# rrwick/Autocycler

Measured on NVIDIA H100. Metric: input-assembly Mbp/sec through compress->unitig GFA, higher is better.
Workload: dtype u64

## Files before the change

### autocycler_b200/csrc/backend.h

```cpp
#pragma once
#include <cstddef>
#include <cstdint>
#include <cstdio>
#include <cstdlib>
#include <cstring>
#include <stdexcept>
#include <string>

extern unsigned long long g_ac_kernel_launches;

#ifdef AC_EMULATE
#define AC_HD inline
#define AC_D inline

template <class T> inline T ac_atomic_cas(T* p, T cmp, T val) { T old = *p; if (old == cmp) *p = val; return old; }
template <class T> inline T ac_atomic_add(T* p, T v) { T old = *p; *p = (T)(old + v); return old; }
template <class T> inline T ac_atomic_or(T* p, T v) { T old = *p; *p = (T)(old | v); return old; }
template <class T> inline T ac_atomic_and(T* p, T v) { T old = *p; *p = (T)(old & v); return old; }
template <class T> inline T ac_atomic_min(T* p, T v) { T old = *p; if (v < old) *p = v; return old; }
template <class T> inline T ac_atomic_max(T* p, T v) { T old = *p; if (v > old) *p = v; return old; }
template <class T> inline T ac_ld_volatile(const T* p) { return *p; }
template <class T> inline T ac_ld_cg(const T* p) { return *p; }
inline void ac_st_stream(uint32_t* p, uint32_t v) { *p = v; }
inline void ac_ld_group(const uint64_t* p, uint64_t out[4]) { out[0] = p[0]; out[1] = p[1]; out[2] = p[2]; out[3] = p[3]; }
inline uint64_t ac_umul64hi(uint64_t a, uint64_t b) { return (uint64_t)(((unsigned __int128)a * b) >> 64); }
inline uint32_t ac_popc(uint32_t v) { return (uint32_t)__builtin_popcount(v); }
inline int ac_ctz(uint32_t v) { return __builtin_ctz(v); }

struct AcStream { int dummy; };

inline void* ac_dev_alloc(size_t bytes) { void* p = malloc(bytes ? bytes : 1); if (!p) throw std::runtime_error("emu alloc failed"); return p; }
inline void ac_dev_free(void* p) { free(p); }
inline void ac_memset(void* p, int v, size_t bytes, AcStream*) { memset(p, v, bytes); }
inline void ac_h2d(void* d, const void* h, size_t bytes, AcStream*) { memcpy(d, h, bytes); }
inline void ac_d2h(void* h, const void* d, size_t bytes, AcStream*) { memcpy(h, d, bytes); }
inline void ac_copy_dd(void* dst, const void* src, size_t bytes, AcStream*) { memcpy(dst, src, bytes); }
inline void ac_sync(AcStream*) {}
inline void* ac_host_alloc(size_t bytes) { return malloc(bytes ? bytes : 1); }
inline void ac_host_free(void* p) { free(p); }
inline int ac_smem_optin() { return 227 * 1024; }
struct AcTimer { explicit AcTimer(AcStream*) {} void stop() {} float ms() const { return 0.f; } };
struct DeviceContext {
    int device; AcStream stream{};
    DeviceContext(int device, void*) : device(device) {}
    void make_current() const {}
};

template <class Body> inline void ac_launch(const char*, AcStream*, const Body& body, uint64_t n);
template <int CTAS, class Body> inline void ac_launch_occ(const char* name, AcStream* st, const Body& body, uint64_t n) { ac_launch(name, st, body, n); }
template <class Body> inline void ac_launch(const char*, AcStream*, const Body& body, uint64_t n) {
    for (uint64_t i = 0; i < n; ++i) body(i);
}
struct AcGridSync { void operator()() const {} };
template <class Body> inline void ac_launch_coop(const char*, AcStream*, const Body& body, uint64_t, uint64_t = 256) { AcGridSync sync; body(0, 1, sync); }
struct AcEvent {};
inline void ac_record(AcEvent*, AcStream*) {}
inline void ac_wait(AcStream*, AcEvent*) {}

#else
#include <cuda_runtime.h>

#ifdef __CUDACC__
#define AC_HD __host__ __device__ __forceinline__
#define AC_D __device__ __forceinline__
#else
#define AC_HD inline
#define AC_D inline
#endif

#define AC_CUDA_CHECK(expr) do { cudaError_t _e = (expr); if (_e != cudaSuccess) \
    throw std::runtime_error(std::string(#expr) + ": " + cudaGetErrorString(_e)); } while (0)

#ifdef __CUDACC__
AC_D uint64_t ac_atomic_cas(uint64_t* p, uint64_t cmp, uint64_t val) {
    return (uint64_t)atomicCAS((unsigned long long*)p, (unsigned long long)cmp, (unsigned long long)val);
}
AC_D uint32_t ac_atomic_cas(uint32_t* p, uint32_t cmp, uint32_t val) { return atomicCAS(p, cmp, val); }
AC_D uint32_t ac_atomic_add(uint32_t* p, uint32_t v) { return atomicAdd(p, v); }
AC_D uint64_t ac_atomic_add(uint64_t* p, uint64_t v) { return (uint64_t)atomicAdd((unsigned long long*)p, (unsigned long long)v); }
AC_D unsigned long long ac_atomic_add(unsigned long long* p, unsigned long long v) { return atomicAdd(p, v); }
AC_D uint32_t ac_atomic_or(uint32_t* p, uint32_t v) { return atomicOr(p, v); }
AC_D uint32_t ac_atomic_min(uint32_t* p, uint32_t v) { return atomicMin(p, v); }
AC_D uint32_t ac_atomic_max(uint32_t* p, uint32_t v) { return atomicMax(p, v); }
AC_D uint64_t ac_atomic_min(uint64_t* p, uint64_t v) { return (uint64_t)atomicMin((unsigned long long*)p, (unsigned long long)v); }
AC_D uint64_t ac_atomic_max(uint64_t* p, uint64_t v) { return (uint64_t)atomicMax((unsigned long long*)p, (unsigned long long)v); }
template <class T> AC_D T ac_ld_volatile(const T* p) { return *(const volatile T*)p; }
AC_D uint64_t ac_ld_cg(const uint64_t* p) { return (uint64_t)__ldcg(reinterpret_cast<const unsigned long long*>(p)); }
AC_D void ac_ld_group(const uint64_t* p, uint64_t out[4]) {
    asm volatile("ld.global.cg.v2.u64 {%0,%1}, [%2];" : "=l"(out[0]), "=l"(out[1]) : "l"(p) : "memory");
    asm volatile("ld.global.cg.v2.u64 {%0,%1}, [%2];" : "=l"(out[2]), "=l"(out[3]) : "l"(p + 2) : "memory");
}
AC_D void ac_st_stream(uint32_t* p, uint32_t v) { __stcs(p, v); }
AC_D uint64_t ac_umul64hi(uint64_t a, uint64_t b) { return __umul64hi(a, b); }
AC_D uint32_t ac_popc(uint32_t v) { return (uint32_t)__popc(v); }
AC_D int ac_ctz(uint32_t v) { return __ffs((int)v) - 1; }
AC_D uint64_t ac_atomic_or(uint64_t* p, uint64_t v) { return (uint64_t)atomicOr((unsigned long long*)p, (unsigned long long)v); }
AC_D uint64_t ac_atomic_and(uint64_t* p, uint64_t v) { return (uint64_t)atomicAnd((unsigned long long*)p, (unsigned long long)v); }
#endif

struct AcStream { cudaStream_t s; };

inline void* ac_dev_alloc(size_t bytes) { void* p = nullptr; AC_CUDA_CHECK(cudaMalloc(&p, bytes ? bytes : 1)); return p; }
inline void ac_dev_free(void* p) { if (p) cudaFree(p); }
inline void ac_memset(void* p, int v, size_t bytes, AcStream* st) { AC_CUDA_CHECK(cudaMemsetAsync(p, v, bytes, st->s)); }
inline void ac_h2d(void* d, const void* h, size_t bytes, AcStream* st) { AC_CUDA_CHECK(cudaMemcpyAsync(d, h, bytes, cudaMemcpyHostToDevice, st->s)); }
inline void ac_d2h(void* h, const void* d, size_t bytes, AcStream* st) { AC_CUDA_CHECK(cudaMemcpyAsync(h, d, bytes, cudaMemcpyDeviceToHost, st->s)); }
inline void ac_copy_dd(void* dst, const void* src, size_t bytes, AcStream* st) { AC_CUDA_CHECK(cudaMemcpyAsync(dst, src, bytes, cudaMemcpyDeviceToDevice, st->s)); }
inline void ac_sync(AcStream* st) { AC_CUDA_CHECK(cudaStreamSynchronize(st->s)); }
inline void ac_debug_sync(const char* name, AcStream* st) {
    static const bool on = getenv("AC_SYNC_LAUNCHES") != nullptr;
    if (!on) return;
    const cudaError_t e = cudaStreamSynchronize(st->s);
    if (e != cudaSuccess) throw std::runtime_error(std::string("kernel ") + name + " failed: " + cudaGetErrorString(e));
}
inline void* ac_host_alloc(size_t bytes) { void* p = nullptr; AC_CUDA_CHECK(cudaMallocHost(&p, bytes ? bytes : 1)); return p; }
inline void ac_host_free(void* p) { if (p) cudaFreeHost(p); }
inline uint64_t ac_sm_count() {
    static int sms = 0;
    if (!sms) { int dev = 0; cudaGetDevice(&dev); cudaDeviceGetAttribute(&sms, cudaDevAttrMultiProcessorCount, dev); if (sms <= 0) sms = 132; }
    return (uint64_t)sms;
}
inline int ac_smem_optin() {
    static int optin = -1;
    if (optin < 0) { int dev = 0; AC_CUDA_CHECK(cudaGetDevice(&dev)); AC_CUDA_CHECK(cudaDeviceGetAttribute(&optin, cudaDevAttrMaxSharedMemoryPerBlockOptin, dev)); }
    return optin;
}
struct AcEvent {
    cudaEvent_t e = nullptr;
    AcEvent() { AC_CUDA_CHECK(cudaEventCreateWithFlags(&e, cudaEventDisableTiming)); }
    AcEvent(const AcEvent&) = delete; AcEvent& operator=(const AcEvent&) = delete;
    ~AcEvent() { cudaEventDestroy(e); }
};
inline void ac_record(AcEvent* ev, AcStream* st) { AC_CUDA_CHECK(cudaEventRecord(ev->e, st->s)); }
inline void ac_wait(AcStream* st, AcEvent* ev) { AC_CUDA_CHECK(cudaStreamWaitEvent(st->s, ev->e, 0)); }
class AcTimer {
    cudaEvent_t e0 = nullptr, e1 = nullptr; AcStream* st;
public:
    explicit AcTimer(AcStream* st) : st(st) { AC_CUDA_CHECK(cudaEventCreate(&e0)); AC_CUDA_CHECK(cudaEventCreate(&e1)); AC_CUDA_CHECK(cudaEventRecord(e0, st->s)); }
    AcTimer(const AcTimer&) = delete; AcTimer& operator=(const AcTimer&) = delete;
    ~AcTimer() { cudaEventDestroy(e0); cudaEventDestroy(e1); }
    void stop() { AC_CUDA_CHECK(cudaEventRecord(e1, st->s)); }
    float ms() const { float t = 0.f; AC_CUDA_CHECK(cudaEventElapsedTime(&t, e0, e1)); return t; }
};
struct DeviceContext {
    int device; AcStream stream; bool own_stream = false;
    DeviceContext(int device, void* s) : device(device) {
        int n = 0;
        cudaError_t e = cudaGetDeviceCount(&n);
        if (e != cudaSuccess || n == 0)
            throw std::runtime_error(std::string("autocycler_gpu: no CUDA device available (") + cudaGetErrorString(e) + "); this library has no CPU path");
        AC_CUDA_CHECK(cudaSetDevice(device));
        if (s) stream.s = (cudaStream_t)s;
        else { AC_CUDA_CHECK(cudaStreamCreateWithFlags(&stream.s, cudaStreamNonBlocking)); own_stream = true; }
    }
    DeviceContext(const DeviceContext&) = delete; DeviceContext& operator=(const DeviceContext&) = delete;
    ~DeviceContext() { if (own_stream) { cudaSetDevice(device); cudaStreamDestroy(stream.s); } }
    void make_current() const { AC_CUDA_CHECK(cudaSetDevice(device)); }
};

#ifdef __CUDACC__
#include <cooperative_groups.h>
template <class... P, class... A> inline void ac_launch_kernel(const char* name, AcStream* st, void (*kernel)(P...), dim3 grid, dim3 block, size_t smem, A... args) {
    if (smem > 0) AC_CUDA_CHECK(cudaFuncSetAttribute(kernel, cudaFuncAttributeMaxDynamicSharedMemorySize, (int)smem));
    kernel<<<grid, block, smem, st->s>>>(args...);
    cudaError_t e = cudaGetLastError();
    if (e != cudaSuccess) throw std::runtime_error(std::string("launch ") + name + ": " + cudaGetErrorString(e));
    ++g_ac_kernel_launches;
    ac_debug_sync(name, st);
}

template <class Body> __global__ void __launch_bounds__(256) ac_body_kernel(const Body body, uint64_t n) {
    const uint64_t stride = (uint64_t)gridDim.x * blockDim.x;
    const uint32_t lane = threadIdx.x & 31u;
    for (uint64_t base = (uint64_t)blockIdx.x * blockDim.x + (threadIdx.x - lane); base < n; base += stride) {
        const uint64_t i = base + lane;
        if (i < n) body(i);
        __syncwarp();
    }
}

template <class Body, int CTAS> __global__ void __launch_bounds__(256, CTAS) ac_body_kernel_occ(const Body body, uint64_t n) {
    const uint64_t stride = (uint64_t)gridDim.x * blockDim.x;
    const uint32_t lane = threadIdx.x & 31u;
    for (uint64_t base = (uint64_t)blockIdx.x * blockDim.x + (threadIdx.x - lane); base < n; base += stride) {
        const uint64_t i = base + lane;
        if (i < n) body(i);
        __syncwarp();
    }
}
template <int CTAS, class Body> inline void ac_launch_occ(const char* name, AcStream* st, const Body& body, uint64_t n) {
    if (n == 0) return;
    const int threads = 256;
    const uint64_t want = (n + threads - 1) / threads, max_blocks = ac_sm_count() * (uint64_t)CTAS * 2;
    ac_launch_kernel(name, st, ac_body_kernel_occ<Body, CTAS>, (unsigned)(want < max_blocks ? want : max_blocks), threads, 0, body, n);
}

struct AcGridSync { __device__ __forceinline__ void operator()() const { cooperative_groups::this_grid().sync(); } };
template <class Body> __global__ void __launch_bounds__(256) ac_coop_kernel(const Body body) {
    AcGridSync sync;
    body((uint64_t)blockIdx.x * blockDim.x + threadIdx.x, (uint64_t)gridDim.x * blockDim.x, sync);
}
template <class Body> inline void ac_launch_coop(const char* name, AcStream* st, const Body& body, uint64_t work, uint64_t per_block = 256) {
    static int resident = 0;
    if (!resident) {
        int per_sm = 0;
        cudaOccupancyMaxActiveBlocksPerMultiprocessor(&per_sm, ac_coop_kernel<Body>, 256, 0);
        resident = per_sm * (int)ac_sm_count();
        if (resident <= 0) throw std::runtime_error(std::string("cooperative launch ") + name + ": kernel does not fit");
    }
    uint64_t want = (work + per_block - 1) / per_block;
    if (want < 1) want = 1;
    const int sms = (int)ac_sm_count();
    const uint64_t cap = resident < sms ? (uint64_t)resident : (uint64_t)sms;
    const unsigned blocks = (unsigned)(want < cap ? want : cap);
    void* args[] = {(void*)&body};
    cudaError_t e = cudaLaunchCooperativeKernel((void*)ac_coop_kernel<Body>, dim3(blocks), dim3(256), args, 0, st->s);
    if (e != cudaSuccess) throw std::runtime_error(std::string("cooperative launch ") + name + ": " + cudaGetErrorString(e));
    ++g_ac_kernel_launches;
    ac_debug_sync(name, st);
}

template <class Body> inline void ac_launch(const char* name, AcStream* st, const Body& body, uint64_t n) {
    if (n == 0) return;
    const int threads = 256;
    uint64_t want = (n + threads - 1) / threads;
    const uint64_t max_blocks = ac_sm_count() * 16;
    ac_launch_kernel(name, st, ac_body_kernel<Body>, (unsigned)(want < max_blocks ? want : max_blocks), threads, 0, body, n);
}
#endif
#endif

struct DevBuf {
    void* p = nullptr; size_t cap = 0;
    void ensure(size_t bytes) {
        if (bytes > cap) {
            ac_dev_free(p); p = nullptr; cap = 0; p = ac_dev_alloc(bytes); cap = bytes;
#ifdef AC_EMULATE
            static const bool poison = getenv("AC_EMU_POISON") != nullptr;
            if (poison) memset(p, 0xA5, cap);
#endif
        }
    }
    template <class T> T* as() { return (T*)p; }
    ~DevBuf() { ac_dev_free(p); }
};

struct PinBuf {
    void* p = nullptr; size_t cap = 0;
    void ensure(size_t bytes) { if (bytes > cap) { ac_host_free(p); p = nullptr; cap = 0; p = ac_host_alloc(bytes); cap = bytes; } }
    template <class T> T* as() { return (T*)p; }
    ~PinBuf() { ac_host_free(p); }
};

template <class T, uint64_t TILE, int LEVELS> struct SerialScan {
    DevBuf level[LEVELS];
    T run(AcStream* st, const T* in, T* out, uint64_t n, bool want_total, int l = 0);
};
#if defined(AC_EMULATE) || defined(__CUDACC__)
template <class T, uint64_t TILE> struct ScanSumBody {
    const T* in; uint64_t n; T* sums;
    AC_D void operator()(uint64_t t) const {
        const uint64_t lo = t * TILE, hi = lo + TILE < n ? lo + TILE : n;
        T s = 0;
        for (uint64_t x = lo; x < hi; ++x) s += in[x];
        sums[t] = s;
    }
};
template <class T, uint64_t TILE> struct ScanApplyBody {
    const T* in; T* out; uint64_t n; const T* tile_off;
    AC_D void operator()(uint64_t t) const {
        const uint64_t lo = t * TILE, hi = lo + TILE < n ? lo + TILE : n;
        T acc = tile_off ? tile_off[t] : 0;
        for (uint64_t x = lo; x < hi; ++x) { const T v = in[x]; out[x] = acc; acc += v; }
    }
};
template <class T, uint64_t TILE, int LEVELS> T SerialScan<T, TILE, LEVELS>::run(AcStream* st, const T* in, T* out, uint64_t n, bool want_total, int l) {
    if (n == 0) return 0;
    if (l >= LEVELS) throw std::runtime_error("scan too deep");
    const uint64_t nb = (n + TILE - 1) / TILE;
    if (nb == 1 && !want_total) { ac_launch("scan_apply", st, ScanApplyBody<T, TILE>{in, out, n, nullptr}, 1); return 0; }
    level[l].ensure(nb * sizeof(T));
    T* sums = level[l].template as<T>();
    T total = 0;
    ac_launch("scan_sum", st, ScanSumBody<T, TILE>{in, n, sums}, nb);
    if (nb == 1) { ac_d2h(&total, sums, sizeof(T), st); ac_sync(st); }
    else total = run(st, sums, sums, nb, want_total, l + 1);
    ac_launch("scan_apply", st, ScanApplyBody<T, TILE>{in, out, n, nb == 1 ? nullptr : sums}, nb);
    return total;
}
#endif

struct DeviceScan {
    uint32_t operator()(AcStream* st, const uint32_t* in, uint32_t* out, uint64_t n, bool want_total = true);
    void keep_total(AcStream* st, uint32_t* x, uint64_t n, uint32_t* total_dst) { (*this)(st, x, x, n, false); ac_copy_dd(total_dst, x + (n - 1), 4, st); }
#ifndef AC_EMULATE
    DevBuf state; unsigned long long epoch = 0, tickets = 0;
#else
    SerialScan<uint32_t, 256, 4> serial;
#endif
};
```

### autocycler_b200/csrc/pipeline.cu

```cuda
#include "pipeline.h"

#include <algorithm>
#include <cmath>
#include <vector>

unsigned long long g_ac_kernel_launches = 0;

#define AC_NONE32 0xFFFFFFFFu
#define AC_CHUNK 32
#define AC_MINCHUNK 128
#define AC_MAX_RANKS 16
#define AC_BOUND_STRIPES 64
#ifndef AC_INSERT_CTAS
#define AC_INSERT_CTAS 2
#endif

struct TableView {
    Slot* slots;
    uint64_t cap;
    const uint64_t* packed;
    const SeqInfo* seqs;
    uint32_t n_seqs;
    uint32_t* count_big;
    uint32_t gb;
    uint32_t alarm;
};
AC_D uint64_t table_home(const TableView& t, uint64_t h) { return ac_umul64hi(h, t.cap >> 2) << 2; }
AC_D uint32_t table_depth(const TableView& t, uint64_t slot) { return t.count_big ? t.count_big[slot] : slot_count(t.slots[slot]); }

template <int W> AC_D Key<W> window_key(const TableView& t, uint64_t g, bool dotted, const KParams& p) {
    Key<W> key = fetch_codes<W>(t.packed, g, p);
    if (dotted) {
        const SeqInfo s = t.seqs[find_seq(t.seqs, t.n_seqs, g)];
        key.d = window_dots(s, g - s.start, p.k);
    }
    return key;
}

template <int W> AC_D uint32_t table_find(const TableView& t, const Key<W>& a, const Key<W>& arc, const KParams& p) {
    const uint64_t h = key_hash(key_select(key_is_canonical(a, p), a, arc));
    const uint32_t tag = make_tag(a.d != 0, h, t.gb);
    uint64_t slot = table_home(t, h);
    for (;;) {
        const Slot e = t.slots[slot];
        if (e == AC_EMPTY_SLOT) return AC_NONE32;
        if (slot_tag(e, t.gb) == tag) {
            Key<W> rep = window_key<W>(t, slot_gpos(e, t.gb), a.d != 0, p);
            if (key_eq(rep, a) || key_eq(rep, arc)) return (uint32_t)slot;
        }
        if (++slot == t.cap) slot = 0;
    }
}

AC_D void slot_add_occurrence(const TableView& t, uint64_t slot, Slot seen, uint64_t g, uint32_t add, uint32_t flags, bool track_min, unsigned long long* counters) {
    if (!t.count_big && slot_count(seen) + add >= t.alarm) counters[3] = 1;
    if (!track_min) {
        if (t.count_big) ac_atomic_add(&t.count_big[slot], add);
        else ac_atomic_add(&t.slots[slot], (uint64_t)add << AC_SLOT_COUNT_SHIFT);
        if (flags & ~slot_flags(seen)) ac_atomic_or(&t.slots[slot], (uint64_t)flags);
        return;
    }
    if (t.count_big) ac_atomic_add(&t.count_big[slot], add);
    Slot old = seen;
    for (;;) {
        Slot nw = old | flags;
        if (!t.count_big) { nw += (uint64_t)add << AC_SLOT_COUNT_SHIFT; if (slot_count(old) + add >= t.alarm) counters[3] = 1; }
        if (g < slot_gpos(old, t.gb)) nw = slot_with_gpos(nw, g, t.gb);
        const Slot was = ac_atomic_cas(&t.slots[slot], old, nw);
        if (was == old) return;
        old = was;
    }
}

template <int W, class F> AC_D void for_each_successor(const Key<W>& a, const Key<W>& arc, bool any_dotted, const KParams& p, F&& f) {
    if (a.d == 0) {
        for (uint64_t x = 0; x < 4; ++x) {
            Key<W> s = a, src = arc;
            key_push_right(s, x, p); key_push_left(src, 3 - x, p);
            f(s, src);
        }
        if (any_dotted) { Key<W> s = a; key_push_right(s, 0, p); s.d = -1; f(s, key_rc(s, p)); }
    } else if (a.d > 0) {
        for (uint64_t x = 0; x < 4; ++x) { Key<W> s = a; key_push_right(s, x, p); s.d = a.d - 1; f(s, key_rc(s, p)); }
        if (a.d == 1) { Key<W> s = a; key_push_right(s, 0, p); s.d = -1; f(s, key_rc(s, p)); }
    } else {
        Key<W> s = a; key_push_right(s, 0, p); s.d = a.d - 1; f(s, key_rc(s, p));
    }
}

struct PackBody {
    const uint8_t* ascii; uint64_t total; uint64_t* packed; const SeqInfo* seqs; uint32_t n_seqs; uint8_t* interior;
    AC_D void operator()(uint64_t i) const {
        uint64_t word = 0;
        const uint64_t base = i * 32;
        for (uint32_t j = 0; j < 32; ++j) {
            const uint64_t g = base + j;
            const uint64_t code = g < total ? base_code(ascii[g]) : 0;
            word |= code << (62 - 2 * j);
        }
        packed[i] = word;
        if (interior) {
            const SeqInfo s = seqs[find_seq(seqs, n_seqs, base)];
            const uint64_t fs0 = base - s.start;
            interior[i] = fs0 >= (uint64_t)s.lead + 1 && fs0 + 33 + s.trail <= s.len ? 1 : 0;
        }
    }
};

template <int W> struct InsertBody {
    TableView t; KParams p;
    const uint8_t* interior;
    uint32_t g_first;
    uint32_t g_begin, g_end;
    bool track_min;
    uint32_t* pos_slot;
    unsigned long long* counters;
    bool sizing;
    uint32_t* claimed_bits;
    struct Unit { Key<W> fwd, rc; uint64_t h; uint32_t flags, g; bool valid; };
    AC_D void interior_unit(uint32_t l, const uint64_t (&x)[W + 2], Unit& u) const {
        uint64_t xs[W + 1];
#pragma unroll
        for (int j = 0; j <= W; ++j) xs[j] = x[j + 1];
        const uint32_t sh = 2 * l;
        uint64_t y[W];
        ac_stream_window<W>(xs, sh, y);
        const uint32_t al = 64 - p.top_bits;
#pragma unroll
        for (int j = W - 1; j >= 0; --j) { uint64_t v = y[j] >> al; if (al && j > 0) v |= y[j - 1] << (64 - al); u.fwd.w[j] = v; }
        u.fwd.d = 0;
        u.rc = key_rc(u.fwd, p);
        const bool canon_fwd = key_is_canonical(u.fwd, p);
        const uint32_t nb = (uint32_t)(y[W - 1] >> (62 - 2 * (p.k & 31u))) & 3u;
        const uint32_t pb = l ? (uint32_t)(xs[0] >> (64 - sh)) & 3u : (uint32_t)x[0] & 3u;
        const uint32_t out_b = canon_fwd ? nb : 3u - pb, in_b = canon_fwd ? pb : 3u - nb;
        u.flags = (1u << (AC_AUX_OBS_OUT_SHIFT + out_b)) | (1u << (AC_AUX_OBS_IN_SHIFT + in_b));
        u.h = key_hash(key_select(canon_fwd, u.fwd, u.rc));
        u.valid = true;
    }
    AC_D bool edge_unit(uint32_t g, Key<W>& fwd, Key<W>& rc, uint64_t& h, uint32_t& flags) const {
        const SeqInfo s = t.seqs[find_seq(t.seqs, t.n_seqs, g)];
        const uint64_t fs = g - s.start;
        if (!(g >= g_begin && g < g_end && fs < s.len)) return false;
        fwd = fetch_codes<W>(t.packed, g, p);
        fwd.d = window_dots(s, fs, p.k);
        rc = key_rc(fwd, p);
        const bool canon_fwd = key_is_canonical(fwd, p);
        flags = 0;
        if (fs == 0) flags |= canon_fwd ? AC_AUX_FIRST_CANON : AC_AUX_FIRST_RC;
        if (fs + 1 == s.len) flags |= canon_fwd ? AC_AUX_FIRST_RC : AC_AUX_FIRST_CANON;
        if (fwd.d == 0) {
            if (fs + 1 < s.len && window_dots(s, fs + 1, p.k) == 0) {
                const uint32_t b = packed_base(t.packed, (uint64_t)g + p.k);
                flags |= canon_fwd ? (1u << (AC_AUX_OBS_OUT_SHIFT + b)) : (1u << (AC_AUX_OBS_IN_SHIFT + 3 - b));
            }
            if (fs > 0 && window_dots(s, fs - 1, p.k) == 0) {
                const uint32_t b = packed_base(t.packed, (uint64_t)g - 1);
                flags |= canon_fwd ? (1u << (AC_AUX_OBS_IN_SHIFT + b)) : (1u << (AC_AUX_OBS_OUT_SHIFT + 3 - b));
            }
        }
        h = key_hash(key_select(canon_fwd, fwd, rc));
        return true;
    }
    template <int N> AC_D void upsert(const Unit (&u)[N], const Slot* home_group = nullptr) const {
        const uint32_t tag_mask = (1u << AC_SLOT_TAG_BITS(t.gb)) - 1u;
        const uint32_t empty_hi = 0xFFFFFFFFu << (32u - t.gb);
        bool dotted[N], done[N], failed[N];
        uint32_t tag[N], probes[N], fresh[N];
        uint64_t slot[N];
#pragma unroll
        for (int w = 0; w < N; ++w) {
            dotted[w] = u[w].valid && u[w].fwd.d != 0;
            tag[w] = make_tag(dotted[w], u[w].h, t.gb);
            slot[w] = table_home(t, u[w].h);
            done[w] = !u[w].valid; failed[w] = false; probes[w] = 0; fresh[w] = 0;
        }
        bool fetched = home_group != nullptr;
        for (;;) {
            bool claimed[N], scanning[N]; Slot q[N];
#pragma unroll
            for (int w = 0; w < N; ++w) { claimed[w] = false; q[w] = 0; scanning[w] = !done[w]; }
            for (;;) {
                Slot grp[N][4];
#pragma unroll
                for (int w = 0; w < N; ++w) {
                    if (!scanning[w]) continue;
                    if (w == 0 && fetched) { grp[0][0] = home_group[0]; grp[0][1] = home_group[1]; grp[0][2] = home_group[2]; grp[0][3] = home_group[3]; }
                    else ac_ld_group(t.slots + (slot[w] & ~3ull), grp[w]);
                }
                fetched = false;
                bool more = false;
#pragma unroll
                for (int w = 0; w < N; ++w) {
                    if (!scanning[w]) continue;
                    const uint64_t base = slot[w] & ~3ull;
                    uint32_t cand = 0;
#pragma unroll
                    for (uint32_t j = 0; j < 4; ++j) {
                        const bool is_empty = (uint32_t)(grp[w][j] >> 32) >= empty_hi;
                        const bool has_tag = ((slot_tag_word(grp[w][j]) ^ tag[w]) & tag_mask) == 0;
                        cand |= (is_empty || has_tag) ? 1u << j : 0u;
                    }
                    cand &= 0xFu << (slot[w] & 3u);
                    if (cand == 0) {
                        slot[w] = base + 4; if (slot[w] >= t.cap) slot[w] = 0;
                        if (++probes[w] > 2048) { counters[2] = 1; failed[w] = true; done[w] = true; scanning[w] = false; }
                        else more = true;
                        continue;
                    }
                    const uint32_t j = (uint32_t)ac_ctz(cand);
                    slot[w] = base + j;
                    q[w] = j == 0 ? grp[w][0] : j == 1 ? grp[w][1] : j == 2 ? grp[w][2] : grp[w][3];
                    if ((uint32_t)(q[w] >> 32) >= empty_hi) {
                        q[w] = ac_atomic_cas(&t.slots[slot[w]], (Slot)AC_EMPTY_SLOT, make_slot(u[w].g, tag[w], t.count_big ? 0u : 1u, u[w].flags, t.gb));
                        if (q[w] == AC_EMPTY_SLOT) { claimed[w] = true; scanning[w] = false; continue; }
                        if (slot_tag(q[w], t.gb) != tag[w]) { ++slot[w]; if (slot[w] >= t.cap) slot[w] = 0; more = true; continue; }
                    }
                    scanning[w] = false;
                }
                if (!more) break;
            }
#ifdef __CUDA_ARCH__
            __syncwarp();
#pragma unroll
            for (int w = 0; w < N; ++w) fresh[w] |= __ballot_sync(0xFFFFFFFFu, !done[w] && claimed[w]);
#else
            for (int w = 0; w < N; ++w) if (!done[w] && claimed[w]) fresh[w] = 1;
#endif
            Key<W> rep[N] = {};
#pragma unroll
            for (int w = 0; w < N; ++w) if (!done[w] && !claimed[w]) rep[w] = window_key<W>(t, slot_gpos(q[w], t.gb), dotted[w], p);
#pragma unroll
            for (int w = 0; w < N; ++w) {
                if (done[w]) continue;
                if (claimed[w]) {
                    if (t.count_big) ac_atomic_add(&t.count_big[slot[w]], 1u);
                    if (sizing) ac_atomic_add(&counters[0], 1ull);
                    if (dotted[w]) ac_atomic_add(&counters[1], 1ull);
                    done[w] = true;
                } else if (key_eq(rep[w], u[w].fwd) || key_eq(rep[w], u[w].rc)) {
                    if (!sizing) slot_add_occurrence(t, slot[w], q[w], u[w].g, 1u, u[w].flags, track_min, counters);
                    done[w] = true;
                } else if (++slot[w] == t.cap) slot[w] = 0;
            }
            bool all_done = true;
#pragma unroll
            for (int w = 0; w < N; ++w) all_done = all_done && done[w];
#ifdef __CUDA_ARCH__
            if (__all_sync(0xFFFFFFFFu, all_done)) break;
#else
            if (all_done) break;
#endif
        }
#pragma unroll
        for (int w = 0; w < N; ++w) {
            if (u[w].valid && !failed[w] && pos_slot) ac_st_stream(&pos_slot[u[w].g], (uint32_t)slot[w]);
            if (!claimed_bits) continue;
#ifdef __CUDA_ARCH__
            if ((threadIdx.x & 31u) == 0) claimed_bits[u[w].g >> 5] = fresh[w];
#else
            if (fresh[w]) claimed_bits[u[w].g >> 5] |= 1u << (u[w].g & 31u);
#endif
        }
    }
    AC_D void prepare(uint64_t i, Unit (&u)[2]) const {
        const uint32_t g0 = g_first + (uint32_t)(i >> 5) * 64u, l = (uint32_t)i & 31u, i0 = g0 >> 5;
        bool inner[2];
#pragma unroll
        for (int s = 0; s < 2; ++s) {
            const uint64_t b = (uint64_t)g0 + 32u * s;
            inner[s] = b >= g_begin && b + 32 <= g_end && interior[i0 + s];
        }
        uint64_t x[W + 3] = {};
        if (inner[0] || inner[1]) {
            if (inner[0]) x[0] = t.packed[i0 - 1];
#pragma unroll
            for (int j = 0; j <= W + 1; ++j) x[j + 1] = t.packed[i0 + j];
        }
#pragma unroll
        for (int s = 0; s < 2; ++s) {
            u[s].g = g0 + 32u * s + l; u[s].fwd = Key<W>(); u[s].rc = Key<W>(); u[s].h = 0; u[s].flags = 0;
            if (inner[s]) {
                uint64_t xs[W + 2];
#pragma unroll
                for (int j = 0; j <= W + 1; ++j) xs[j] = x[s + j];
                interior_unit(l, xs, u[s]);
            } else u[s].valid = edge_unit(u[s].g, u[s].fwd, u[s].rc, u[s].h, u[s].flags);
        }
    }
    AC_D void operator()(uint64_t i) const {
        Unit u[2]; prepare(i, u);
#ifdef AC_EMULATE
        Slot grp[4] = {0, 0, 0, 0};
        if (u[0].valid && !sizing) { ac_ld_group(t.slots + table_home(t, u[0].h), grp); upsert<2>(u, grp); return; }
#endif
        upsert<2>(u);
    }
};

template <int W> struct SampleBody {
    InsertBody<W> ins; uint32_t total;
    AC_D static bool sampled(uint32_t centre7) {
        uint32_t c = centre7;
        if ((c >> 6) & 2u) {
            uint32_t r = 0;
            for (int b = 0; b < 7; ++b) r |= ((c >> (2 * b)) & 3u) << (2 * (6 - b));
            c = ~r & 0x3FFFu;
        }
        return ((c * 0x9E3779B1u) >> 26) == 0;
    }
    AC_D void operator()(uint64_t i) const {
        const uint32_t g0 = (uint32_t)i * 32u;
        const uint32_t k = ins.p.k, h = ins.p.h;
        const bool interior = g0 + 32 <= total && ins.interior[g0 >> 5];
        uint32_t hits = 0;
        if (interior) {
            const uint32_t first = g0 + h - 3;
            uint64_t acc = 0;
            for (uint32_t b = 0; b < 6; ++b) acc = (acc << 2) | packed_base(ins.t.packed, (uint64_t)first + b);
            for (uint32_t l = 0; l < 32; ++l) {
                acc = (acc << 2) | packed_base(ins.t.packed, (uint64_t)first + 6 + l);
                if (sampled((uint32_t)acc & 0x3FFFu)) hits |= 1u << l;
            }
        } else if (g0 < total) {
            uint32_t sj = find_seq(ins.t.seqs, ins.t.n_seqs, g0);
            for (uint32_t l = 0; l < 32; ++l) {
                const uint32_t g = g0 + l;
                if (g >= total) break;
                while (sj + 1 < ins.t.n_seqs && ins.t.seqs[sj + 1].start <= g) ++sj;
                const SeqInfo q = ins.t.seqs[sj];
                const uint64_t fs = g - q.start;
                if (fs >= q.len || window_dots(q, fs, k) != 0) continue;
                uint32_t c = 0;
                for (uint32_t b = 0; b < 7; ++b) c = (c << 2) | packed_base(ins.t.packed, (uint64_t)g + h - 3 + b);
                if (sampled(c)) hits |= 1u << l;
            }
        }
#ifdef __CUDA_ARCH__
        for (;;) {
            const bool have = hits != 0;
            if (!__any_sync(0xFFFFFFFFu, have)) break;
            typename InsertBody<W>::Unit u[1];
            u[0].fwd = Key<W>(); u[0].rc = Key<W>(); u[0].h = 0; u[0].flags = 0; u[0].g = g0; u[0].valid = have;
            if (have) {
                const uint32_t l = (uint32_t)ac_ctz(hits); hits &= hits - 1; u[0].g = g0 + l;
                u[0].fwd = fetch_codes<W>(ins.t.packed, u[0].g, ins.p); u[0].rc = key_rc(u[0].fwd, ins.p);
                u[0].h = key_hash(key_select(key_is_canonical(u[0].fwd, ins.p), u[0].fwd, u[0].rc));
            }
            ins.template upsert<1>(u);
        }
#else
        for (; hits; hits &= hits - 1) {
            typename InsertBody<W>::Unit u[1];
            u[0].g = g0 + (uint32_t)ac_ctz(hits); u[0].flags = 0; u[0].valid = true;
            u[0].fwd = fetch_codes<W>(ins.t.packed, u[0].g, ins.p); u[0].rc = key_rc(u[0].fwd, ins.p);
            u[0].h = key_hash(key_select(key_is_canonical(u[0].fwd, ins.p), u[0].fwd, u[0].rc));
            ins.template upsert<1>(u);
        }
#endif
    }
};

struct ExtNode { uint64_t h; bool flip, palindrome; };
template <int W> AC_D ExtNode ext_node(const Key<W>& m, const Key<W>& m_rc) {
    const int c = key_cmp_codes(m, m_rc);
    ExtNode n; n.flip = c > 0; n.palindrome = c == 0; n.h = key_hash(key_select(n.flip, m_rc, m));
    return n;
}
AC_D uint64_t ext_word(uint64_t h, uint64_t n_words) { return ac_umul64hi(h * 0x9E3779B97F4A7C15ull, n_words); }
AC_D uint32_t ext_other_strand(uint32_t e) { const uint32_t s = e < 5 ? e : e - 5; return (e < 5 ? 5u : 0u) + (s == 4 ? 4u : 3u - s); }
AC_D uint64_t ext_bits(uint64_t h, uint32_t e) {
    const uint64_t x = (h ^ (e + 1) * 0xD6E8FEB86659FD93ull) * 0x9E3779B97F4A7C15ull;
    return (1ull << (x >> 58)) | (1ull << ((x >> 52) & 63)) | (1ull << ((x >> 46) & 63));
}
template <int W> AC_D void ext_add(uint64_t* filter, uint64_t n_words, const Key<W>& m, const Key<W>& m_rc, uint32_t e) {
    const ExtNode n = ext_node(m, m_rc);
    uint64_t mask = ext_bits(n.h, n.flip ? ext_other_strand(e) : e);
    if (n.palindrome) mask |= ext_bits(n.h, ext_other_strand(e));
    uint64_t* w = &filter[ext_word(n.h, n_words)];
    if ((ac_ld_volatile(w) & mask) != mask) ac_atomic_or(w, mask);
}
template <int W> AC_D void ext_add_kmer(uint64_t* filter, uint64_t n_words, const Key<W>& f, const Key<W>& r, const KParams& p) {
    if (f.d == 0 || f.d == -1) ext_add<W>(filter, n_words, key_prefix(f), key_suffix(r, p), f.d ? 4u : (uint32_t)f.w[W - 1] & 3u);
    if (f.d == 0 || f.d == 1) ext_add<W>(filter, n_words, key_suffix(f, p), key_prefix(r), 5u + (f.d ? 4u : key_base(f, 0, p)));
}
AC_D uint32_t ext_test(uint64_t word, const ExtNode& n, uint32_t side, uint32_t want) {
    uint32_t got = 0;
#pragma unroll
    for (uint32_t s = 0; s < 5; ++s) {
        const uint32_t e = 5 * side + s;
        const uint64_t m = ext_bits(n.h, n.flip ? ext_other_strand(e) : e);
        if (((want >> s) & 1u) && (word & m) == m) got |= 1u << s;
    }
    return got;
}

template <int W> struct AdjacencyBody {
    TableView t; KParams p; bool any_dotted; const uint32_t* occupied; uint8_t* flags8;
    const uint64_t* filter; uint64_t n_fwords;
    AC_D void operator()(uint64_t x) const {
        const uint64_t i = occupied[x];
        const Slot e = t.slots[i];
        const uint32_t aux = slot_flags(e);
        const Key<W> f = window_key<W>(t, slot_gpos(e, t.gb), slot_dotted(e, t.gb), p);
        const Key<W> r = key_rc(f, p);
        const bool canon_fwd = key_is_canonical(f, p);
        const Key<W> c = key_select(canon_fwd, f, r), crc = key_select(canon_fwd, r, f);
        uint32_t out_c = 0, in_c = 0, cand;
        if (c.d == 0) {
            const uint32_t obs_out = (aux >> AC_AUX_OBS_OUT_SHIFT) & 15u, obs_in = (aux >> AC_AUX_OBS_IN_SHIFT) & 15u;
            out_c = ac_popc(obs_out); in_c = ac_popc(obs_in);
            const uint32_t syms = any_dotted ? 31u : 15u;
            const ExtNode last = ext_node<W>(key_suffix(c, p), key_prefix(crc)), first = ext_node<W>(key_prefix(c), key_suffix(crc, p));
            const uint64_t w_last = filter[ext_word(last.h, n_fwords)], w_first = filter[ext_word(first.h, n_fwords)];
            cand = ext_test(w_last, last, 0, syms & ~obs_out) | ext_test(w_first, first, 1, syms & ~obs_in) << 5;
        } else {
            const int32_t d = c.d;
            cand = (d > 0 ? 15u : 0u) | (d == 1 || d < 0 ? 16u : 0u) | (d < 0 ? 15u << 5 : 0u) | (d == -1 || d > 0 ? 16u << 5 : 0u);
        }
        for (; cand; cand &= cand - 1) {
            const uint32_t j = (uint32_t)ac_ctz(cand), s = j < 5 ? j : j - 5;
            Key<W> a = c;
            if (j < 5) { key_push_right(a, s & 3u, p); a.d = s == 4 ? (c.d > 0 ? -1 : c.d - 1) : (c.d > 0 ? c.d - 1 : c.d); }
            else { key_push_left(a, s & 3u, p); a.d = s == 4 ? (c.d < 0 ? 1 : c.d + 1) : (c.d < 0 ? c.d + 1 : c.d); }
            if (table_find<W>(t, a, key_rc(a, p), p) != AC_NONE32) { if (j < 5) ++out_c; else ++in_c; }
        }
        uint32_t bits = 0;
        if (out_c == 1 && !(aux & AC_AUX_FIRST_RC)) bits |= AC_FLAG8_OUT_OK;
        if (in_c == 1 && !(aux & AC_AUX_FIRST_CANON)) bits |= AC_FLAG8_IN_OK;
        flags8[i] = (uint8_t)bits;
    }
};
template <int W> struct AdjacencyOwnBody {
    AdjacencyBody<W> all; const uint32_t* range; uint64_t w0, w1;
    AC_D void operator()(uint64_t x) const { x += range[w0]; if (x < range[w1]) all(x); }
};

struct BoundaryBody {
    const uint64_t* packed; const SeqInfo* seqs; uint32_t n_seqs; uint32_t h; uint64_t g_begin, g_end;
    const uint32_t* pos_slot; const uint8_t* flags8; const uint8_t* interior;
    uint32_t* bmask; uint32_t* bcount;
    struct State { uint32_t slot; bool valid, first, in_ok, out_ok; };
    AC_D State state(uint64_t g, bool known_interior) const {
        State st; st.slot = 0; st.valid = false; st.first = false; st.in_ok = false; st.out_ok = false;
        if (!known_interior) {
            if (g < g_begin || g >= g_end) return st;
            const SeqInfo s = seqs[find_seq(seqs, n_seqs, g)];
            const uint64_t fs = g - s.start;
            if (fs >= s.len) return st;
            st.first = fs == 0;
        }
        st.valid = true;
        st.slot = pos_slot[g];
        const uint8_t fl = flags8[st.slot];
        const bool o = packed_base(packed, g + h) < 2;
        st.in_ok = o ? (fl & 2) : (fl & 1); st.out_ok = o ? (fl & 1) : (fl & 2);
        return st;
    }
    AC_D static bool starts(const State& me, const State& prev) {
        if (!me.valid) return false;
        const bool merged = !me.first && prev.out_ok && me.in_ok && me.slot != prev.slot;
        return !merged;
    }
    AC_D void operator()(uint64_t g) const {
        const uint64_t g0 = g & ~31ull;
        const bool inside = interior[g0 >> 5] && g0 >= g_begin && g0 + 32 <= g_end;
#ifdef __CUDA_ARCH__
        const uint32_t lane = (uint32_t)g & 31u;
        State me, prev; prev.valid = true; prev.first = false; prev.in_ok = false;
        if (inside) {
            const bool extra = lane == 0;
            const uint32_t slot = pos_slot[g], slot_b = extra ? pos_slot[g - 1] : 0u;
            const uint32_t fl = flags8[slot], fl_b = extra ? flags8[slot_b] : 0u;
            const bool o = packed_base(packed, g + h) < 2, o_b = extra && packed_base(packed, g - 1 + h) < 2;
            me.valid = true; me.first = false; me.slot = slot; me.in_ok = o ? (fl & 2u) : (fl & 1u); me.out_ok = o ? (fl & 1u) : (fl & 2u);
            prev.slot = __shfl_up_sync(0xFFFFFFFFu, slot, 1); prev.out_ok = __shfl_up_sync(0xFFFFFFFFu, (int)me.out_ok, 1) != 0;
            if (extra) { prev.slot = slot_b; prev.out_ok = o_b ? (fl_b & 1u) : (fl_b & 2u); }
        } else {
            me = state(g, false);
            prev.slot = __shfl_up_sync(0xFFFFFFFFu, me.slot, 1); prev.out_ok = __shfl_up_sync(0xFFFFFFFFu, (int)me.out_ok, 1) != 0;
            if (lane == 0 && me.valid && !me.first) prev = state(g - 1, false);
        }
        const uint32_t word = __ballot_sync(0xFFFFFFFFu, starts(me, prev));
        if (lane == 0) { bmask[g0 >> 5] = word; bcount[g0 >> 5] = (uint32_t)__popc(word); }
#else
        if (g != g0) return;
        uint32_t word = 0;
        State prev = state(g0, inside);
        if (prev.valid && !prev.first) { const State before = state(g0 - 1, false); if (starts(prev, before)) word |= 1u; } else if (prev.valid) word |= 1u;
        for (uint32_t j = 1; j < 32; ++j) { const State me = state(g0 + j, inside); if (starts(me, prev)) word |= 1u << j; prev = me; }
        bmask[g0 >> 5] = word; bcount[g0 >> 5] = (uint32_t)__builtin_popcount(word);
#endif
    }
};

struct RunScatterBody {
    const uint32_t* bmask; const uint32_t* boff; uint64_t* run_start;
    AC_D void operator()(uint64_t i) const {
        uint32_t bits = bmask[i];
        uint32_t off = boff[i];
        while (bits) {
            const int b = ac_ctz(bits);
            run_start[off++] = i * 32 + (uint64_t)b;
            bits &= bits - 1;
        }
    }
};

struct RunEndsLocalBody {
    const SeqInfo* seqs; uint32_t n_seqs; const uint64_t* run_start; uint64_t n_runs; const uint32_t* pos_slot;
    uint32_t* run_len; uint32_t* run_hs; uint32_t* run_ts;
    AC_D void operator()(uint64_t r) const {
        const uint64_t g0 = run_start[r];
        const SeqInfo s = seqs[find_seq(seqs, n_seqs, g0)];
        const uint64_t seq_last = s.start + s.len - 1;
        uint64_t g1 = seq_last;
        if (r + 1 < n_runs && run_start[r + 1] <= seq_last) g1 = run_start[r + 1] - 1;
        run_len[r] = (uint32_t)(g1 - g0 + 1); run_hs[r] = pos_slot[g0]; run_ts[r] = pos_slot[g1];
    }
};
struct RunExportBody {
    const uint64_t* run_start; const uint32_t* run_len; const uint32_t* run_hs; const uint32_t* run_ts; const Slot* slots; uint32_t gb; RunRec* out;
    AC_D void operator()(uint64_t r) const {
        RunRec x; x.start = (uint32_t)run_start[r]; x.len = run_len[r];
        x.head_rep = (uint32_t)slot_gpos(slots[run_hs[r]], gb); x.tail_rep = (uint32_t)slot_gpos(slots[run_ts[r]], gb);
        out[r] = x;
    }
};
struct RunImportBody {
    const RunRec* in; const uint32_t* pos_slot; uint64_t* run_start; uint32_t* run_len; uint32_t* run_hs; uint32_t* run_ts;
    uint32_t n_ranks; uint64_t first[AC_MAX_RANKS + 1]; const RunRec* src[AC_MAX_RANKS];
    AC_D void operator()(uint64_t r) const {
        const RunRec* from = in + r;
        if (n_ranks) { uint32_t q = 0; while (q + 1 < n_ranks && first[q + 1] <= r) ++q; from = src[q] + (r - first[q]); }
        const RunRec x = *from;
        run_start[r] = x.start; run_len[r] = x.len; run_hs[r] = pos_slot[x.head_rep]; run_ts[r] = pos_slot[x.tail_rep];
    }
};
struct RunKeyBody {
    const uint64_t* packed; uint32_t h; const uint64_t* run_start; const uint32_t* run_hs; const uint32_t* run_ts;
    uint32_t* run_uk; uint8_t* run_dir; uint32_t* uid_rep;
    AC_D void operator()(uint64_t r) const {
        const uint32_t hs = run_hs[r], ts = run_ts[r];
        const uint32_t uk = hs < ts ? hs : ts;
        uint8_t dir;
        if (hs != ts) dir = hs < ts ? 0 : 1;
        else dir = packed_base(packed, run_start[r] + h) < 2 ? 0 : 1;
        run_uk[r] = uk; run_dir[r] = dir;
        ac_atomic_min(&uid_rep[uk], (uint32_t)r);
    }
};

struct RepFlagBody {
    const uint32_t* run_uk; const uint32_t* uid_rep; uint32_t* is_rep;
    AC_D void operator()(uint64_t r) const { is_rep[r] = uid_rep[run_uk[r]] == (uint32_t)r ? 1u : 0u; }
};

struct RunAssignBody {
    const uint64_t* run_start; const uint32_t* run_len; const uint32_t* run_uk; const uint8_t* run_dir;
    const uint32_t* uid_rep; const uint32_t* rep_idx; const uint32_t* run_hs; const uint32_t* run_ts; TableView t;
    uint32_t* run_unitig; DeviceUnitig* unitigs; uint32_t* slot_unitig;
    AC_D void operator()(uint64_t r) const {
        const uint32_t rep = uid_rep[run_uk[r]];
        const uint32_t j = rep_idx[rep];
        run_unitig[r] = (j << 1) | (run_dir[r] == run_dir[rep] ? 1u : 0u);
        if (rep == (uint32_t)r) {
            const uint32_t hs = run_hs[r], ts = run_ts[r];
            DeviceUnitig u;
            u.start = run_start[r]; u.len = run_len[r]; u.depth = table_depth(t, hs); u.flip = 0; u.min_d = 0;
            u.head_slot = hs; u.tail_slot = ts;
            for (int w = 0; w < AC_MAX_W; ++w) u.min_w[w] = 0;
            unitigs[j] = u;
            slot_unitig[hs] = j; slot_unitig[ts] = j;
        }
    }
};

struct ClaimedCountBody { const uint32_t* bits; uint64_t n_words; uint32_t* cnt; AC_D void operator()(uint64_t w) const { cnt[w] = w < n_words ? ac_popc(bits[w]) : 0u; } };
template <int W> struct ClaimedListBody {
    const uint32_t* bits; const uint32_t* off; const uint32_t* pos_slot; uint32_t* list;
    TableView t; KParams p; const uint8_t* interior; uint64_t* filter; uint64_t n_fwords;
    AC_D void operator()(uint64_t g) const {
        const uint32_t m = bits[g >> 5], b = (uint32_t)g & 31u;
        if (!((m >> b) & 1u)) return;
        list[off[g >> 5] + ac_popc(m & ((1u << b) - 1u))] = pos_slot[g];
        if (filter) {
            const Key<W> f = window_key<W>(t, g, !interior[g >> 5], p);
            ext_add_kmer<W>(filter, n_fwords, f, key_rc(f, p), p);
        }
    }
};
struct ExportScatterBody {
    TableView t; const uint32_t* occupied; SlotRec* out;
    AC_D void operator()(uint64_t x) const { const uint64_t i = occupied[x]; SlotRec r; r.slot = t.slots[i]; r.count = table_depth(t, i); r.pad = 0; out[x] = r; }
};
template <int W> struct MergeBody {
    TableView t; KParams p; const SlotRec* in; uint32_t* pos_slot; unsigned long long* counters; uint32_t* claimed_bits;
    AC_D void operator()(uint64_t i) const {
        const SlotRec r = in[i];
        const uint64_t g = slot_gpos(r.slot, t.gb);
        const bool dotted = slot_dotted(r.slot, t.gb);
        const uint32_t flags = slot_flags(r.slot);
        const Key<W> fwd = window_key<W>(t, g, dotted, p);
        const Key<W> rc = key_rc(fwd, p);
        const uint64_t h = key_hash(key_is_canonical(fwd, p) ? fwd : rc);
        const uint32_t tag = make_tag(dotted, h, t.gb);
        const Slot mine = make_slot(g, tag, t.count_big ? 0u : r.count, flags, t.gb);
        if (!t.count_big && r.count >= t.alarm) counters[3] = 1;
        uint64_t slot = table_home(t, h);
        for (uint32_t probes = 0;; ++probes) {
            if (probes > 8192) { counters[2] = 1; return; }
            Slot e = ac_ld_cg(&t.slots[slot]);
            if (e == AC_EMPTY_SLOT) {
                e = ac_atomic_cas(&t.slots[slot], (Slot)AC_EMPTY_SLOT, mine);
                if (e == AC_EMPTY_SLOT) { if (t.count_big) ac_atomic_add(&t.count_big[slot], r.count); if (dotted) ac_atomic_add(&counters[1], 1ull); ac_atomic_or(&claimed_bits[g >> 5], 1u << (g & 31u)); break; }
            }
            if (slot_tag(e, t.gb) == tag) {
                const Key<W> rep = window_key<W>(t, slot_gpos(e, t.gb), dotted, p);
                if (key_eq(rep, fwd) || key_eq(rep, rc)) { slot_add_occurrence(t, slot, e, g, r.count, flags, true, counters); break; }
            }
            if (++slot == t.cap) slot = 0;
        }
        pos_slot[g] = (uint32_t)slot;
    }
};

struct ChunkCountBody {
    const DeviceUnitig* unitigs; uint32_t* nchunks;
    AC_D void operator()(uint64_t j) const { nchunks[j] = (unitigs[j].len + AC_MINCHUNK - 1) / AC_MINCHUNK; }
};

template <int W> struct MinPartial { Key<W> key; uint32_t from_rc; };

template <int W> struct ChunkMinBody {
    const uint64_t* packed; const SeqInfo* seqs; uint32_t n_seqs; KParams p;
    const DeviceUnitig* unitigs; uint32_t n_unitigs; const uint32_t* chunk_off; MinPartial<W>* partial;
    AC_D void operator()(uint64_t c) const {
        uint32_t lo = 0, hi = n_unitigs;
        while (hi - lo > 1) { uint32_t mid = (lo + hi) >> 1; if (chunk_off[mid] <= c) lo = mid; else hi = mid; }
        const DeviceUnitig u = unitigs[lo];
        const uint64_t first = (c - chunk_off[lo]) * AC_MINCHUNK;
        const uint64_t n = (u.len - first < AC_MINCHUNK) ? u.len - first : AC_MINCHUNK;
        uint64_t g = u.start + first;
        const SeqInfo s = seqs[find_seq(seqs, n_seqs, g)];
        uint64_t fs = g - s.start;
        Key<W> fwd, rc, best = Key<W>(); bool rolling = false, have = false; uint32_t best_rc = 0;
        for (uint64_t t = 0; t < n; ++t, ++g, ++fs) {
            const int32_t d = window_dots(s, fs, p.k);
            if (d != 0) { fwd = fetch_codes<W>(packed, g, p); fwd.d = d; rc = key_rc(fwd, p); rolling = false; }
            else if (!rolling) { fwd = fetch_codes<W>(packed, g, p); rc = key_rc(fwd, p); rolling = true; }
            else { const uint64_t code = packed_base(packed, g + p.k - 1); key_push_right(fwd, code, p); key_push_left(rc, 3 - code, p); }
            if (!have || key_less5(fwd, best)) { best = fwd; best_rc = 0; have = true; }
            if (key_less5(rc, best)) { best = rc; best_rc = 1; }
        }
        MinPartial<W> out; out.key = best; out.from_rc = best_rc;
        partial[c] = out;
    }
};

template <int W> struct UnitigMinBody {
    const uint32_t* chunk_off; const MinPartial<W>* partial; DeviceUnitig* unitigs;
    AC_D void operator()(uint64_t j) const {
        const uint32_t c0 = chunk_off[j], c1 = chunk_off[j + 1];
        MinPartial<W> best = partial[c0];
        for (uint32_t c = c0 + 1; c < c1; ++c) { const MinPartial<W> q = partial[c]; if (key_less5(q.key, best.key)) best = q; }
        DeviceUnitig u = unitigs[j];
        u.flip = best.from_rc; u.min_d = best.key.d;
        for (int w = 0; w < W; ++w) u.min_w[w] = best.key.w[w];
        unitigs[j] = u;
    }
};

template <int W> struct LinkBody {
    TableView t; KParams p; bool any_dotted;
    const DeviceUnitig* unitigs; const uint32_t* pos_slot; const uint32_t* slot_unitig;
    uint32_t* link_count; uint32_t* links;
    AC_D void operator()(uint64_t i) const {
        const uint32_t j = (uint32_t)(i >> 1), e = (uint32_t)(i & 1);
        const DeviceUnitig u = unitigs[j];
        Key<W> tail, tail_rc;
        if (e == 0) {
            const uint64_t g = u.start + u.len - 1;
            tail = fetch_codes<W>(t.packed, g, p);
            const SeqInfo s = t.seqs[find_seq(t.seqs, t.n_seqs, g)];
            tail.d = window_dots(s, g - s.start, p.k);
            tail_rc = key_rc(tail, p);
        } else {
            const uint64_t g = u.start;
            tail_rc = fetch_codes<W>(t.packed, g, p);
            const SeqInfo s = t.seqs[find_seq(t.seqs, t.n_seqs, g)];
            tail_rc.d = window_dots(s, g - s.start, p.k);
            tail = key_rc(tail_rc, p);
        }
        uint32_t n = 0;
        for_each_successor<W>(tail, tail_rc, any_dotted, p, [&](const Key<W>& a, const Key<W>& arc) {
            const uint32_t s2 = table_find<W>(t, a, arc, p);
            if (s2 == AC_NONE32) return;
            const uint32_t j2 = slot_unitig[s2];
            const DeviceUnitig v = unitigs[j2];
            const bool a_canon = key_is_canonical(a, p);
            const bool head_fwd = v.head_slot == s2 && ((packed_base(t.packed, v.start + p.h) < 2) == a_canon);
            if (n < AC_MAX_LINKS) links[i * AC_MAX_LINKS + n] = (j2 << 1) | (head_fwd ? 0u : 1u);
            ++n;
        });
        link_count[i] = n;
    }
};

struct alignas(16) SortRec { uint64_t a, b; uint32_t c, d, id, pad; };
struct SeedLess {
    const DeviceUnitig* unitigs; int W;
    typedef SortRec Key;
    AC_D Key load(uint32_t id) const {
        const DeviceUnitig& x = unitigs[id];
        Key k; k.id = id; k.pad = 0; k.a = x.min_w[0]; k.b = W > 1 ? x.min_w[1] : 0; k.c = x.min_d > 0 ? (uint32_t)x.min_d : 0u; k.d = x.min_d < 0 ? (uint32_t)-x.min_d : 0u;
        return k;
    }
    AC_D bool less_keys(const Key& x, const Key& y, uint32_t ia, uint32_t ib) const {
        if (x.c != y.c) return x.c > y.c;
        if (x.a != y.a) return x.a < y.a;
        if (x.b != y.b) return x.b < y.b;
        if (W > 2) return (*this)(ia, ib);
        return x.d > y.d;
    }
    AC_D bool operator()(uint32_t a, uint32_t b) const {
        const DeviceUnitig& x = unitigs[a]; const DeviceUnitig& y = unitigs[b];
        const int lx = x.min_d > 0 ? x.min_d : 0, ly = y.min_d > 0 ? y.min_d : 0;
        if (lx != ly) return lx > ly;
        for (int w = 0; w < W; ++w) if (x.min_w[w] != y.min_w[w]) return x.min_w[w] < y.min_w[w];
        const int tx = x.min_d < 0 ? -x.min_d : 0, ty = y.min_d < 0 ? -y.min_d : 0;
        return tx > ty;
    }
};
#define AC_SORT_LEAF 8
#define AC_SORT_WAYS 8
template <class Less> struct MergeWaysBody {
    Less less; uint32_t n, width, steps; const SortRec* in; SortRec* out; uint32_t* idx_out;
    AC_D void operator()(uint64_t i) const {
        const SortRec me = in[i];
        const uint64_t run = i / width, group = run / AC_SORT_WAYS, group_start = group * AC_SORT_WAYS * (uint64_t)width;
        uint32_t lo[AC_SORT_WAYS], hi[AC_SORT_WAYS];
#pragma unroll
        for (int s = 0; s < AC_SORT_WAYS; ++s) {
            const uint64_t first = group_start + (uint64_t)s * width, last = first + width;
            lo[s] = (uint32_t)(first < n ? first : n); hi[s] = (uint32_t)(last < n ? last : n);
            if (group * AC_SORT_WAYS + s == run) hi[s] = lo[s];
        }
        for (uint32_t step = 0; step < steps; ++step) {
#pragma unroll
            for (int s = 0; s < AC_SORT_WAYS; ++s) {
                if (lo[s] < hi[s]) {
                    const uint32_t mid = (lo[s] + hi[s]) >> 1;
                    const SortRec x = in[mid];
                    const bool earlier = group * AC_SORT_WAYS + s < run;
                    const bool before = earlier ? !less.less_keys(me, x, me.id, x.id) : less.less_keys(x, me, x.id, me.id);
                    if (before) lo[s] = mid + 1; else hi[s] = mid;
                }
            }
        }
        uint64_t pos = group_start + (i - run * width);
#pragma unroll
        for (int s = 0; s < AC_SORT_WAYS; ++s) {
            const uint64_t first = group_start + (uint64_t)s * width;
            if (group * AC_SORT_WAYS + s != run && first < n) pos += lo[s] - (uint32_t)first;
        }
        out[pos] = me; idx_out[pos] = me.id;
    }
};

#ifndef AC_EMULATE
#define AC_SORT_TILE 2048
#else
#define AC_SORT_TILE 16
#endif
#ifndef AC_EMULATE
template <class Less> __global__ void __launch_bounds__(1024) ac_tile_sort_kernel(const Less less, uint32_t n, uint32_t* __restrict__ idx, SortRec* __restrict__ recs) {
    extern __shared__ __align__(16) unsigned char tile_smem[];
    SortRec* keys = reinterpret_cast<SortRec*>(tile_smem);
    uint16_t* buf0 = reinterpret_cast<uint16_t*>(tile_smem + AC_SORT_TILE * sizeof(SortRec));
    uint16_t* buf1 = buf0 + AC_SORT_TILE;
    const uint32_t base = blockIdx.x * AC_SORT_TILE, count = n - base < AC_SORT_TILE ? n - base : AC_SORT_TILE;
    for (uint32_t i = threadIdx.x; i < count; i += blockDim.x) { SortRec r = less.load(base + i); r.id = base + i; r.pad = 0; keys[i] = r; }
    __syncthreads();
    auto before = [&](uint32_t x, uint32_t y) { return less.less_keys(keys[x], keys[y], base + x, base + y); };
    if (threadIdx.x < AC_SORT_TILE / AC_SORT_LEAF) {
        const uint32_t a = threadIdx.x * AC_SORT_LEAF, b = a + AC_SORT_LEAF < count ? a + AC_SORT_LEAF : count;
        uint16_t v[AC_SORT_LEAF];
        for (uint32_t x = a; x < b; ++x) {
            uint32_t y = x - a;
            while (y > 0 && before(x, v[y - 1])) { v[y] = v[y - 1]; --y; }
            v[y] = (uint16_t)x;
        }
        for (uint32_t x = a; x < b; ++x) buf0[x] = v[x - a];
    }
    __syncthreads();
    uint16_t* in = buf0; uint16_t* out = buf1;
    for (uint32_t width = AC_SORT_LEAF; width < count; width *= 2) {
        for (uint32_t i = threadIdx.x; i < count; i += blockDim.x) {
            const uint32_t me = in[i];
            const uint32_t run = i / width, pair_start = (run & ~1u) * width, run_start = run * width;
            const bool left = !(run & 1u);
            uint32_t lo, hi;
            if (left) { lo = run_start + width; hi = lo + width; } else { lo = pair_start; hi = run_start; }
            if (lo > count) lo = count;
            if (hi > count) hi = count;
            const uint32_t first = lo;
            while (lo < hi) { const uint32_t mid = (lo + hi) >> 1; const bool bf = left ? before(in[mid], me) : !before(me, in[mid]); if (bf) lo = mid + 1; else hi = mid; }
            out[pair_start + (i - run_start) + (lo - first)] = (uint16_t)me;
        }
        __syncthreads();
        uint16_t* t = in; in = out; out = t;
    }
    for (uint32_t i = threadIdx.x; i < count; i += blockDim.x) { const SortRec r = keys[in[i]]; recs[base + i] = r; idx[base + i] = r.id; }
}
#endif
template <class Less> struct TileSortBody {
    Less less; uint32_t n; uint32_t* idx; SortRec* recs;
    AC_D void operator()(uint64_t c) const {
        const uint32_t a = (uint32_t)c * AC_SORT_TILE, b = a + AC_SORT_TILE < n ? a + AC_SORT_TILE : n;
        for (uint32_t x = a; x < b; ++x) {
            uint32_t y = x;
            while (y > a && less(x, idx[y - 1])) { idx[y] = idx[y - 1]; --y; }
            idx[y] = x;
        }
        for (uint32_t x = a; x < b; ++x) { SortRec r = less.load(idx[x]); r.id = idx[x]; r.pad = 0; recs[x] = r; }
    }
};
template <class Less> static uint32_t* sort_indices(AcStream* stream, const Less& less, uint32_t n, uint32_t* a, uint32_t* b, SortRec* ra, SortRec* rb) {
    if (n == 0) return a;
    const uint64_t tiles = ((uint64_t)n + AC_SORT_TILE - 1) / AC_SORT_TILE;
#ifndef AC_EMULATE
    const size_t smem = AC_SORT_TILE * (sizeof(SortRec) + 2 * sizeof(uint16_t));
    ac_launch_kernel("tile_sort", stream, ac_tile_sort_kernel<Less>, (unsigned)tiles, 1024, smem, less, n, a, ra);
#else
    ac_launch("tile_sort", stream, TileSortBody<Less>{less, n, a, ra}, tiles);
#endif
    for (uint64_t width = AC_SORT_TILE; width < n; width *= AC_SORT_WAYS) {
        uint32_t steps = 1; while ((1ull << steps) <= width) ++steps;
        ac_launch("merge_pass", stream, MergeWaysBody<Less>{less, n, (uint32_t)width, steps, ra, rb, b}, n);
        std::swap(a, b); std::swap(ra, rb);
    }
    return a;
}

struct NumberKeyBody {
    const UnitigRec* rec; const char* arena; uint64_t* prefix;
    AC_D void operator()(uint64_t s) const {
        const unsigned char* q = (const unsigned char*)(arena + rec[s].seq_off);
        const uint32_t m = rec[s].len < 8 ? rec[s].len : 8;
        uint64_t v = 0;
        for (uint32_t i = 0; i < m; ++i) v |= (uint64_t)q[i] << (56 - 8 * i);
        prefix[s] = v;
    }
};
struct InversePermBody { const uint32_t* order; uint32_t* pos; AC_D void operator()(uint64_t n) const { pos[order[n]] = (uint32_t)n; } };
struct NumberLess {
    const UnitigRec* rec; const uint32_t* depth; const char* arena; const uint64_t* prefix;
    const uint32_t* pos;
    typedef SortRec Key;
    AC_D Key load(uint32_t id) const { Key k; k.id = id; k.pad = 0; k.a = prefix[id]; k.b = pos ? pos[id] : id; k.c = rec[id].len; k.d = depth[id]; return k; }
    AC_D bool less_keys(const Key& x, const Key& y, uint32_t ia, uint32_t ib) const {
        if (x.c != y.c) return x.c > y.c;
        if (x.a != y.a) return x.a < y.a;
        if (x.c > 8) return (*this)(ia, ib);
        if (x.d != y.d) return x.d > y.d;
        return x.b < y.b;
    }
    AC_D bool operator()(uint32_t a, uint32_t b) const {
        const uint32_t la = rec[a].len, lb = rec[b].len;
        if (la != lb) return la > lb;
        if (prefix[a] != prefix[b]) return prefix[a] < prefix[b];
        const char* x = arena + rec[a].seq_off; const char* y = arena + rec[b].seq_off;
        for (uint32_t i = 8; i < la; ++i) if (x[i] != y[i]) return (unsigned char)x[i] < (unsigned char)y[i];
        if (depth[a] != depth[b]) return depth[a] > depth[b];
        return pos ? pos[a] < pos[b] : a < b;
    }
};


struct SeedGatherBody {
    const uint32_t* perm; const DeviceUnitig* unitigs; uint32_t n;
    uint32_t* rank; uint32_t* len; uint32_t* depth; uint32_t* need; uint32_t* min_fpos; uint32_t* min_rpos;
    AC_D void operator()(uint64_t s) const {
        if (s == n) { need[s] = 0; return; }
        const uint32_t j = perm[s];
        const DeviceUnitig& u = unitigs[j];
        rank[j] = (uint32_t)s; len[s] = u.len; depth[s] = u.depth; need[s] = u.len + 2 * AC_SEQ_SLACK;
        min_fpos[s] = 0xFFFFFFFFu; min_rpos[s] = 0xFFFFFFFFu;
    }
};
struct SeqOffBody { const uint32_t* need_off; uint64_t* seq_off; AC_D void operator()(uint64_t s) const { seq_off[s] = (uint64_t)need_off[s] + AC_SEQ_SLACK; } };

struct EmitSeqBody {
    const uint64_t* packed; uint32_t h; const DeviceUnitig* unitigs; uint32_t n_unitigs; const uint32_t* chunk_off;
    const uint32_t* rank; const uint64_t* seq_off; char* arena;
    AC_D void operator()(uint64_t c) const {
        uint32_t lo = 0, hi = n_unitigs;
        while (hi - lo > 1) { uint32_t mid = (lo + hi) >> 1; if (chunk_off[mid] <= c) lo = mid; else hi = mid; }
        const DeviceUnitig u = unitigs[lo];
        const uint64_t first = (c - chunk_off[lo]) * AC_MINCHUNK;
        const uint64_t n = (u.len - first < AC_MINCHUNK) ? u.len - first : AC_MINCHUNK;
        char* dst = arena + seq_off[rank[lo]];
        const uint64_t g0 = u.start + h + first;
        if (!u.flip) for (uint64_t t = 0; t < n; ++t) dst[first + t] = "ACGT"[packed_base(packed, g0 + t)];
        else for (uint64_t t = 0; t < n; ++t) dst[u.len - 1 - (first + t)] = "TGCA"[packed_base(packed, g0 + t)];
    }
};

AC_D UStrand seed_strand(uint32_t dev_strand, const uint32_t* rank, const DeviceUnitig* unitigs) {
    const uint32_t j = dev_strand >> 1;
    return (rank[j] << 1) | ((dev_strand & 1u) ^ (unitigs[j].flip & 1u));
}

struct LinkCountBody {
    const uint32_t* link_count; const uint32_t* rank; const DeviceUnitig* unitigs; uint32_t n_strands; uint32_t* cnt;
    AC_D void operator()(uint64_t i) const {
        if (i == n_strands) { cnt[i] = 0; return; }
        cnt[seed_strand((uint32_t)i, rank, unitigs)] = link_count[i];
    }
};

struct LinkOrderBody {
    const uint32_t* link_count; const uint32_t* links; const uint32_t* rank; const DeviceUnitig* unitigs;
    const uint32_t* next_off; UStrand* next; uint32_t* prev_cnt; uint32_t* hairpins;
    AC_D static uint64_t order_key(UStrand from, UStrand t) {
        const uint32_t a = from >> 1, b = t >> 1; const bool trev = t & 1;
        uint32_t phase;
        if (!(from & 1)) phase = trev ? 1 : 0;
        else phase = trev ? (b < a ? 0 : (b == a ? 1 : 3)) : 2;
        return ((uint64_t)phase << 32) | b;
    }
    AC_D void operator()(uint64_t i) const {
        const UStrand from = seed_strand((uint32_t)i, rank, unitigs);
        const uint32_t n = link_count[i];
        UStrand t[AC_MAX_LINKS];
        for (uint32_t x = 0; x < n && x < AC_MAX_LINKS; ++x) t[x] = seed_strand(links[i * AC_MAX_LINKS + x], rank, unitigs);
        for (uint32_t x = 1; x < n; ++x) {
            const UStrand v = t[x]; const uint64_t kv = order_key(from, v); uint32_t y = x;
            while (y > 0 && order_key(from, t[y - 1]) > kv) { t[y] = t[y - 1]; --y; }
            t[y] = v;
        }
        UStrand* out = next + next_off[from];
        for (uint32_t x = 0; x < n; ++x) { out[x] = t[x]; ac_atomic_add(&prev_cnt[t[x]], 1u); if (t[x] == (from ^ 1u)) ac_atomic_add(hairpins, 1u); }
    }
};
struct PrevFillBody {
    const uint32_t* next_off; const UStrand* next; const uint32_t* prev_off; uint32_t* cursor; UStrand* prev;
    AC_D void operator()(uint64_t from) const {
        for (uint32_t x = next_off[from]; x < next_off[from + 1]; ++x) { const UStrand t = next[x]; prev[prev_off[t] + ac_atomic_add(&cursor[t], 1u)] = (UStrand)from; }
    }
};
struct PrevSortBody {
    const uint32_t* prev_off; UStrand* prev;
    AC_D void operator()(uint64_t s) const {
        UStrand* p = prev + prev_off[s]; const uint32_t n = prev_off[s + 1] - prev_off[s];
        for (uint32_t x = 1; x < n; ++x) { const UStrand v = p[x]; uint32_t y = x; while (y > 0 && p[y - 1] > v) { p[y] = p[y - 1]; --y; } p[y] = v; }
    }
};

struct PathBody {
    const SeqInfo* seqs; uint32_t n_seqs; const uint64_t* run_start; const uint32_t* run_len; const uint32_t* run_unitig;
    const uint32_t* rank; const DeviceUnitig* unitigs; UStrand* path; uint32_t* min_fpos; uint32_t* min_rpos;
    AC_D void operator()(uint64_t x) const {
        const uint32_t dev = run_unitig[x] >> 1, same = run_unitig[x] & 1;
        const uint32_t s = rank[dev];
        const bool plus = (same ^ (unitigs[dev].flip & 1u)) != 0;
        path[x] = (s << 1) | (plus ? 0u : 1u);
        const uint64_t g = run_start[x];
        const SeqInfo q = seqs[find_seq(seqs, n_seqs, g)];
        const uint32_t fs = (uint32_t)(g - q.start), mirrored = q.len - fs - run_len[x];
        ac_atomic_min(&min_fpos[s], plus ? fs : mirrored);
        ac_atomic_min(&min_rpos[s], plus ? mirrored : fs);
    }
};
struct PackRecBody {
    const uint64_t* seq_off; const uint32_t* len; const uint32_t* min_fpos; const uint32_t* min_rpos; UnitigRec* rec;
    AC_D void operator()(uint64_t s) const {
        UnitigRec r; r.seq_off = seq_off[s]; r.len = len[s]; r.min_fpos = min_fpos[s]; r.min_rpos = min_rpos[s];
        r.room_before = AC_SEQ_SLACK; r.room_after = AC_SEQ_SLACK; r.flags = 0;
        rec[s] = r;
    }
};
struct FixedSeedBody {
    const uint64_t* path_off; const UStrand* path; uint8_t* fixed_start; uint8_t* fixed_end;
    AC_D void operator()(uint64_t i) const {
        if (path_off[i + 1] == path_off[i]) return;
        const UStrand first = path[path_off[i]], last = path[path_off[i + 1] - 1];
        if (!(first & 1u)) fixed_start[first >> 1] = 1; else fixed_end[first >> 1] = 1;
        if (!(last & 1u)) fixed_end[last >> 1] = 1; else fixed_start[last >> 1] = 1;
    }
};
struct FixedSpreadBody {
    const uint8_t* seed_start; const uint8_t* seed_end; const uint32_t* next_off; const UStrand* next; const uint32_t* prev_off; const UStrand* prev;
    uint8_t* fixed_start; uint8_t* fixed_end;
    AC_D void operator()(uint64_t u) const {
        const uint32_t s = (uint32_t)u << 1;
        if (seed_start[u]) for (uint32_t x = prev_off[s]; x < prev_off[s + 1]; ++x) { const UStrand up = prev[x]; if (!(up & 1u)) fixed_end[up >> 1] = 1; else fixed_start[up >> 1] = 1; }
        if (seed_end[u]) for (uint32_t x = next_off[s]; x < next_off[s + 1]; ++x) { const UStrand down = next[x]; if (!(down & 1u)) fixed_start[down >> 1] = 1; else fixed_end[down >> 1] = 1; }
    }
};
struct CandidateView {
    const uint32_t* order; const uint32_t* next_off; const UStrand* next; const uint32_t* prev_off; const UStrand* prev;
    const uint8_t* fixed_start; const uint8_t* fixed_end;
    AC_D bool eligible(uint32_t idx, uint32_t side) const {
        const UStrand self = idx << 1;
        const uint32_t* off = side == 0 ? prev_off : next_off; const UStrand* lst = side == 0 ? prev : next;
        const uint32_t* back_off = side == 0 ? next_off : prev_off; const UStrand* back = side == 0 ? next : prev;
        const uint32_t gn = off[self + 1] - off[self];
        if (gn < 2 || (side == 0 ? fixed_start[idx] : fixed_end[idx])) return false;
        for (uint32_t a = 0; a < gn; ++a) {
            const UStrand p = lst[off[self] + a];
            if (back_off[p + 1] - back_off[p] != 1 || back[back_off[p]] != self || (p >> 1) == idx) return false;
            const bool rev = p & 1u;
            if (side == 0 ? ((!rev && fixed_end[p >> 1]) || (rev && fixed_start[p >> 1])) : ((!rev && fixed_start[p >> 1]) || (rev && fixed_end[p >> 1]))) return false;
        }
        return true;
    }
};
struct CandidateFlagBody {
    CandidateView v; uint32_t n; uint32_t* flag;
    AC_D void operator()(uint64_t x) const {
        if (x == 2ull * n) { flag[x] = 0; return; }
        flag[x] = v.eligible(v.order[x >> 1], (uint32_t)(x & 1)) ? 1u : 0u;
    }
};
struct CandidateFillBody {
    CandidateView v; const uint32_t* flag_in; const uint32_t* index; ExpandCandidate* cands; int32_t* cand_at;
    AC_D void operator()(uint64_t x) const {
        const uint32_t idx = v.order[x >> 1], side = (uint32_t)(x & 1);
        const bool is_cand = index[x + 1] != index[x];
        cand_at[2 * (size_t)idx + side] = is_cand ? (int32_t)index[x] : -1;
        if (!is_cand) return;
        const UStrand self = idx << 1;
        const uint32_t* off = side == 0 ? v.prev_off : v.next_off; const UStrand* lst = side == 0 ? v.prev : v.next;
        ExpandCandidate c; c.idx = idx; c.side = (uint16_t)side; c.gn = (uint16_t)(off[self + 1] - off[self]);
        for (uint32_t a = 0; a < 6; ++a) c.src[a] = a < c.gn ? lst[off[self] + a] : 0u;
        cands[index[x]] = c;
        (void)flag_in;
    }
};
struct DependentsBody {
    const uint32_t* next_off; const UStrand* next; const uint32_t* prev_off; const UStrand* prev; const int32_t* cand_at; ExpandDeps* deps;
    AC_D void operator()(uint64_t u) const {
        ExpandDeps d;
        d.c[0] = cand_at[2 * u]; d.c[1] = cand_at[2 * u + 1];
        for (uint32_t rev = 0; rev < 2; ++rev) {
            const UStrand s = ((uint32_t)u << 1) | rev;
            const bool one_next = next_off[s + 1] - next_off[s] == 1, one_prev = prev_off[s + 1] - prev_off[s] == 1;
            d.c[2 + 2 * rev] = (one_next && !(next[next_off[s]] & 1u)) ? cand_at[2 * (size_t)(next[next_off[s]] >> 1)] : -1;
            d.c[3 + 2 * rev] = (one_prev && !(prev[prev_off[s]] & 1u)) ? cand_at[2 * (size_t)(prev[prev_off[s]] >> 1) + 1] : -1;
        }
        deps[u] = d;
    }
};
AC_D char ac_complement(char c) { return c == 'A' ? 'T' : c == 'T' ? 'A' : c == 'C' ? 'G' : c == 'G' ? 'C' : c; }
struct CommonLengthBody {
    const ExpandCandidate* cands; const UnitigRec* rec; const char* arena; uint32_t* spec_len;
    AC_D char at(UStrand s, uint32_t side, uint32_t i) const {
        const UnitigRec& r = rec[s >> 1]; const char* p = arena + r.seq_off;
        const bool at_back = (side == 0) != (bool)(s & 1u);
        const char b = at_back ? p[r.len - 1 - i] : p[i];
        return (s & 1u) ? ac_complement(b) : b;
    }
    AC_D void operator()(uint64_t ci) const {
        const ExpandCandidate& cd = cands[ci];
        uint32_t c = rec[cd.src[0] >> 1].len;
        for (uint32_t a = 1; a < cd.gn; ++a) {
            const uint32_t la = rec[cd.src[a] >> 1].len;
            if (la < c) c = la;
            uint32_t m = 0;
            while (m < c && at(cd.src[a], cd.side, m) == at(cd.src[0], cd.side, m)) ++m;
            c = m;
        }
        spec_len[ci] = c;
    }
};

struct LevelPredBody {
    const ExpandCandidate* cands; const ExpandDeps* deps; int32_t* pred;
    AC_D int32_t before(uint32_t u, int32_t ci) const { int32_t best = -1; for (int x = 0; x < 6; ++x) { const int32_t d = deps[u].c[x]; if (d < ci && d > best) best = d; } return best; }
    AC_D void operator()(uint64_t ci) const {
        const ExpandCandidate& cd = cands[ci];
        pred[ci * 7] = before(cd.idx, (int32_t)ci);
        for (uint32_t a = 0; a < 6; ++a) pred[ci * 7 + 1 + a] = a < cd.gn ? before(cd.src[a] >> 1, (int32_t)ci) : -1;
    }
};
struct LevelRelaxBody {
    const int32_t* pred; uint32_t* level; uint32_t* changed_and_max;
    AC_D void operator()(uint64_t ci) const {
        uint32_t lv = 0;
        for (int x = 0; x < 7; ++x) { const int32_t q = pred[ci * 7 + x]; if (q >= 0) { const uint32_t l = ac_ld_volatile(&level[q]); if (l > lv) lv = l; } }
        if (lv + 1 != level[ci]) { level[ci] = lv + 1; changed_and_max[0] = 1; }
        ac_atomic_max(&changed_and_max[1], lv + 1);
    }
};
struct RelocBoundBody {
    const ExpandCandidate* cands; const UnitigRec* rec; const int32_t* cand_at; unsigned long long* bound;
    AC_D uint32_t shortest(const ExpandCandidate& cd) const { uint32_t m = 0xFFFFFFFFu; for (uint32_t a = 0; a < cd.gn; ++a) { const uint32_t l = rec[cd.src[a] >> 1].len; if (l < m) m = l; } return m; }
    AC_D unsigned long long bound_of(uint64_t ci) const {
        const ExpandCandidate& cd = cands[ci];
        const int32_t other = cand_at[2 * (size_t)cd.idx + (cd.side ^ 1u)];
        const unsigned long long mine = shortest(cd), partner = other >= 0 ? shortest(cands[other]) : 0;
        return (unsigned long long)rec[cd.idx].len + mine + 2 * partner + 10ull * AC_SEQ_SLACK + 64;
    }
    AC_D void operator()(uint64_t ci) const {
        ac_atomic_add(bound + (ci & (AC_BOUND_STRIPES - 1)), bound_of(ci));
    }
};
struct LevelsCoopBody {
    const int32_t* pred; uint32_t* level; uint32_t* flags; uint64_t n;
    template <class Sync> AC_D void operator()(uint64_t tid, uint64_t nt, Sync& sync) const {
        for (uint32_t round = 0;; ++round) {
            uint32_t* changed = flags + round % 3;
            if (tid == 0) flags[(round + 1) % 3] = 0;
            for (uint64_t ci = tid; ci < n; ci += nt) {
                uint32_t lv = 0;
                for (int x = 0; x < 7; ++x) { const int32_t q = pred[ci * 7 + x]; if (q >= 0) { const uint32_t l = ac_ld_volatile(&level[q]); if (l > lv) lv = l; } }
                if (lv + 1 != level[ci]) { level[ci] = lv + 1; *changed = 1; }
                ac_atomic_max(&flags[3], lv + 1);
            }
            sync();
            if (!ac_ld_volatile(changed)) return;
            if (round > 100000) { if (tid == 0) flags[4] = 1; return; }
        }
    }
};
struct StrandCursor { const char* base; int32_t step; uint32_t comp; };
AC_D char cursor_at(const StrandCursor& c, uint32_t i) { const char b = c.base[(int64_t)i * c.step]; return c.comp ? ac_complement(b) : b; }
AC_D uint32_t warp_first_mismatch(bool have, const StrandCursor& x, const StrandCursor& y, uint32_t limit) {
#ifdef __CUDA_ARCH__
    uint32_t mine = limit;
    const uint32_t lane = threadIdx.x & 31u;
    for (unsigned jobs = __ballot_sync(0xFFFFFFFFu, have); jobs; jobs &= jobs - 1) {
        const int o = __ffs((int)jobs) - 1;
        StrandCursor a, b;
        a.base = (const char*)__shfl_sync(0xFFFFFFFFu, (unsigned long long)x.base, o); a.step = __shfl_sync(0xFFFFFFFFu, x.step, o); a.comp = __shfl_sync(0xFFFFFFFFu, x.comp, o);
        b.base = (const char*)__shfl_sync(0xFFFFFFFFu, (unsigned long long)y.base, o); b.step = __shfl_sync(0xFFFFFFFFu, y.step, o); b.comp = __shfl_sync(0xFFFFFFFFu, y.comp, o);
        const uint32_t n = __shfl_sync(0xFFFFFFFFu, limit, o);
        uint32_t found = n;
        for (uint32_t i0 = 0; i0 < n; i0 += 32) {
            const uint32_t i = i0 + lane;
            const bool differs = i < n && cursor_at(a, i) != cursor_at(b, i);
            const unsigned m = __ballot_sync(0xFFFFFFFFu, differs);
            if (m) { found = i0 + (uint32_t)(__ffs((int)m) - 1); break; }
        }
        if ((int)lane == o) mine = found;
    }
    return mine;
#else
    if (!have) return limit;
    uint32_t m = 0;
    while (m < limit && cursor_at(x, m) == cursor_at(y, m)) ++m;
    return m;
#endif
}
AC_D void warp_copy(bool have, char* dst, const StrandCursor& src, uint32_t n) {
#ifdef __CUDA_ARCH__
    const uint32_t lane = threadIdx.x & 31u;
    for (unsigned jobs = __ballot_sync(0xFFFFFFFFu, have); jobs; jobs &= jobs - 1) {
        const int o = __ffs((int)jobs) - 1;
        StrandCursor a;
        a.base = (const char*)__shfl_sync(0xFFFFFFFFu, (unsigned long long)src.base, o); a.step = __shfl_sync(0xFFFFFFFFu, src.step, o); a.comp = __shfl_sync(0xFFFFFFFFu, src.comp, o);
        char* d = (char*)__shfl_sync(0xFFFFFFFFu, (unsigned long long)dst, o);
        const uint32_t m = __shfl_sync(0xFFFFFFFFu, n, o);
        for (uint32_t i = lane; i < m; i += 32) d[i] = cursor_at(a, i);
    }
    __syncwarp();
#else
    if (have) for (uint32_t i = 0; i < n; ++i) dst[i] = cursor_at(src, i);
#endif
}

struct ApplyLevelBody {
    const ExpandCandidate* cands; const ExpandDeps* deps; const uint32_t* level; uint32_t this_level; const uint32_t* spec_len;
    UnitigRec* rec; char* arena; unsigned long long* arena_used; unsigned long long* total_shifted; uint64_t* dirty; uint8_t* exhausted;
    bool all_due;
    unsigned long long* total_removed;
    uint32_t* due_cur = nullptr; uint32_t* due_next = nullptr;
    AC_D void count_mark(uint32_t cnd) const {
        const uint32_t lv = level[cnd];
        uint32_t* counts = !all_due && lv > this_level ? due_cur : due_next;
        ac_atomic_add(counts + lv, 1u);
    }
    AC_D StrandCursor cursor(UStrand s, uint32_t side) const {
        const UnitigRec& r = rec[s >> 1]; const char* p = arena + r.seq_off;
        const bool at_back = (side == 0) != (bool)(s & 1u);
        StrandCursor c; c.base = at_back ? p + r.len - 1 : p; c.step = at_back ? -1 : 1; c.comp = s & 1u;
        return c;
    }
    AC_D void mark(int32_t cnd, bool hard, int32_t below) const {
        if (cnd < 0 || cnd >= below || (!hard && exhausted[cnd])) return;
        ac_atomic_or(&dirty[(size_t)cnd >> 6], (uint64_t)1 << (cnd & 63));
        count_mark((uint32_t)cnd);
    }
    AC_D void operator()(uint64_t ci, uint64_t n) const {
        bool active = ci < n && level[ci] == this_level;
        if (active && !all_due) {
            const uint64_t bit = (uint64_t)1 << (ci & 63);
            if (!(ac_ld_volatile(&dirty[ci >> 6]) & bit)) active = false;
            else ac_atomic_and(&dirty[ci >> 6], ~bit);
        }
#ifdef __CUDA_ARCH__
        if (!__any_sync(0xFFFFFFFFu, active)) return;
#else
        if (!active) return;
#endif
        ExpandCandidate cd; cd.idx = 0; cd.side = 0; cd.gn = 0;
        if (active) cd = cands[ci];
        const uint32_t idx = cd.idx, gn = cd.gn, side = cd.side;
        bool dup = false, pristine = all_due; uint32_t min_len = 0xFFFFFFFFu;
        for (uint32_t a = 0; a < gn; ++a) {
            const uint32_t s = cd.src[a] >> 1;
            if (rec[s].len < min_len) min_len = rec[s].len;
            if (rec[s].flags) pristine = false;
            for (uint32_t b = 0; b < a; ++b) if (s == (cd.src[b] >> 1)) dup = true;
        }
        uint32_t common_len = 0;
        const bool compare = active && !pristine;
        if (active) common_len = pristine ? spec_len[ci] : rec[cd.src[0] >> 1].len;
        const StrandCursor first = active ? cursor(cd.src[0], side) : StrandCursor{nullptr, 0, 0};
        for (uint32_t a = 1; a < 6; ++a) {
            const bool have = compare && a < gn;
            StrandCursor other = first;
            if (have) { const uint32_t la = rec[cd.src[a] >> 1].len; if (la < common_len) common_len = la; other = cursor(cd.src[a], side); }
            const uint32_t m = warp_first_mismatch(have, other, first, common_len);
            if (have) common_len = m;
        }
        uint32_t c = common_len;
        if (c > 0) { const uint32_t cap = (min_len - 1) / (dup ? 2u : 1u); if (cap < c) c = cap; }
        const uint32_t min_pos = active ? (side == 0 ? rec[idx].min_fpos : rec[idx].min_rpos) : 0;
        if (c > 0) { if (min_pos == 0) c = 0; else if (min_pos - 1 < c) c = min_pos - 1; }
        if (active) exhausted[ci] = c == common_len;
        const bool moving = active && c > 0;
        UnitigRec d = rec[moving ? idx : 0];
        const bool relocate = moving && (side == 0 ? d.room_before < c : d.room_after < c);
        StrandCursor old_seq{arena + d.seq_off, 1, 0};
        if (relocate) {
            const uint32_t before = side == 0 ? c + 4 * AC_SEQ_SLACK : (d.room_before > AC_SEQ_SLACK ? d.room_before : AC_SEQ_SLACK);
            const uint32_t after = side == 0 ? (d.room_after > AC_SEQ_SLACK ? d.room_after : AC_SEQ_SLACK) : c + 4 * AC_SEQ_SLACK;
            const unsigned long long at_off = ac_atomic_add(arena_used, (unsigned long long)before + d.len + after);
            d.seq_off = at_off + before; d.room_before = before; d.room_after = after;
        }
        warp_copy(relocate, arena + d.seq_off, old_seq, d.len);
        StrandCursor piece = first;
        if (moving && side == 0) { piece.base = first.base + (int64_t)(c - 1) * first.step; piece.step = -first.step; }
        warp_copy(moving, side == 0 ? arena + d.seq_off - c : arena + d.seq_off + d.len, piece, c);
        if (!moving) return;
        for (uint32_t a = 0; a < gn; ++a) {
            UnitigRec& r = rec[cd.src[a] >> 1];
            const bool rev = cd.src[a] & 1u;
            if (side == 0) { if (!rev) { r.min_rpos += c; r.len -= c; r.room_after += c; } else { r.min_fpos += c; r.len -= c; r.seq_off += c; r.room_before += c; } }
            else           { if (!rev) { r.min_fpos += c; r.len -= c; r.seq_off += c; r.room_before += c; } else { r.min_rpos += c; r.len -= c; r.room_after += c; } }
            r.flags = 1;
        }
        if (side == 0) { d.seq_off -= c; d.room_before -= c; d.len += c; d.min_fpos -= c; }
        else { d.room_after -= c; d.len += c; d.min_rpos -= c; }
        d.flags = 1;
        rec[idx] = d;
        const int32_t below = all_due ? (int32_t)ci : 0x7FFFFFFF;
        { const ExpandDeps& dd = deps[idx]; const bool grew_start = side == 0;
          mark(dd.c[3], grew_start, below); mark(dd.c[4], grew_start, below); mark(dd.c[2], !grew_start, below); mark(dd.c[5], !grew_start, below); }
        for (uint32_t a = 0; a < gn; ++a) {
            const ExpandDeps& ds = deps[cd.src[a] >> 1];
            const bool trimmed_end = (side == 0) != (bool)(cd.src[a] & 1u);
            if (trimmed_end) { mark(ds.c[3], false, below); mark(ds.c[4], false, below); mark(ds.c[1], false, below); }
            else { mark(ds.c[2], false, below); mark(ds.c[5], false, below); mark(ds.c[0], false, below); }
        }
        if (c != common_len) { ac_atomic_or(&dirty[(size_t)ci >> 6], (uint64_t)1 << (ci & 63)); count_mark((uint32_t)ci); }
        ac_atomic_add(total_shifted, (unsigned long long)c);
        ac_atomic_add(total_removed, (unsigned long long)c * (gn - 1));
    }
};

#define AC_PASS_SET_WORDS (AC_BOUND_STRIPES + 3)
#define AC_PASS_SET(q) (1 + (q) * AC_PASS_SET_WORDS)
#define AC_PASS_REMOVED (1 + 2 * AC_PASS_SET_WORDS)
#define AC_PASS_WORDS (2 + 2 * AC_PASS_SET_WORDS)
struct SimplifyCoopBody {
    ApplyLevelBody apply; RelocBoundBody next_bound; uint64_t n; const uint32_t* n_levels;
    unsigned long long* c64; unsigned long long* res; uint64_t arena_cap; uint32_t first_set; bool first_is_pass_one;
    uint32_t* due; uint32_t due_stride, first_due;
    template <class Sync> AC_D void operator()(uint64_t tid, uint64_t nt, Sync& sync) const {
        const uint32_t levels = *n_levels;
        ApplyLevelBody a = apply;
        RelocBoundBody nb = next_bound;
        for (uint32_t pass = 0;; ++pass) {
            const uint32_t q = (first_set + pass) & 1u;
            unsigned long long* mine = c64 + AC_PASS_SET(q); unsigned long long* other = c64 + AC_PASS_SET(q ^ 1u);
            a.all_due = first_is_pass_one && pass == 0; a.total_shifted = mine;
            const uint32_t dq = (first_due + pass) % 3u;
            a.due_cur = due + (size_t)dq * due_stride; a.due_next = due + (size_t)((dq + 1u) % 3u) * due_stride;
            uint32_t* due_old = due + (size_t)((dq + 2u) % 3u) * due_stride;
            bool fenced = false;
            for (uint32_t l = 1; l <= levels; ++l) {
                if (!a.all_due && l < levels && ac_ld_volatile(&a.due_cur[l]) == 0) continue;
                a.this_level = l;
#ifdef AC_EMULATE
                if (getenv("AC_HOST_PROFILE")) {
                    uint64_t due = 0;
                    for (uint64_t ci = 0; ci < n; ++ci) if (a.level[ci] == l && (a.all_due || ((a.dirty[ci >> 6] >> (ci & 63)) & 1))) ++due;
                    fprintf(stderr, "[device] pass %u level %u: %llu due at its start\n", pass, l, (unsigned long long)due);
                }
#endif
                for (uint64_t base = 0; base < n; base += nt) a(base + tid, n);
                sync();
                if (!fenced && tid == 0) {
                    for (uint32_t x = 0; x < AC_PASS_SET_WORDS; ++x) other[x] = 0;
                    for (uint32_t x = 0; x <= levels; ++x) due_old[x] = 0;
                }
                fenced = true;
                if (l == levels && tid == 0) mine[2 + AC_BOUND_STRIPES] = ac_ld_volatile(c64);
            }
            nb.bound = mine + 1;
            for (uint64_t ci = tid; ci < n; ci += nt)
                if (ac_ld_volatile(&a.dirty[ci >> 6]) >> (ci & 63) & 1) {
                    ac_atomic_add(nb.bound + (ci & (AC_BOUND_STRIPES - 1)), nb.bound_of(ci));
                    ac_atomic_add(mine + 1 + AC_BOUND_STRIPES, 1ull);
                }
            sync();
            const unsigned long long moved = ac_ld_volatile(mine), used = ac_ld_volatile(mine + 2 + AC_BOUND_STRIPES);
            unsigned long long bound = 0;
            for (uint32_t x = 0; x < AC_BOUND_STRIPES; ++x) bound += ac_ld_volatile(mine + 1 + x);
            const bool go_on = moved != 0 && used + bound + 64 <= arena_cap && pass < 1000000u;
            if (tid == 0) { res[0] = moved; res[1] += moved; res[2] = pass + 1; res[3] = bound; res[4] = ac_ld_volatile(mine + 1 + AC_BOUND_STRIPES); res[5] = q ^ 1u; res[6] = used; res[7] = (dq + 1u) % 3u; }
            if (!go_on) return;
        }
    }
};

AC_D uint32_t ac_put_dec(char* p, uint32_t v) {
    char tmp[10]; uint32_t n = 0;
    do { tmp[n++] = (char)('0' + v % 10); v /= 10; } while (v);
    for (uint32_t i = 0; i < n; ++i) p[i] = tmp[n - 1 - i];
    return n;
}
AC_D uint32_t ac_dec_len(uint32_t v) { uint32_t n = 1; while (v >= 10) { v /= 10; ++n; } return n; }
struct GfaView {
    const uint32_t* order; const uint32_t* number_of;
    const UnitigRec* rec; const char* arena; const uint32_t* depth; const uint32_t* next_off; const UStrand* next;
};
struct GfaSizeBody {
    GfaView v; uint32_t n_unitigs; uint32_t* s_size; uint32_t* l_size;
    AC_D void operator()(uint64_t n) const {
        if (n == n_unitigs) { s_size[n] = 0; l_size[n] = 0; return; }
        const uint32_t idx = v.order[n], nl = ac_dec_len((uint32_t)n + 1);
        s_size[n] = 2 + nl + 1 + v.rec[idx].len + 6 + ac_dec_len(v.depth[idx]) + 4;
        uint32_t l = 0;
        for (uint32_t from = idx << 1; from <= (idx << 1 | 1u); ++from)
            for (uint32_t x = v.next_off[from]; x < v.next_off[from + 1]; ++x) l += nl + ac_dec_len(v.number_of[v.next[x] >> 1] + 1) + 11;
        l_size[n] = l;
    }
};
struct GfaSegmentBody {
    GfaView v; const uint32_t* s_off; char* text;
    AC_D void operator()(uint64_t n) const {
        const uint32_t idx = v.order[n];
        char* p = text + s_off[n];
        *p++ = 'S'; *p++ = '\t'; p += ac_put_dec(p, (uint32_t)n + 1); *p++ = '\t';
        p += v.rec[idx].len;
        *p++ = '\t'; *p++ = 'D'; *p++ = 'P'; *p++ = ':'; *p++ = 'f'; *p++ = ':'; p += ac_put_dec(p, v.depth[idx]);
        *p++ = '.'; *p++ = '0'; *p++ = '0'; *p++ = '\n';
    }
};
struct GfaChunkCountBody {
    GfaView v; uint32_t n_unitigs; uint32_t* pieces;
    AC_D void operator()(uint64_t n) const { pieces[n] = n == n_unitigs ? 0u : (v.rec[v.order[n]].len + 63) / 64; }
};
struct GfaSequenceBody {
    GfaView v; uint32_t n_unitigs; const uint32_t* piece_off; const uint32_t* s_off; char* text;
    AC_D void operator()(uint64_t t) const {
        const uint64_t c = t >> 5; const uint32_t lane = (uint32_t)t & 31u;
        uint32_t lo = 0, hi = n_unitigs;
#ifdef __CUDA_ARCH__
        while (hi - lo > 1) {
            const uint32_t step = (hi - lo + 31) / 32, probe = lo + lane * step;
            const unsigned le = __ballot_sync(0xFFFFFFFFu, probe < hi && piece_off[probe] <= c);
            lo += (uint32_t)(31 - __clz((int)le)) * step;
            hi = lo + step < hi ? lo + step : hi;
        }
#else
        while (hi - lo > 1) { const uint32_t mid = (lo + hi) >> 1; if (piece_off[mid] <= c) lo = mid; else hi = mid; }
#endif
        const uint32_t idx = v.order[lo], first = ((uint32_t)c - piece_off[lo]) * 64, len = v.rec[idx].len;
        const uint32_t m = len - first < 64 ? len - first : 64;
        const char* src = v.arena + v.rec[idx].seq_off + first;
        char* dst = text + s_off[lo] + 2 + ac_dec_len(lo + 1) + 1 + first;
        for (uint32_t i = lane; i < m; i += 32) dst[i] = src[i];
    }
};
struct GfaLinkBody {
    GfaView v; const uint32_t* l_off; char* text;
    AC_D void operator()(uint64_t n) const {
        const uint32_t idx = v.order[n];
        char* p = text + l_off[n];
        for (uint32_t rev = 0; rev < 2; ++rev) {
            const uint32_t from = idx << 1 | rev;
            for (uint32_t x = v.next_off[from]; x < v.next_off[from + 1]; ++x) {
                const UStrand to = v.next[x];
                *p++ = 'L'; *p++ = '\t'; p += ac_put_dec(p, (uint32_t)n + 1); *p++ = '\t'; *p++ = rev ? '-' : '+'; *p++ = '\t';
                p += ac_put_dec(p, v.number_of[to >> 1] + 1); *p++ = '\t'; *p++ = (to & 1u) ? '-' : '+'; *p++ = '\t'; *p++ = '0'; *p++ = 'M'; *p++ = '\n';
            }
        }
    }
};
struct PathLastBody { const uint64_t* path_off; uint8_t* last; AC_D void operator()(uint64_t i) const { if (path_off[i + 1] > path_off[i]) last[path_off[i + 1] - 1] = 1; } };
AC_D uint32_t path_number(const UStrand* path, const uint32_t* number_of, uint64_t x) { return (number_of ? number_of[path[x] >> 1] : path[x] >> 1) + 1; }
struct PathSizeBody {
    const UStrand* path; const uint32_t* number_of; const uint8_t* last; uint64_t steps; uint32_t* p_size;
    AC_D void operator()(uint64_t x) const { p_size[x] = x == steps ? 0u : ac_dec_len(path_number(path, number_of, x)) + 1 + (last[x] ? 0u : 1u); }
};
struct PathTokenBody {
    const UStrand* path; const uint32_t* number_of; uint32_t* dst; uint64_t stride; uint32_t n_ranks; uint64_t first[AC_MAX_RANKS + 1];
    AC_D void operator()(uint64_t x) const {
        uint32_t q = 0; while (q + 1 < n_ranks && first[q + 1] <= x) ++q;
        dst[(uint64_t)q * stride + (x - first[q])] = (number_of[path[x] >> 1] << 1) | (path[x] & 1u);
    }
};
struct PathTextBody {
    const UStrand* path; const uint32_t* number_of; const uint8_t* last; const uint32_t* p_off; char* text;
    AC_D void operator()(uint64_t x) const {
        char* p = text + p_off[x];
        p += ac_put_dec(p, path_number(path, number_of, x)); *p++ = (path[x] & 1u) ? '-' : '+';
        if (!last[x]) *p++ = ',';
    }
};
struct PathLineView { const uint64_t* path_off; uint32_t n_seqs; const uint32_t* p_off; const uint64_t* wrap_off; const uint32_t* pre_len; const uint32_t* suf_len; const char* blob; const uint64_t* blob_off;
                      uint64_t wrap_base; };
struct PathTextFullBody {
    const UStrand* path; const uint32_t* number_of; const uint8_t* last; PathLineView v; char* text;
    AC_D void operator()(uint64_t x) const {
        uint32_t lo = 0, hi = v.n_seqs;
        while (hi - lo > 1) { const uint32_t mid = (lo + hi) >> 1; if (v.path_off[mid] <= x) lo = mid; else hi = mid; }
        char* p = text + (v.wrap_off[lo] - v.wrap_base) + v.pre_len[lo] + v.p_off[x];
        p += ac_put_dec(p, path_number(path, number_of, x)); *p++ = (path[x] & 1u) ? '-' : '+';
        if (!last[x]) *p++ = ',';
    }
};
struct PathWrapBody {
    PathLineView v; char* text;
    AC_D void operator()(uint64_t x) const {
        const uint64_t t = x >> 5; const uint32_t lane = (uint32_t)x & 31u;
        const uint32_t i = (uint32_t)(t >> 1); const bool suffix = t & 1;
        const char* src = v.blob + v.blob_off[i] + (suffix ? v.pre_len[i] : 0u);
        char* dst = text + (v.wrap_off[i] - v.wrap_base) + (suffix ? v.pre_len[i] + v.p_off[v.path_off[i + 1]] : v.p_off[v.path_off[i]]);
        const uint32_t n = suffix ? v.suf_len[i] : v.pre_len[i];
        for (uint32_t b = lane; b < n; b += 32) dst[b] = src[b];
    }
};

struct PathOffBody {
    const SeqInfo* seqs; uint32_t n_seqs; const uint64_t* run_start; uint64_t n_runs; uint64_t* path_off;
    AC_D void operator()(uint64_t i) const {
        if (i == n_seqs) { path_off[i] = n_runs; return; }
        uint64_t lo = 0, hi = n_runs;
        while (lo < hi) { const uint64_t mid = (lo + hi) >> 1; if (run_start[mid] < seqs[i].start) lo = mid + 1; else hi = mid; }
        path_off[i] = lo;
    }
};

struct NeedleSlot { uint64_t w[2]; uint32_t id; uint32_t used; };
template <int WH> struct LiteralScanBody {
    const uint64_t* packed; const SeqInfo* seqs; uint32_t n_seqs; KParams p; uint64_t total;
    const NeedleSlot* table; uint64_t table_mask;
    LiteralHit* hits; uint64_t hit_cap; unsigned long long* n_hits;
    AC_D void operator()(uint64_t i) const {
        uint64_t g = i * 64;
        const uint64_t g1 = (g + 64 < total) ? g + 64 : total;
        uint32_t si = find_seq(seqs, n_seqs, g);
        while (g < g1) {
            const SeqInfo s = seqs[si];
            const uint64_t lo = s.start + s.lead, hi = s.start + s.lead + s.len - p.k;
            if (g > hi || s.len < p.k) { if (si + 1 >= n_seqs) return; ++si; if (seqs[si].start > g) g = seqs[si].start; continue; }
            if (g < lo) g = lo;
            if (g >= g1) return;
            const uint64_t stop = (hi + 1 < g1) ? hi + 1 : g1;
            Key<WH> key = fetch_codes<WH>(packed, g, p);
            for (;;) {
                uint64_t slot = key_hash(key) & table_mask;
                for (;;) {
                    const NeedleSlot n = table[slot];
                    if (!n.used) break;
                    bool eq = n.w[0] == key.w[0];
                    if (WH > 1) eq = eq && n.w[1] == key.w[WH - 1];
                    if (eq) { const unsigned long long at = ac_atomic_add(n_hits, 1ull); if (at < hit_cap) { LiteralHit hh; hh.needle = n.id; hh.pad = 0; hh.gpos = g; hits[at] = hh; } break; }
                    slot = (slot + 1) & table_mask;
                }
                if (++g >= stop) break;
                key_push_right(key, packed_base(packed, g + p.k - 1), p);
            }
        }
    }
};

#ifndef AC_EMULATE
#define AC_SCAN_TILE 4096
#define AC_SCAN_STATE(epoch, status, value) (((unsigned long long)(epoch) << 34) | ((unsigned long long)(status) << 32) | (unsigned long long)(value))
__global__ void __launch_bounds__(256) ac_scan_chained_kernel(const uint32_t* in, uint64_t n, uint32_t* out, unsigned long long* state, unsigned long long epoch,
                                                               unsigned long long* ticket, unsigned long long ticket_base, uint32_t n_tiles, uint32_t* total_out) {
    __shared__ uint32_t warp_tot[8];
    __shared__ uint32_t s_tile, s_prefix;
    const uint32_t lane = threadIdx.x & 31, warp = threadIdx.x >> 5;
    if (threadIdx.x == 0) s_tile = (uint32_t)(atomicAdd(ticket, 1ull) - ticket_base);
    __syncthreads();
    const uint32_t tile = s_tile;
    const uint64_t tile0 = (uint64_t)tile * AC_SCAN_TILE;
    uint32_t v[AC_SCAN_TILE / 1024][4], t[AC_SCAN_TILE / 1024], mine = 0;
#pragma unroll
    for (int r = 0; r < AC_SCAN_TILE / 1024; ++r) {
        const uint64_t i = tile0 + (uint64_t)r * 1024 + threadIdx.x * 4;
        if (i + 3 < n) { const uint4 q = *reinterpret_cast<const uint4*>(in + i); v[r][0] = q.x; v[r][1] = q.y; v[r][2] = q.z; v[r][3] = q.w; }
        else { for (int j = 0; j < 4; ++j) v[r][j] = (i + j < n) ? in[i + j] : 0; }
        t[r] = v[r][0] + v[r][1] + v[r][2] + v[r][3]; mine += t[r];
    }
    uint32_t sum = mine;
    for (int o = 16; o; o >>= 1) sum += __shfl_down_sync(0xFFFFFFFFu, sum, o);
    if (lane == 0) warp_tot[warp] = sum;
    __syncthreads();
    if (warp == 0) {
        uint32_t total = 0;
        for (int w2 = 0; w2 < 8; ++w2) total += warp_tot[w2];
        uint32_t prefix = 0;
        if (tile > 0) {
            if (lane == 0) *(volatile unsigned long long*)&state[tile] = AC_SCAN_STATE(epoch, 1, total);
            for (int64_t first = (int64_t)tile - 1; first >= 0; first -= 32) {
                const int64_t j = first - lane;
                unsigned long long w = AC_SCAN_STATE(epoch, 2, 0);
                if (j >= 0) do { w = *(volatile unsigned long long*)&state[j]; } while ((w >> 34) != epoch || ((w >> 32) & 3ull) == 0);
                const unsigned closed = __ballot_sync(0xFFFFFFFFu, ((w >> 32) & 3ull) == 2);
                const int stop = closed ? __ffs((int)closed) - 1 : 31;
                uint32_t part = (int)lane <= stop ? (uint32_t)w : 0u;
                for (int o = 16; o; o >>= 1) part += __shfl_down_sync(0xFFFFFFFFu, part, o);
                prefix += __shfl_sync(0xFFFFFFFFu, part, 0);
                if (closed) break;
            }
        }
        if (lane == 0) {
            *(volatile unsigned long long*)&state[tile] = AC_SCAN_STATE(epoch, 2, prefix + total);
            s_prefix = prefix;
            if (tile + 1 == n_tiles && total_out) *total_out = prefix + total;
        }
    }
    __syncthreads();
    uint32_t carry = s_prefix;
#pragma unroll
    for (int r = 0; r < AC_SCAN_TILE / 1024; ++r) {
        const uint64_t i = tile0 + (uint64_t)r * 1024 + threadIdx.x * 4;
        uint32_t inc = t[r];
        for (int o = 1; o < 32; o <<= 1) { const uint32_t u = __shfl_up_sync(0xFFFFFFFFu, inc, o); if (lane >= (uint32_t)o) inc += u; }
        __syncthreads();
        if (lane == 31) warp_tot[warp] = inc;
        __syncthreads();
        uint32_t wbase = 0, total = 0;
        for (uint32_t w2 = 0; w2 < 8; ++w2) { const uint32_t x = warp_tot[w2]; if (w2 < warp) wbase += x; total += x; }
        uint32_t e = carry + wbase + inc - t[r];
        if (i + 3 < n) { uint4 q; q.x = e; q.y = e + v[r][0]; q.z = q.y + v[r][1]; q.w = q.z + v[r][2]; *reinterpret_cast<uint4*>(out + i) = q; }
        else { for (int j = 0; j < 4; ++j) { if (i + j < n) out[i + j] = e; e += v[r][j]; } }
        carry += total;
    }
}
uint32_t DeviceScan::operator()(AcStream* st, const uint32_t* in, uint32_t* out, uint64_t n, bool want_total) {
    if (n == 0) return 0;
    const uint64_t nb = (n + AC_SCAN_TILE - 1) / AC_SCAN_TILE;
    if (nb > 0x7FFFFFFFull) throw std::runtime_error("scan too large");
    if ((nb + 4) * 8 > state.cap) {
        state.ensure((nb + 4) * 8 * 2);
        ac_memset(state.p, 0, state.cap, st);
        tickets = 0;
    }
    unsigned long long* s = state.as<unsigned long long>();
    epoch = (epoch + 1) & 0x3FFFFFFFull; if (epoch == 0) epoch = 1;
    ac_launch_kernel("scan", st, ac_scan_chained_kernel, (unsigned)nb, 256, 0, in, n, out, s + 2, epoch, s, tickets, (uint32_t)nb, (uint32_t*)(s + 1));
    tickets += nb;
    uint32_t total_sum = 0;
    if (want_total) { ac_d2h(&total_sum, s + 1, sizeof(uint32_t), st); ac_sync(st); }
    return total_sum;
}
#else
uint32_t DeviceScan::operator()(AcStream* st, const uint32_t* in, uint32_t* out, uint64_t n, bool want_total) { return serial.run(st, in, out, n, want_total); }
#endif

#ifdef AC_EMULATE
struct ScratchSet { std::vector<DevBuf*> bufs; };
struct ScratchBuf : DevBuf { explicit ScratchBuf(ScratchSet& set) { set.bufs.push_back(this); } };
#else
struct ScratchSet {};
struct ScratchBuf : DevBuf { explicit ScratchBuf(ScratchSet&) {} };
#endif

enum Mark {
    UPLOAD_BEGIN, UPLOAD_END,
    PACK_BEGIN, PACK_END, SAMPLE_END, INSERT_BEGIN, INSERT_END, TABLE_END,
    RUNS_BEGIN, ADJACENCY_END, BOUNDARIES_END,
    FINISH_BEGIN, UNITIGS_END, SEEDS_END, LINKS_END, SEED_SORT_END, WORK_LIST_END, SIMPLIFY_END, GFA_END,
    ALL_BUT_ARENA, RESULTS_END, N_MARKS
};
enum class Stage { UPLOADED, TABLE, RUNS };

struct DevicePipeline::Impl : DeviceContext {
    uint64_t total = 0; uint32_t n_seqs = 0, k = 0, U = 0, n_chunks = 0; int W = 0;
    DevBuf ascii, seqs, d_wrap_off, d_pre_len, d_suf_len, d_blob, d_blob_off, needles;
    ScratchSet scratch;
    ScratchBuf packed{scratch}, interior8{scratch}, slots{scratch}, pos_slot{scratch}, counters{scratch}, count_big{scratch}, claimed{scratch}, claimed_cnt{scratch}, occ_list{scratch},
        ext_filter{scratch}, hits{scratch};
    ScratchBuf flags8{scratch}, bmask{scratch}, bcount{scratch}, boff{scratch}, run_start{scratch}, run_len{scratch}, run_hs{scratch}, run_ts{scratch};
    ScratchBuf run_uk{scratch}, run_dir{scratch}, is_rep{scratch}, rep_idx{scratch}, run_unitig{scratch}, uid_rep{scratch}, slot_unitig{scratch}, unitigs{scratch}, nchunks{scratch},
        chunk_off{scratch}, partial{scratch}, link_count{scratch}, links{scratch}, sort_a{scratch}, sort_b{scratch}, sort_ra{scratch}, sort_rb{scratch}, rank{scratch}, d_len{scratch},
        d_depth{scratch}, need{scratch}, d_seq_off{scratch}, d_min_fpos{scratch}, d_min_rpos{scratch}, d_arena{scratch}, strand_cnt{scratch}, d_next_off{scratch}, d_next{scratch},
        prev_cnt{scratch}, d_prev_off{scratch}, d_prev{scratch}, d_small{scratch}, d_path{scratch}, d_path_off{scratch}, d_rec{scratch}, num_prefix{scratch}, d_fixed{scratch}, cand_flag{scratch},
        cand_index{scratch}, d_cands{scratch}, d_cand_at{scratch}, d_deps{scratch}, d_spec{scratch};
    ScratchBuf d_pred{scratch}, d_level{scratch}, d_flagmax{scratch}, d_counters64{scratch}, d_dirty{scratch}, d_exhausted{scratch}, d_due{scratch}, d_arena2{scratch}, d_arena3{scratch},
        d_pos{scratch}, sort_c{scratch}, sort_d{scratch};
    ScratchBuf d_pos2{scratch}, gfa_s_size{scratch}, gfa_l_size{scratch}, gfa_p_size{scratch}, gfa_pieces{scratch}, d_last{scratch}, d_totals{scratch}, d_text{scratch}, d_own_off{scratch},
        d_own_last{scratch}, d_own_size{scratch}, d_ptext{scratch};
    ScratchBuf own_entries{scratch}, own_runs{scratch};
    DeviceScan scan;
    PinBuf h_rec, h_depth, h_order, h_order2, h_arena, h_next_off, h_next, h_prev_off, h_prev, h_path, h_path_off, h_run_start, h_run_len;
    PinBuf h_cands, h_deps, h_spec, h_fixed, h_text, h_ptext;
#ifndef AC_EMULATE
    cudaEvent_t ev[N_MARKS];
    AcStream copy_stream;
    Impl(int device, void* stream) : DeviceContext(device, stream) {
        for (auto& e : ev) AC_CUDA_CHECK(cudaEventCreate(&e));
        AC_CUDA_CHECK(cudaStreamCreateWithFlags(&copy_stream.s, cudaStreamNonBlocking));
    }
    ~Impl() { cudaSetDevice(device); for (auto& e : ev) cudaEventDestroy(e); cudaStreamDestroy(copy_stream.s); }
    void mark(Mark m) { AC_CUDA_CHECK(cudaEventRecord(ev[m], stream.s)); }
    void wait_mark(Mark m) { AC_CUDA_CHECK(cudaEventSynchronize(ev[m])); }
    float between(Mark a, Mark b) { float ms = 0; AC_CUDA_CHECK(cudaEventElapsedTime(&ms, ev[a], ev[b])); return ms; }
#else
    AcStream copy_stream{};
    Impl(int device, void* stream) : DeviceContext(device, stream) {}
    void mark(Mark) {}
    void wait_mark(Mark) {}
    float between(Mark, Mark) { return 0.f; }
#endif
    AcEvent text_rendered, text_copied;
    void copy_text_after_rendering(uint64_t to) {
        ac_record(&text_rendered, &stream); ac_wait(&copy_stream, &text_rendered);
        if (to > R.gfa_copied) ac_d2h(h_text.as<char>() + R.gfa_copied, d_text.as<char>() + R.gfa_copied, to - R.gfa_copied, &copy_stream);
        R.gfa_copied = to;
    }
    bool arena_pending = false;
    const std::function<void()>* before_results = nullptr;

    std::vector<SeqInfo> host_seqs;
    uint64_t cap = 0, n_windows = 0, n_runs = 0, g_begin = 0, g_end = 0, n_slots_used = 0, n_dotted = 0, n_fwords = 0;
    bool any_dotted = false, is_multi = false, big_counts = false;
    Stage stage = Stage::UPLOADED;
    void require(Stage s, const char* message) const { if (stage < s) throw std::runtime_error(message); }
    TableView table_view() { return TableView{slots.as<Slot>(), cap, packed.as<uint64_t>(), seqs.as<SeqInfo>(), n_seqs, big_counts ? count_big.as<uint32_t>() : nullptr, slot_gpos_bits(total), count_alarm()}; }
    static uint32_t count_alarm() { static const uint32_t a = getenv("AC_COUNT_ALARM") ? (uint32_t)atoi(getenv("AC_COUNT_ALARM")) : AC_SLOT_COUNT_ALARM; return a; }
    template <int W> void local_w(uint32_t seq_lo, uint32_t seq_hi, bool multi);
    template <int W> void insert_w();
    uint64_t safe_cap = 0;
    int table_attempt = 0;
    std::vector<std::pair<const void*, uint64_t>> merged;
    template <int W> void merge_w(const void* dev_ptr, uint64_t n);
    template <int W> void runs_local_w();
    template <int W> void unitigs_w(PipelineResult& out);
    void host_arrays(), paths(), work_list(), simplify(), renumber(), gfa(bool split_paths);
    void results(PipelineResult& out, bool keep_positions, bool fused);
    struct Pending {
        uint64_t n_links = 0, n_cands = 0;
        uint32_t* order_built = nullptr; uint32_t* final_order = nullptr; uint8_t* fix_start = nullptr;
        DevBuf* arena_src = nullptr; uint64_t arena_final = 0;
        bool any_moved = false, gfa_on_device = false, paths_split = false;
        uint64_t bases_removed = 0, gfa_bytes = 0, gfa_copied = 0;
    } R;
    void pull_graph(PipelineResult& out, bool keep_positions);
    std::vector<char> path_blob; std::vector<uint32_t> path_pre, path_suf; uint64_t path_wrap_total = 0;
    uint64_t uploaded_bytes = 0;
    uint64_t exp_n = 0, n_own_runs = 0; uint32_t own_seq_lo = 0, own_seq_hi = 0; bool exp_valid = false;
    template <int W> uint64_t list_claimed(bool with_filter);
    template <int W> uint64_t count_entries_w();
#ifdef AC_EMULATE
    static void fill(DevBuf* b) { static const bool on = getenv("AC_EMU_POISON") != nullptr; if (on && b->p) memset(b->p, 0xA5, b->cap); }
    void poison() { for (DevBuf* b : scratch.bufs) fill(b); for (DevBuf& b : scan.serial.level) fill(&b); }
    void poison_table() { for (DevBuf* b : {&slots, &pos_slot, &claimed, &claimed_cnt, &occ_list, &count_big, &counters}) fill(b); }
#else
    void poison() {}
    void poison_table() {}
#endif
};

DevicePipeline::DevicePipeline(int device, void* stream) : impl(new Impl(device, stream)) { impl->before_results = &before_results; }
DevicePipeline::~DevicePipeline() { delete impl; }

unsigned long long DevicePipeline::kernel_launches() const { return g_ac_kernel_launches; }
DeviceContext& DevicePipeline::context() { return *impl; }

void DevicePipeline::upload(const uint8_t* ascii, uint64_t total, const SeqInfo* seqs, uint32_t n_seqs, uint32_t k, uint32_t seq_lo, uint32_t seq_hi) {
    Impl& m = *impl; m.make_current();
    if (k < 3 || (k & 1) == 0) throw std::runtime_error("k must be odd and >= 3");
    const int W = (int)((2 * k + 63) / 64);
    if (W > AC_MAX_W) throw std::runtime_error("k-mer sizes above " + std::to_string(AC_MAX_K) + " are not supported by the GPU path (no CPU fallback exists)");
    if (total >= 0xFFFFFFF0ull) throw std::runtime_error("more than 2^32 padded input bytes are not supported");
    if (n_seqs == 0 || total == 0) throw std::runtime_error("no sequences");
    m.total = total; m.n_seqs = n_seqs; m.k = k; m.W = W; m.stage = Stage::UPLOADED;
    m.host_seqs.assign(seqs, seqs + n_seqs);
    m.mark(UPLOAD_BEGIN);
    m.ascii.ensure(total);
    if (seq_lo == 0 && seq_hi >= n_seqs) { ac_h2d(m.ascii.p, ascii, total, &m.stream); m.uploaded_bytes = total; }
    else {
        if (seq_lo > seq_hi || seq_hi > n_seqs) throw std::runtime_error("bad sequence shard");
        const uint64_t b0 = seq_lo < n_seqs ? seqs[seq_lo].start : total, b1 = seq_hi < n_seqs ? seqs[seq_hi].start : total;
        if (b1 > b0) ac_h2d(m.ascii.as<uint8_t>() + b0, ascii + b0, b1 - b0, &m.stream);
        m.uploaded_bytes = b1 - b0;
    }
    m.seqs.ensure(n_seqs * sizeof(SeqInfo));
    ac_h2d(m.seqs.p, seqs, n_seqs * sizeof(SeqInfo), &m.stream);
    if (m.path_pre.size() == n_seqs) {
        std::vector<uint64_t> wrap((size_t)n_seqs + 1, 0), boff((size_t)n_seqs + 1, 0);
        for (uint32_t i = 0; i < n_seqs; ++i) { wrap[i + 1] = wrap[i] + m.path_pre[i] + m.path_suf[i]; boff[i + 1] = wrap[i + 1]; }
        m.path_wrap_total = wrap[n_seqs];
        m.d_wrap_off.ensure(wrap.size() * 8); m.d_blob_off.ensure(boff.size() * 8); m.d_pre_len.ensure((size_t)n_seqs * 4); m.d_suf_len.ensure((size_t)n_seqs * 4); m.d_blob.ensure(m.path_blob.size() + 8);
        ac_h2d(m.d_wrap_off.p, wrap.data(), wrap.size() * 8, &m.stream); ac_h2d(m.d_blob_off.p, boff.data(), boff.size() * 8, &m.stream);
        ac_h2d(m.d_pre_len.p, m.path_pre.data(), (size_t)n_seqs * 4, &m.stream); ac_h2d(m.d_suf_len.p, m.path_suf.data(), (size_t)n_seqs * 4, &m.stream);
        if (!m.path_blob.empty()) ac_h2d(m.d_blob.p, m.path_blob.data(), m.path_blob.size(), &m.stream);
        ac_sync(&m.stream);
    } else m.path_wrap_total = 0;
    m.mark(UPLOAD_END);
}

void DevicePipeline::set_path_line_texts(const char* blob, const uint32_t* prefix_len, const uint32_t* suffix_len, uint32_t n) {
    Impl& m = *impl;
    m.path_pre.assign(prefix_len, prefix_len + n); m.path_suf.assign(suffix_len, suffix_len + n);
    uint64_t bytes = 0; for (uint32_t i = 0; i < n; ++i) bytes += (uint64_t)prefix_len[i] + suffix_len[i];
    m.path_blob.assign(blob, blob + bytes);
}

void DevicePipeline::find_literals(const uint8_t* ascii_host, uint64_t total_bytes, const SeqInfo* host_seq, uint32_t n, uint32_t h,
                                   const uint64_t* needle_words, uint32_t n_needles, std::vector<LiteralHit>& out) {
    Impl& m = *impl; m.make_current();
    const int WH = (int)((2 * h + 63) / 64);
    if (WH > 2) throw std::runtime_error("end repair literals longer than 64 bases are not supported by the GPU path");
    const KParams p = make_kparams(h, WH);
    m.ascii.ensure(total_bytes); ac_h2d(m.ascii.p, ascii_host, total_bytes, &m.stream);
    m.seqs.ensure(n * sizeof(SeqInfo)); ac_h2d(m.seqs.p, host_seq, n * sizeof(SeqInfo), &m.stream);
    const uint64_t n_words = (total_bytes + 31) / 32;
    m.packed.ensure((n_words + 6) * sizeof(uint64_t));
    ac_memset(m.packed.as<uint64_t>() + n_words, 0, 6 * sizeof(uint64_t), &m.stream);
    ac_launch("pack", &m.stream, PackBody{m.ascii.as<uint8_t>(), total_bytes, m.packed.as<uint64_t>(), nullptr, 0, nullptr}, n_words);
    uint64_t cap = 64; while (cap < 4ull * n_needles) cap <<= 1;
    std::vector<NeedleSlot> table(cap);
    for (uint32_t i = 0; i < n_needles; ++i) {
        Key<2> k2; k2.w[0] = needle_words[2 * i]; k2.w[1] = needle_words[2 * i + 1]; k2.d = 0;
        uint64_t hsh;
        if (WH == 1) { Key<1> k1; k1.w[0] = k2.w[1]; k1.d = 0; hsh = key_hash(k1); } else hsh = key_hash(k2);
        uint64_t slot = hsh & (cap - 1);
        while (table[slot].used) slot = (slot + 1) & (cap - 1);
        table[slot].w[0] = WH == 1 ? k2.w[1] : k2.w[0]; table[slot].w[1] = k2.w[1]; table[slot].id = i; table[slot].used = 1;
    }
    m.needles.ensure(cap * sizeof(NeedleSlot)); ac_h2d(m.needles.p, table.data(), cap * sizeof(NeedleSlot), &m.stream);
    m.counters.ensure(8 * sizeof(unsigned long long));
    uint64_t hit_cap = 1u << 20;
    for (;;) {
        m.hits.ensure(hit_cap * sizeof(LiteralHit));
        ac_memset(m.counters.p, 0, sizeof(unsigned long long), &m.stream);
        if (WH == 1) ac_launch("literal_scan", &m.stream, LiteralScanBody<1>{m.packed.as<uint64_t>(), m.seqs.as<SeqInfo>(), n, p, total_bytes, m.needles.as<NeedleSlot>(), cap - 1,
                                                                           m.hits.as<LiteralHit>(), hit_cap, m.counters.as<unsigned long long>()}, (total_bytes + 63) / 64);
        else ac_launch("literal_scan", &m.stream, LiteralScanBody<2>{m.packed.as<uint64_t>(), m.seqs.as<SeqInfo>(), n, p, total_bytes, m.needles.as<NeedleSlot>(), cap - 1,
                                                                     m.hits.as<LiteralHit>(), hit_cap, m.counters.as<unsigned long long>()}, (total_bytes + 63) / 64);
        unsigned long long found = 0;
        ac_d2h(&found, m.counters.p, sizeof found, &m.stream); ac_sync(&m.stream);
        if (found <= hit_cap) { out.resize(found); if (found) { ac_d2h(out.data(), m.hits.p, found * sizeof(LiteralHit), &m.stream); ac_sync(&m.stream); } break; }
        hit_cap = found + 1024;
    }
    m.stage = Stage::UPLOADED;
}

#define AC_W_CASE(fn, n, ...) case n: fn<n>(__VA_ARGS__); break;
#define AC_DISPATCH_W(fn, ...) switch (W) { AC_W_CASE(fn, 1, __VA_ARGS__) AC_W_CASE(fn, 2, __VA_ARGS__) AC_W_CASE(fn, 3, __VA_ARGS__) AC_W_CASE(fn, 4, __VA_ARGS__) \
    AC_W_CASE(fn, 5, __VA_ARGS__) AC_W_CASE(fn, 6, __VA_ARGS__) AC_W_CASE(fn, 7, __VA_ARGS__) AC_W_CASE(fn, 8, __VA_ARGS__) AC_W_CASE(fn, 9, __VA_ARGS__) AC_W_CASE(fn, 10, __VA_ARGS__) \
    AC_W_CASE(fn, 11, __VA_ARGS__) AC_W_CASE(fn, 12, __VA_ARGS__) AC_W_CASE(fn, 13, __VA_ARGS__) AC_W_CASE(fn, 14, __VA_ARGS__) AC_W_CASE(fn, 15, __VA_ARGS__) AC_W_CASE(fn, 16, __VA_ARGS__) \
    default: throw std::runtime_error("upload() must precede build()"); }

#define AC_N_COUNTERS 4
template <int W> void DevicePipeline::Impl::local_w(uint32_t seq_lo, uint32_t seq_hi, bool multi) {
    const KParams p = make_kparams(k, W);
    if (seq_lo > seq_hi || seq_hi > n_seqs) throw std::runtime_error("bad sequence shard");
    const SeqInfo* hs = host_seqs.data();
    if (seq_lo == seq_hi) { g_begin = g_end = 0; }
    else { g_begin = hs[seq_lo].start; g_end = hs[seq_hi - 1].start + hs[seq_hi - 1].len; }
    is_multi = multi; own_seq_lo = seq_lo; own_seq_hi = seq_hi; exp_valid = false;
    poison();
    n_windows = total - (uint64_t)n_seqs * (k - 1);
    cap = (n_windows + n_windows / 2 + 64 + 3) & ~3ull;
    if (cap >= 0xFFFFFFF0ull) throw std::runtime_error("input too large for 32-bit slot indices");

    mark(PACK_BEGIN);
    const uint64_t n_words = (total + 31) / 32;
    packed.ensure((n_words + W + 2) * sizeof(uint64_t));
    ac_memset(packed.as<uint64_t>() + n_words, 0, (W + 2) * sizeof(uint64_t), &stream);
    interior8.ensure(n_words + 8);
    ac_launch("pack", &stream, PackBody{ascii.as<uint8_t>(), total, packed.as<uint64_t>(), seqs.as<SeqInfo>(), n_seqs, interior8.as<uint8_t>()}, n_words);
    mark(PACK_END);

    const uint64_t safe_cap = cap;
    counters.ensure(AC_N_COUNTERS * sizeof(unsigned long long));
    unsigned long long hc[AC_N_COUNTERS] = {0, 0, 0, 0};
    big_counts = getenv("AC_BIG_COUNTS") != nullptr;
    const double load = getenv("AC_TABLE_LOAD") ? atof(getenv("AC_TABLE_LOAD")) : 0.5;
    if (load > 0 && n_windows > (1u << 16) && k >= 7) {
        const uint64_t sample_cap = (n_windows / 64 * 4 + 4096) & ~3ull;
        slots.ensure(sample_cap * sizeof(Slot));
        ac_memset(slots.p, 0xFF, sample_cap * sizeof(Slot), &stream);
        ac_memset(counters.p, 0, sizeof hc, &stream);
        const TableView sv{slots.as<Slot>(), sample_cap, packed.as<uint64_t>(), seqs.as<SeqInfo>(), n_seqs, nullptr, slot_gpos_bits(total), AC_SLOT_COUNT_ALARM};
        const InsertBody<W> sample_ins{sv, p, interior8.as<uint8_t>(), 0, 0, (uint32_t)total, false, nullptr, counters.as<unsigned long long>(), true, nullptr};
        ac_launch("sample", &stream, SampleBody<W>{sample_ins, (uint32_t)total}, ((total + 31) / 32 + 31) / 32 * 32);
        ac_d2h(hc, counters.p, sizeof hc, &stream); ac_sync(&stream);
        if (!hc[2]) {
            const uint64_t est = (hc[0] + 3 * (uint64_t)std::sqrt((double)hc[0]) + 16) * 64 + (uint64_t)n_seqs * 2 * k;
            cap = std::min<uint64_t>(safe_cap, ((uint64_t)((double)est / load) + 4096 + 3) & ~3ull);
        }
    }
    mark(SAMPLE_END);
    this->safe_cap = safe_cap;
    table_attempt = 0;
    merged.clear();
    insert_w<W>();
    mark(TABLE_END);
    stage = Stage::TABLE;
}

template <int W> void DevicePipeline::Impl::insert_w() {
    const KParams p = make_kparams(k, W);
    const uint64_t n_words = (total + 31) / 32;
    unsigned long long hc[AC_N_COUNTERS] = {0, 0, 0, 0};
    pos_slot.ensure(total * sizeof(uint32_t));
    for (;; ++table_attempt) {
        if (table_attempt > 3) throw std::runtime_error("k-mer table build did not settle");
        if (getenv("AC_HOST_PROFILE")) fprintf(stderr, "[device] k-mer table attempt %d: capacity %llu, side counts %d\n", table_attempt, (unsigned long long)cap, (int)big_counts);
        poison_table();
        slots.ensure(cap * sizeof(Slot));
        ac_memset(slots.p, 0xFF, cap * sizeof(Slot), &stream);
        if (big_counts) { count_big.ensure(cap * 4); ac_memset(count_big.p, 0, cap * 4, &stream); }
        ac_memset(counters.p, 0, sizeof hc, &stream);
        const TableView tv = table_view();
        const uint64_t g_first = g_begin & ~63ull;
        claimed.ensure((n_words + 8) * 4); ac_memset(claimed.p, 0, (n_words + 8) * 4, &stream);
        const InsertBody<W> ins{tv, p, interior8.as<uint8_t>(), (uint32_t)g_first, (uint32_t)g_begin, (uint32_t)g_end, is_multi, pos_slot.as<uint32_t>(), counters.as<unsigned long long>(), false, claimed.as<uint32_t>()};
        mark(INSERT_BEGIN);
        ac_launch_occ<AC_INSERT_CTAS>("insert", &stream, ins, (g_end - g_first + 63) / 64 * 32);
        mark(INSERT_END);
        ac_d2h(hc, counters.p, sizeof hc, &stream); ac_sync(&stream);
        if (hc[2] && cap != safe_cap) { cap = safe_cap; continue; }
        if (hc[2]) throw std::runtime_error("k-mer table overflow");
        if (hc[3] && !big_counts) { big_counts = true; continue; }
        break;
    }
    ++table_attempt;
    n_dotted = hc[1];
}

template <int W> uint64_t DevicePipeline::Impl::list_claimed(bool with_filter) {
    const uint64_t n_words = (total + 31) / 32;
    claimed_cnt.ensure((n_words + 1) * 4);
    ac_launch("claimed_count", &stream, ClaimedCountBody{claimed.as<uint32_t>(), n_words, claimed_cnt.as<uint32_t>()}, n_words + 1);
    const uint64_t n = scan(&stream, claimed_cnt.as<uint32_t>(), claimed_cnt.as<uint32_t>(), n_words + 1);
    occ_list.ensure((n + 1) * 4);
    if (with_filter) {
        static const uint64_t words_env = getenv("AC_EXT_FILTER_WORDS") ? strtoull(getenv("AC_EXT_FILTER_WORDS"), nullptr, 10) : 0;
        n_fwords = words_env ? words_env : n / 2 + 64;
        ext_filter.ensure(n_fwords * 8);
        ac_memset(ext_filter.p, 0, n_fwords * 8, &stream);
    }
    ac_launch("claimed_list", &stream, ClaimedListBody<W>{claimed.as<uint32_t>(), claimed_cnt.as<uint32_t>(), pos_slot.as<uint32_t>(), occ_list.as<uint32_t>(),
                                                          table_view(), make_kparams(k, W), interior8.as<uint8_t>(), with_filter ? ext_filter.as<uint64_t>() : nullptr, n_fwords}, n_words * 32);
    return n;
}
template <int W> uint64_t DevicePipeline::Impl::count_entries_w() {
    require(Stage::TABLE, "build_local must precede the entry export");
    exp_n = list_claimed<W>(false);
    exp_valid = true;
    return exp_n;
}
void DevicePipeline::export_entries(void* dst, uint64_t cap_records) {
    Impl& m = *impl; m.make_current();
    if (cap_records < m.exp_n) throw std::runtime_error("entry buffer too small");
    ac_launch("export_scatter", &m.stream, ExportScatterBody{m.table_view(), m.occ_list.as<uint32_t>(), (SlotRec*)dst}, m.exp_n);
    ac_sync(&m.stream);
}

template <int W> void DevicePipeline::Impl::merge_w(const void* dev_ptr, uint64_t n) {
    require(Stage::TABLE, "build_local must precede merge_entries");
    const KParams p = make_kparams(k, W);
    ac_launch("merge", &stream, MergeBody<W>{table_view(), p, (const SlotRec*)dev_ptr, pos_slot.as<uint32_t>(), counters.as<unsigned long long>(), claimed.as<uint32_t>()}, n);
    merged.emplace_back(dev_ptr, n);
}

template <int W> void DevicePipeline::Impl::runs_local_w() {
    require(Stage::TABLE, "build_local must precede runs_local");
    const KParams p = make_kparams(k, W);
    mark(RUNS_BEGIN);
    if (is_multi) {
        unsigned long long hc[AC_N_COUNTERS];
        ac_d2h(hc, counters.p, sizeof hc, &stream); ac_sync(&stream);
        if (hc[2] && cap != safe_cap) {
            cap = safe_cap;
            insert_w<W>();
            const TableView tv = table_view();
            for (const auto& e : merged)
                ac_launch("merge", &stream, MergeBody<W>{tv, p, (const SlotRec*)e.first, pos_slot.as<uint32_t>(), counters.as<unsigned long long>(), claimed.as<uint32_t>()}, e.second);
            ac_d2h(hc, counters.p, sizeof hc, &stream); ac_sync(&stream);
        }
        if (hc[2]) throw std::runtime_error("k-mer table overflow while merging");
        if (hc[3] && !big_counts) throw std::runtime_error("a k-mer occurs more than 524287 times across the ranks: not supported by the multi-GPU exchange");
        n_dotted = hc[1];
    }
    any_dotted = n_dotted != 0;
    const TableView tv = table_view();

    flags8.ensure(cap);
    n_slots_used = list_claimed<W>(true);
    const AdjacencyBody<W> adj{tv, p, any_dotted, occ_list.as<uint32_t>(), flags8.as<uint8_t>(), ext_filter.as<uint64_t>(), n_fwords};
    if (is_multi && exp_valid && exp_n + 64 < n_slots_used) {
        const uint64_t n_cw = (total + 31) / 32, n_adj = exp_n + 64;
        if (getenv("AC_HOST_PROFILE")) fprintf(stderr, "[device] adjacency flags for this rank's own k-mers: at most %llu of %llu\n", (unsigned long long)n_adj, (unsigned long long)n_slots_used);
        ac_launch("adjacency", &stream, AdjacencyOwnBody<W>{adj, claimed_cnt.as<uint32_t>(), g_begin >> 5, std::min<uint64_t>((g_end + 31) >> 5, n_cw)}, n_adj);
    } else ac_launch("adjacency", &stream, adj, n_slots_used);
    mark(ADJACENCY_END);

    const uint64_t n_bwords = (total + 31) / 32;
    bmask.ensure(n_bwords * sizeof(uint32_t)); bcount.ensure(n_bwords * sizeof(uint32_t)); boff.ensure(n_bwords * sizeof(uint32_t));
    ac_launch("boundaries", &stream, BoundaryBody{packed.as<uint64_t>(), seqs.as<SeqInfo>(), n_seqs, p.h, g_begin, g_end, pos_slot.as<uint32_t>(),
                                                  flags8.as<uint8_t>(), interior8.as<uint8_t>(), bmask.as<uint32_t>(), bcount.as<uint32_t>()}, n_bwords * 32);
    n_runs = scan(&stream, bcount.as<uint32_t>(), boff.as<uint32_t>(), n_bwords);
    mark(BOUNDARIES_END);
    run_start.ensure(n_runs * sizeof(uint64_t)); run_len.ensure(n_runs * 4); run_hs.ensure(n_runs * 4); run_ts.ensure(n_runs * 4);
    ac_launch("run_scatter", &stream, RunScatterBody{bmask.as<uint32_t>(), boff.as<uint32_t>(), run_start.as<uint64_t>()}, n_bwords);
    ac_launch("run_ends", &stream, RunEndsLocalBody{seqs.as<SeqInfo>(), n_seqs, run_start.as<uint64_t>(), n_runs, pos_slot.as<uint32_t>(),
                                                    run_len.as<uint32_t>(), run_hs.as<uint32_t>(), run_ts.as<uint32_t>()}, n_runs);
    n_own_runs = n_runs;
    stage = Stage::RUNS;
}

void DevicePipeline::export_runs(void* dst, uint64_t cap_records) {
    Impl& m = *impl; m.make_current();
    m.require(Stage::RUNS, "runs_local must precede export_runs");
    if (cap_records < m.n_runs) throw std::runtime_error("run buffer too small");
    ac_launch("run_export", &m.stream, RunExportBody{m.run_start.as<uint64_t>(), m.run_len.as<uint32_t>(), m.run_hs.as<uint32_t>(), m.run_ts.as<uint32_t>(),
                                                     m.slots.as<Slot>(), slot_gpos_bits(m.total), (RunRec*)dst}, m.n_runs);
    ac_sync(&m.stream);
}

void DevicePipeline::import_runs(const void* dev_ptr, uint64_t n) {
    Impl& m = *impl; m.make_current();
    m.require(Stage::RUNS, "runs_local must precede import_runs");
    m.n_runs = n;
    m.run_start.ensure(n * sizeof(uint64_t)); m.run_len.ensure(n * 4); m.run_hs.ensure(n * 4); m.run_ts.ensure(n * 4);
    RunImportBody body{(const RunRec*)dev_ptr, m.pos_slot.as<uint32_t>(), m.run_start.as<uint64_t>(), m.run_len.as<uint32_t>(), m.run_hs.as<uint32_t>(), m.run_ts.as<uint32_t>(), 0, {0}, {nullptr}};
    ac_launch("run_import", &m.stream, body, n);
}

void DevicePipeline::import_runs_from(const void* const* ptrs, const uint64_t* counts, uint32_t n_ranks) {
    Impl& m = *impl; m.make_current();
    m.require(Stage::RUNS, "runs_local must precede import_runs");
    if (n_ranks == 0 || n_ranks > AC_MAX_RANKS) throw std::runtime_error("import_runs: bad rank count");
    RunImportBody body{nullptr, m.pos_slot.as<uint32_t>(), nullptr, nullptr, nullptr, nullptr, n_ranks, {0}, {nullptr}};
    for (uint32_t q = 0; q < n_ranks; ++q) { body.first[q + 1] = body.first[q] + counts[q]; body.src[q] = (const RunRec*)ptrs[q]; }
    const uint64_t n = m.n_runs = body.first[n_ranks];
    m.run_start.ensure(n * sizeof(uint64_t)); m.run_len.ensure(n * 4); m.run_hs.ensure(n * 4); m.run_ts.ensure(n * 4);
    body.run_start = m.run_start.as<uint64_t>(); body.run_len = m.run_len.as<uint32_t>(); body.run_hs = m.run_hs.as<uint32_t>(); body.run_ts = m.run_ts.as<uint32_t>();
    ac_launch("run_import", &m.stream, body, n);
}

void DevicePipeline::finish(PipelineResult& out, bool keep_positions, bool fused, bool split_paths) {
    Impl& m = *impl; m.make_current(); const int W = m.W;
    if (split_paths && !fused) throw std::runtime_error("split path lines need the fused finish");
    AC_DISPATCH_W(m.unitigs_w, out)
    m.host_arrays();
    m.paths();
    m.work_list();
    if (fused && m.R.n_cands > 0) m.simplify();
    m.mark(SIMPLIFY_END);
    if (fused) {
        m.renumber();
        if (m.U < 100000000u) m.gfa(split_paths);
    }
    m.mark(GFA_END);
    m.results(out, keep_positions, fused);
}

template <int W> void DevicePipeline::Impl::unitigs_w(PipelineResult& out) {
    require(Stage::RUNS, "runs_local must precede finish");
    const KParams p = make_kparams(k, W);
    const TableView tv = table_view();
    out = PipelineResult();
    out.W = W; out.capacity = cap; out.n_slots_used = n_slots_used; out.n_dotted = n_dotted;
    R = Pending();
    mark(FINISH_BEGIN);
    run_uk.ensure(n_runs * 4); run_dir.ensure(n_runs);
    is_rep.ensure(n_runs * 4); rep_idx.ensure(n_runs * 4); run_unitig.ensure(n_runs * 4);
    uid_rep.ensure(cap * 4); slot_unitig.ensure(cap * 4);
    ac_memset(uid_rep.p, 0xFF, cap * 4, &stream);
    ac_launch("run_key", &stream, RunKeyBody{packed.as<uint64_t>(), p.h, run_start.as<uint64_t>(), run_hs.as<uint32_t>(), run_ts.as<uint32_t>(),
                                             run_uk.as<uint32_t>(), run_dir.as<uint8_t>(), uid_rep.as<uint32_t>()}, n_runs);
    ac_launch("rep_flag", &stream, RepFlagBody{run_uk.as<uint32_t>(), uid_rep.as<uint32_t>(), is_rep.as<uint32_t>()}, n_runs);
    U = scan(&stream, is_rep.as<uint32_t>(), rep_idx.as<uint32_t>(), n_runs);
    unitigs.ensure((size_t)U * sizeof(DeviceUnitig));
    ac_launch("run_assign", &stream, RunAssignBody{run_start.as<uint64_t>(), run_len.as<uint32_t>(), run_uk.as<uint32_t>(), run_dir.as<uint8_t>(),
                                                   uid_rep.as<uint32_t>(), rep_idx.as<uint32_t>(), run_hs.as<uint32_t>(), run_ts.as<uint32_t>(), tv,
                                                   run_unitig.as<uint32_t>(), unitigs.as<DeviceUnitig>(), slot_unitig.as<uint32_t>()}, n_runs);
    mark(UNITIGS_END);

    nchunks.ensure(((size_t)U + 1) * 4); chunk_off.ensure(((size_t)U + 1) * 4);
    ac_launch("chunk_count", &stream, ChunkCountBody{unitigs.as<DeviceUnitig>(), nchunks.as<uint32_t>()}, U);
    ac_memset(nchunks.as<uint32_t>() + U, 0, 4, &stream);
    n_chunks = scan(&stream, nchunks.as<uint32_t>(), chunk_off.as<uint32_t>(), (uint64_t)U + 1);
    partial.ensure((size_t)n_chunks * sizeof(MinPartial<W>));
    ac_launch("chunk_min", &stream, ChunkMinBody<W>{packed.as<uint64_t>(), seqs.as<SeqInfo>(), n_seqs, p, unitigs.as<DeviceUnitig>(), U,
                                                    chunk_off.as<uint32_t>(), partial.as<MinPartial<W>>()}, n_chunks);
    ac_launch("unitig_min", &stream, UnitigMinBody<W>{chunk_off.as<uint32_t>(), partial.as<MinPartial<W>>(), unitigs.as<DeviceUnitig>()}, U);
    mark(SEEDS_END);

    link_count.ensure((size_t)U * 2 * 4); links.ensure((size_t)U * 2 * AC_MAX_LINKS * 4);
    ac_launch("links", &stream, LinkBody<W>{tv, p, any_dotted, unitigs.as<DeviceUnitig>(), pos_slot.as<uint32_t>(), slot_unitig.as<uint32_t>(),
                                            link_count.as<uint32_t>(), links.as<uint32_t>()}, (uint64_t)U * 2);
    mark(LINKS_END);
}

void DevicePipeline::Impl::host_arrays() {
    sort_a.ensure((size_t)U * 4); sort_b.ensure((size_t)U * 4); sort_ra.ensure((size_t)U * sizeof(SortRec)); sort_rb.ensure((size_t)U * sizeof(SortRec));
    const SeedLess seed_less{unitigs.as<DeviceUnitig>(), W};
    const uint32_t* perm = sort_indices(&stream, seed_less, U, sort_a.as<uint32_t>(), sort_b.as<uint32_t>(), sort_ra.as<SortRec>(), sort_rb.as<SortRec>());
    mark(SEED_SORT_END);
    rank.ensure((size_t)U * 4); d_len.ensure((size_t)U * 4); d_depth.ensure((size_t)U * 4); need.ensure(((size_t)U + 1) * 4);
    d_seq_off.ensure((size_t)U * 8); d_min_fpos.ensure((size_t)U * 4); d_min_rpos.ensure((size_t)U * 4);
    ac_launch("seed_gather", &stream, SeedGatherBody{perm, unitigs.as<DeviceUnitig>(), U, rank.as<uint32_t>(), d_len.as<uint32_t>(), d_depth.as<uint32_t>(),
                                                     need.as<uint32_t>(), d_min_fpos.as<uint32_t>(), d_min_rpos.as<uint32_t>()}, (uint64_t)U + 1);
    if (n_windows + (uint64_t)U * 2 * AC_SEQ_SLACK >= 0xFFFFFFF0ull) throw std::runtime_error("unitig sequence arena would exceed 4 GB");
    const uint64_t arena_bytes = scan(&stream, need.as<uint32_t>(), need.as<uint32_t>(), (uint64_t)U + 1);
    ac_launch("seq_off", &stream, SeqOffBody{need.as<uint32_t>(), d_seq_off.as<uint64_t>()}, U);
    d_arena.ensure(arena_bytes);
    ac_launch("emit_seq", &stream, EmitSeqBody{packed.as<uint64_t>(), make_kparams(k, W).h, unitigs.as<DeviceUnitig>(), U, chunk_off.as<uint32_t>(), rank.as<uint32_t>(),
                                               d_seq_off.as<uint64_t>(), d_arena.as<char>()}, n_chunks);
    R.arena_final = arena_bytes; R.arena_src = &d_arena;
    const uint32_t n_strands = 2 * U;
    strand_cnt.ensure(((size_t)n_strands + 1) * 4); d_next_off.ensure(((size_t)n_strands + 1) * 4);
    prev_cnt.ensure(((size_t)n_strands + 1) * 4); d_prev_off.ensure(((size_t)n_strands + 1) * 4);
    ac_launch("link_count", &stream, LinkCountBody{link_count.as<uint32_t>(), rank.as<uint32_t>(), unitigs.as<DeviceUnitig>(), n_strands, strand_cnt.as<uint32_t>()},
              (uint64_t)n_strands + 1);
    const uint64_t n_links = R.n_links = scan(&stream, strand_cnt.as<uint32_t>(), d_next_off.as<uint32_t>(), (uint64_t)n_strands + 1);
    d_next.ensure(n_links * 4); d_prev.ensure(n_links * 4);
    ac_memset(prev_cnt.p, 0, ((size_t)n_strands + 1) * 4, &stream);
    d_small.ensure(64); ac_memset(d_small.p, 0, 64, &stream);
    ac_launch("link_order", &stream, LinkOrderBody{link_count.as<uint32_t>(), links.as<uint32_t>(), rank.as<uint32_t>(), unitigs.as<DeviceUnitig>(),
                                                   d_next_off.as<uint32_t>(), d_next.as<UStrand>(), prev_cnt.as<uint32_t>(), d_small.as<uint32_t>()}, n_strands);
    scan(&stream, prev_cnt.as<uint32_t>(), d_prev_off.as<uint32_t>(), (uint64_t)n_strands + 1, false);
    ac_memset(prev_cnt.p, 0, ((size_t)n_strands + 1) * 4, &stream);
    ac_launch("prev_fill", &stream, PrevFillBody{d_next_off.as<uint32_t>(), d_next.as<UStrand>(), d_prev_off.as<uint32_t>(), prev_cnt.as<uint32_t>(), d_prev.as<UStrand>()}, n_strands);
    ac_launch("prev_sort", &stream, PrevSortBody{d_prev_off.as<uint32_t>(), d_prev.as<UStrand>()}, n_strands);
}

void DevicePipeline::Impl::paths() {
    d_path.ensure(n_runs * 4); d_path_off.ensure(((size_t)n_seqs + 1) * 8);
    ac_launch("path", &stream, PathBody{seqs.as<SeqInfo>(), n_seqs, run_start.as<uint64_t>(), run_len.as<uint32_t>(), run_unitig.as<uint32_t>(), rank.as<uint32_t>(),
                                        unitigs.as<DeviceUnitig>(), d_path.as<UStrand>(), d_min_fpos.as<uint32_t>(), d_min_rpos.as<uint32_t>()}, n_runs);
    d_rec.ensure((size_t)U * sizeof(UnitigRec));
    ac_launch("pack_rec", &stream, PackRecBody{d_seq_off.as<uint64_t>(), d_len.as<uint32_t>(), d_min_fpos.as<uint32_t>(), d_min_rpos.as<uint32_t>(), d_rec.as<UnitigRec>()}, U);
    ac_launch("path_off", &stream, PathOffBody{seqs.as<SeqInfo>(), n_seqs, run_start.as<uint64_t>(), n_runs, d_path_off.as<uint64_t>()}, (uint64_t)n_seqs + 1);
    num_prefix.ensure((size_t)U * 8);
    ac_launch("number_key", &stream, NumberKeyBody{d_rec.as<UnitigRec>(), d_arena.as<char>(), num_prefix.as<uint64_t>()}, U);
    const NumberLess number_less{d_rec.as<UnitigRec>(), d_depth.as<uint32_t>(), d_arena.as<char>(), num_prefix.as<uint64_t>(), nullptr};
    R.order_built = sort_indices(&stream, number_less, U, sort_a.as<uint32_t>(), sort_b.as<uint32_t>(), sort_ra.as<SortRec>(), sort_rb.as<SortRec>());
}

void DevicePipeline::Impl::work_list() {
    d_fixed.ensure((size_t)U * 4); ac_memset(d_fixed.p, 0, (size_t)U * 4, &stream);
    uint8_t* seed_start = d_fixed.as<uint8_t>(); uint8_t* seed_end = seed_start + U; uint8_t* fix_start = R.fix_start = seed_end + U; uint8_t* fix_end = fix_start + U;
    ac_launch("fixed_seed", &stream, FixedSeedBody{d_path_off.as<uint64_t>(), d_path.as<UStrand>(), seed_start, seed_end}, n_seqs);
    ac_copy_dd(fix_start, seed_start, (size_t)U * 2, &stream);
    ac_launch("fixed_spread", &stream, FixedSpreadBody{seed_start, seed_end, d_next_off.as<uint32_t>(), d_next.as<UStrand>(), d_prev_off.as<uint32_t>(), d_prev.as<UStrand>(),
                                                       fix_start, fix_end}, U);
    const CandidateView cview{R.order_built, d_next_off.as<uint32_t>(), d_next.as<UStrand>(), d_prev_off.as<uint32_t>(), d_prev.as<UStrand>(), fix_start, fix_end};
    cand_flag.ensure((2 * (size_t)U + 1) * 4); cand_index.ensure((2 * (size_t)U + 1) * 4);
    ac_launch("candidate_flag", &stream, CandidateFlagBody{cview, U, cand_flag.as<uint32_t>()}, 2ull * U + 1);
    const uint64_t n_cands = R.n_cands = scan(&stream, cand_flag.as<uint32_t>(), cand_index.as<uint32_t>(), 2ull * U + 1);
    d_cands.ensure((n_cands + 1) * sizeof(ExpandCandidate)); d_cand_at.ensure(2 * (size_t)U * 4 + 4); d_deps.ensure((size_t)U * sizeof(ExpandDeps) + 4); d_spec.ensure((n_cands + 1) * 4);
    ac_launch("candidate_fill", &stream, CandidateFillBody{cview, cand_flag.as<uint32_t>(), cand_index.as<uint32_t>(), d_cands.as<ExpandCandidate>(), d_cand_at.as<int32_t>()}, 2ull * U);
    ac_launch("dependents", &stream, DependentsBody{d_next_off.as<uint32_t>(), d_next.as<UStrand>(), d_prev_off.as<uint32_t>(), d_prev.as<UStrand>(), d_cand_at.as<int32_t>(),
                                                    d_deps.as<ExpandDeps>()}, U);
    ac_launch("common_length", &stream, CommonLengthBody{d_cands.as<ExpandCandidate>(), d_rec.as<UnitigRec>(), d_arena.as<char>(), d_spec.as<uint32_t>()}, n_cands);
    mark(WORK_LIST_END);
}

void DevicePipeline::Impl::simplify() {
    const uint64_t n_cands = R.n_cands, arena_bytes = R.arena_final;
    d_pred.ensure(n_cands * 7 * 4); d_level.ensure(n_cands * 4); d_flagmax.ensure(32); d_counters64.ensure((AC_PASS_WORDS + 8) * 8);
    d_dirty.ensure(((n_cands + 63) / 64) * 8 + 8); d_exhausted.ensure(n_cands + 8);
    unsigned long long* c64 = d_counters64.as<unsigned long long>();
    unsigned long long* res = c64 + AC_PASS_WORDS;
    ac_launch("level_pred", &stream, LevelPredBody{d_cands.as<ExpandCandidate>(), d_deps.as<ExpandDeps>(), d_pred.as<int32_t>()}, n_cands);
    ac_memset(d_level.p, 0, n_cands * 4, &stream); ac_memset(d_flagmax.p, 0, 32, &stream);
    ac_launch_coop("levels", &stream, LevelsCoopBody{d_pred.as<int32_t>(), d_level.as<uint32_t>(), d_flagmax.as<uint32_t>(), n_cands}, n_cands, 1024);
    ac_memset(d_counters64.p, 0, (AC_PASS_WORDS + 8) * 8, &stream);
    const RelocBoundBody bound_body{d_cands.as<ExpandCandidate>(), d_rec.as<UnitigRec>(), d_cand_at.as<int32_t>(), c64 + AC_PASS_SET(1) + 1};
    ac_launch("reloc_bound", &stream, bound_body, n_cands);
    uint32_t fm[8]; unsigned long long h64[AC_PASS_WORDS + 8];
    ac_d2h(fm, d_flagmax.p, 32, &stream); ac_d2h(h64, c64, sizeof h64, &stream); ac_sync(&stream);
    if (fm[4]) throw std::runtime_error("candidate levels did not settle");
    unsigned long long bound = 0; for (int x = 0; x < AC_BOUND_STRIPES; ++x) bound += h64[AC_PASS_SET(1) + 1 + x];
    if (arena_bytes + bound >= 0xFFFFFFF0ull) throw std::runtime_error("unitig sequence arena would exceed 4 GB");
    d_arena2.ensure(arena_bytes + 2 * bound + 64);
    ac_copy_dd(d_arena2.p, d_arena.p, arena_bytes, &stream);
    const unsigned long long start = arena_bytes;
    ac_h2d(c64, &start, 8, &stream);
    ac_memset(c64 + AC_PASS_SET(1), 0, AC_PASS_SET_WORDS * 8, &stream);
    ac_memset(d_dirty.p, 0, ((n_cands + 63) / 64) * 8 + 8, &stream); ac_memset(d_exhausted.p, 0, n_cands + 8, &stream);
    static const bool always_grow = getenv("AC_DEVICE_TIGHT_ARENA") != nullptr;
    uint32_t next_set = 0, next_due = 0; uint64_t passes = 0;
    const uint32_t due_stride = fm[3] + 2;
    d_due.ensure((size_t)3 * due_stride * 4); ac_memset(d_due.p, 0, (size_t)3 * due_stride * 4, &stream);
    for (bool first = true;; first = false) {
        const ApplyLevelBody apply{d_cands.as<ExpandCandidate>(), d_deps.as<ExpandDeps>(), d_level.as<uint32_t>(), 0, d_spec.as<uint32_t>(),
                                   d_rec.as<UnitigRec>(), d_arena2.as<char>(), c64, c64, d_dirty.as<uint64_t>(), d_exhausted.as<uint8_t>(), first, c64 + AC_PASS_REMOVED};
        const uint64_t room = always_grow ? 0 : d_arena2.cap;
        ac_launch_coop("simplify", &stream, SimplifyCoopBody{apply, bound_body, n_cands, d_flagmax.as<uint32_t>() + 3, c64, res, room, next_set, first,
                                                             d_due.as<uint32_t>(), due_stride, next_due}, n_cands, 64);
        ac_d2h(h64, c64, sizeof h64, &stream); ac_sync(&stream);
        const unsigned long long* r = h64 + AC_PASS_WORDS;
        R.arena_final = h64[0]; R.bases_removed = h64[AC_PASS_REMOVED]; R.any_moved = r[1] != 0;
        passes += r[2]; next_set = (uint32_t)r[5]; next_due = (uint32_t)r[7];
        if (getenv("AC_HOST_PROFILE")) fprintf(stderr, "[device] expand_repeats launch: %llu passes (%llu so far), %u levels, %llu candidates, %llu left on the work list, last pass moved %llu bases\n",
                                               r[2], (unsigned long long)passes, fm[3], (unsigned long long)n_cands, r[4], r[0]);
        if (r[0] == 0) break;
        if (passes > 1000000) throw std::runtime_error("repeat expansion did not settle");
        bound = r[3];
        if (R.arena_final + bound >= 0xFFFFFFF0ull) throw std::runtime_error("unitig sequence arena would exceed 4 GB");
        d_arena3.ensure(std::max<size_t>((R.arena_final + bound) * 2 + 64, d_arena3.cap + (always_grow ? 64 : 0)));
        ac_copy_dd(d_arena3.p, d_arena2.p, R.arena_final, &stream); ac_sync(&stream);
        std::swap(d_arena2.p, d_arena3.p); std::swap(d_arena2.cap, d_arena3.cap);
    }
    R.arena_src = &d_arena2;
}

void DevicePipeline::Impl::renumber() {
    if (!R.any_moved) { R.final_order = R.order_built; return; }
    d_pos.ensure((size_t)U * 4); sort_c.ensure((size_t)U * 4); sort_d.ensure((size_t)U * 4);
    ac_launch("inverse_perm", &stream, InversePermBody{R.order_built, d_pos.as<uint32_t>()}, U);
    ac_launch("number_key", &stream, NumberKeyBody{d_rec.as<UnitigRec>(), R.arena_src->as<char>(), num_prefix.as<uint64_t>()}, U);
    const NumberLess final_less{d_rec.as<UnitigRec>(), d_depth.as<uint32_t>(), R.arena_src->as<char>(), num_prefix.as<uint64_t>(), d_pos.as<uint32_t>()};
    R.final_order = sort_indices(&stream, final_less, U, sort_c.as<uint32_t>(), sort_d.as<uint32_t>(), sort_ra.as<SortRec>(), sort_rb.as<SortRec>());
}

void DevicePipeline::Impl::gfa(bool split_paths) {
    d_pos2.ensure((size_t)U * 4);
    ac_launch("inverse_perm", &stream, InversePermBody{R.final_order, d_pos2.as<uint32_t>()}, U);
    const GfaView gv{R.final_order, d_pos2.as<uint32_t>(), d_rec.as<UnitigRec>(), R.arena_src->as<char>(), d_depth.as<uint32_t>(), d_next_off.as<uint32_t>(), d_next.as<UStrand>()};
    gfa_s_size.ensure(((size_t)U + 1) * 4); gfa_l_size.ensure(((size_t)U + 1) * 4); gfa_pieces.ensure(((size_t)U + 1) * 4);
    const uint64_t steps = split_paths ? 0 : n_runs;
    d_last.ensure(steps + 8); gfa_p_size.ensure((steps + 1) * 4);
    ac_launch("gfa_size", &stream, GfaSizeBody{gv, U, gfa_s_size.as<uint32_t>(), gfa_l_size.as<uint32_t>()}, (uint64_t)U + 1);
    ac_launch("gfa_chunk_count", &stream, GfaChunkCountBody{gv, U, gfa_pieces.as<uint32_t>()}, (uint64_t)U + 1);
    d_totals.ensure(64); ac_memset(d_totals.p, 0, 64, &stream);
    if (!split_paths) {
        ac_memset(d_last.p, 0, steps + 8, &stream);
        ac_launch("path_last", &stream, PathLastBody{d_path_off.as<uint64_t>(), d_last.as<uint8_t>()}, n_seqs);
        ac_launch("path_size", &stream, PathSizeBody{d_path.as<UStrand>(), d_pos2.as<uint32_t>(), d_last.as<uint8_t>(), steps, gfa_p_size.as<uint32_t>()}, steps + 1);
        scan.keep_total(&stream, gfa_p_size.as<uint32_t>(), steps + 1, d_totals.as<uint32_t>() + 3);
    }
    scan.keep_total(&stream, gfa_s_size.as<uint32_t>(), (uint64_t)U + 1, d_totals.as<uint32_t>() + 0);
    scan.keep_total(&stream, gfa_l_size.as<uint32_t>(), (uint64_t)U + 1, d_totals.as<uint32_t>() + 1);
    scan.keep_total(&stream, gfa_pieces.as<uint32_t>(), (uint64_t)U + 1, d_totals.as<uint32_t>() + 2);
    uint32_t tot[4];
    ac_d2h(tot, d_totals.p, 16, &stream); ac_sync(&stream);
    const uint64_t s_bytes = tot[0], l_bytes = tot[1], n_pieces = tot[2], p_list_bytes = tot[3];
    char head[64]; const uint64_t head_bytes = (uint64_t)snprintf(head, sizeof head, "H\tVN:Z:1.0\tKM:i:%u\n", k);
    if (path_wrap_total == 0 && n_seqs) throw std::runtime_error("set_path_line_texts() must precede a build that renders the GFA");
    const uint64_t p_bytes = split_paths ? 0 : p_list_bytes + path_wrap_total;
    R.gfa_bytes = head_bytes + s_bytes + l_bytes + p_bytes;
    d_text.ensure(R.gfa_bytes + 64);
    char* text = d_text.as<char>();
    ac_h2d(text, head, head_bytes, &stream);
    ac_launch("gfa_segment", &stream, GfaSegmentBody{gv, gfa_s_size.as<uint32_t>(), text + head_bytes}, U);
    ac_launch("gfa_sequence", &stream, GfaSequenceBody{gv, U, gfa_pieces.as<uint32_t>(), gfa_s_size.as<uint32_t>(), text + head_bytes}, 32 * n_pieces);
    h_text.ensure(R.gfa_bytes + 64);
    copy_text_after_rendering(head_bytes + s_bytes);
    ac_launch("gfa_link", &stream, GfaLinkBody{gv, gfa_l_size.as<uint32_t>(), text + head_bytes + s_bytes}, U);
    copy_text_after_rendering(head_bytes + s_bytes + l_bytes);
    const PathLineView pv{d_path_off.as<uint64_t>(), n_seqs, gfa_p_size.as<uint32_t>(), d_wrap_off.as<uint64_t>(), d_pre_len.as<uint32_t>(), d_suf_len.as<uint32_t>(),
                          d_blob.as<char>(), d_blob_off.as<uint64_t>(), 0};
    char* p_text = text + head_bytes + s_bytes + l_bytes;
    if (!split_paths) {
        ac_launch("path_text", &stream, PathTextFullBody{d_path.as<UStrand>(), d_pos2.as<uint32_t>(), d_last.as<uint8_t>(), pv, p_text}, steps);
        ac_launch("path_wrap", &stream, PathWrapBody{pv, p_text}, 64ull * n_seqs);
    }
    R.paths_split = split_paths;
    R.gfa_on_device = true;
}

void DevicePipeline::Impl::results(PipelineResult& out, bool keep_positions, bool fused) {
    if (before_results && *before_results) (*before_results)();
    out.fused = fused; out.graph_fetched = false;
    if (fused && !R.gfa_on_device) throw std::runtime_error("fused build: the device GFA writer did not run");
    uint64_t d2h = 0;
    if (R.gfa_on_device) {
        copy_text_after_rendering(R.gfa_bytes);
        ac_record(&text_copied, &copy_stream); ac_wait(&stream, &text_copied);
        d2h += R.gfa_bytes;
    }
    uint32_t small[16];
    ac_d2h(small, d_small.p, 64, &stream); ac_sync(&stream); d2h += 64;
    out.links_single = (R.n_links - small[0]) / 2 + small[0];
    out.length_before = n_slots_used;
    out.length_after = n_slots_used - R.bases_removed;
    out.gfa_text = R.gfa_on_device ? h_text.as<char>() : nullptr; out.gfa_bytes = R.gfa_on_device ? R.gfa_bytes : 0;
    out.n_unitigs = U; out.n_runs = n_runs; out.n_seqs = n_seqs; out.n_links = R.n_links;
    out.h2d_bytes = uploaded_bytes + (uint64_t)n_seqs * sizeof(SeqInfo);
    out.d2h_bytes = d2h;
    if (!fused) pull_graph(out, keep_positions);
    else { mark(ALL_BUT_ARENA); mark(RESULTS_END); arena_pending = true; }
}

void DevicePipeline::Impl::pull_graph(PipelineResult& out, bool keep_positions) {
    const uint64_t n_links = R.n_links, n_cands = R.n_cands; const uint32_t n_strands = 2 * U;
    const uint64_t arena_cap = R.arena_final + R.arena_final / 4 + (1u << 20);
    h_rec.ensure((size_t)U * sizeof(UnitigRec)); h_depth.ensure((size_t)U * 4);
    h_arena.ensure(arena_cap); h_next_off.ensure(((size_t)n_strands + 1) * 4); h_prev_off.ensure(((size_t)n_strands + 1) * 4);
    h_next.ensure(n_links * 4 + 4); h_prev.ensure(n_links * 4 + 4); h_path.ensure(n_runs * 4 + 4); h_path_off.ensure(((size_t)n_seqs + 1) * 8);
    uint64_t d2h = 0;
    auto pull = [&](PinBuf& dst, DevBuf& src, size_t bytes) { if (bytes) ac_d2h(dst.p, src.p, bytes, &stream); d2h += bytes; };
    pull(h_rec, d_rec, (size_t)U * sizeof(UnitigRec)); pull(h_depth, d_depth, (size_t)U * 4);
    const bool plain = !out.fused;
    if (plain) { h_order.ensure((size_t)U * 4 + 4); if (U) { ac_d2h(h_order.p, R.order_built, (size_t)U * 4, &stream); d2h += (size_t)U * 4; } }
    pull(h_next_off, d_next_off, ((size_t)n_strands + 1) * 4); pull(h_prev_off, d_prev_off, ((size_t)n_strands + 1) * 4);
    pull(h_next, d_next, n_links * 4); pull(h_prev, d_prev, n_links * 4); pull(h_path, d_path, n_runs * 4); pull(h_path_off, d_path_off, ((size_t)n_seqs + 1) * 8);
    if (keep_positions) {
        h_run_start.ensure(n_runs * 8 + 8); h_run_len.ensure(n_runs * 4 + 4);
        pull(h_run_start, run_start, n_runs * 8); pull(h_run_len, run_len, n_runs * 4);
    }
    if (plain) {
        h_cands.ensure((n_cands + 1) * sizeof(ExpandCandidate)); h_deps.ensure((size_t)U * sizeof(ExpandDeps) + 4); h_spec.ensure((n_cands + 1) * 4); h_fixed.ensure((size_t)U * 2 + 4);
        pull(h_cands, d_cands, n_cands * sizeof(ExpandCandidate)); pull(h_deps, d_deps, (size_t)U * sizeof(ExpandDeps)); pull(h_spec, d_spec, n_cands * 4);
        if (U) { ac_d2h(h_fixed.p, R.fix_start, (size_t)U * 2, &stream); d2h += (size_t)U * 2; }
    } else { h_order2.ensure((size_t)U * 4 + 4); if (U) { ac_d2h(h_order2.p, R.final_order, (size_t)U * 4, &stream); d2h += (size_t)U * 4; } }
    mark(ALL_BUT_ARENA);
    pull(h_arena, *R.arena_src, R.arena_final);
    out.d2h_bytes += d2h;
    mark(RESULTS_END);
    wait_mark(ALL_BUT_ARENA);
    out.graph_fetched = true;
    out.rec = h_rec.as<UnitigRec>(); out.depth = h_depth.as<uint32_t>();
    out.order = plain ? h_order.as<uint32_t>() : nullptr; out.final_order = plain ? nullptr : h_order2.as<uint32_t>();
    out.n_cands = plain ? n_cands : 0; out.cands = plain ? h_cands.as<ExpandCandidate>() : nullptr; out.deps = plain ? h_deps.as<ExpandDeps>() : nullptr;
    out.spec_len = plain ? h_spec.as<uint32_t>() : nullptr;
    out.fixed_start = plain ? h_fixed.as<uint8_t>() : nullptr; out.fixed_end = plain ? h_fixed.as<uint8_t>() + U : nullptr;
    out.arena = h_arena.as<char>(); out.arena_used = R.arena_final; out.arena_cap = arena_cap;
    out.next_off = h_next_off.as<uint32_t>(); out.next = h_next.as<UStrand>(); out.prev_off = h_prev_off.as<uint32_t>(); out.prev = h_prev.as<UStrand>();
    out.path_off = h_path_off.as<uint64_t>(); out.path = h_path.as<UStrand>();
    out.run_start = keep_positions ? h_run_start.as<uint64_t>() : nullptr; out.run_len = keep_positions ? h_run_len.as<uint32_t>() : nullptr;
    arena_pending = true;
}

void DevicePipeline::complete(PipelineResult& out) {
    Impl& m = *impl; m.make_current();
    if (!m.arena_pending) return;
    ac_sync(&m.stream);
    m.arena_pending = false;
    PipelineTimings& t = out.t;
    const struct { float* field; Mark from, to; } spans[] = {
        {&t.h2d, UPLOAD_BEGIN, UPLOAD_END}, {&t.pack, PACK_BEGIN, PACK_END}, {&t.sample, PACK_END, SAMPLE_END}, {&t.insert, SAMPLE_END, TABLE_END},
        {&t.insert_kernel, INSERT_BEGIN, INSERT_END}, {&t.adjacency, RUNS_BEGIN, ADJACENCY_END}, {&t.boundaries, ADJACENCY_END, BOUNDARIES_END},
        {&t.runs, FINISH_BEGIN, UNITIGS_END}, {&t.unitigs, UNITIGS_END, SEEDS_END}, {&t.links, SEEDS_END, LINKS_END}, {&t.seed_sort, LINKS_END, SEED_SORT_END},
        {&t.emit, SEED_SORT_END, WORK_LIST_END}, {&t.simplify, WORK_LIST_END, SIMPLIFY_END}, {&t.gfa, SIMPLIFY_END, GFA_END}, {&t.d2h, GFA_END, RESULTS_END}};
    for (const auto& s : spans) *s.field = m.between(s.from, s.to);
    t.total = m.between(PACK_BEGIN, TABLE_END) + m.between(RUNS_BEGIN, BOUNDARIES_END) + m.between(FINISH_BEGIN, RESULTS_END);
}

void DevicePipeline::export_path_tokens(void* dst, uint64_t stride, const uint64_t* counts, uint32_t n_ranks) {
    Impl& m = *impl; m.make_current();
    if (m.stage < Stage::RUNS || !m.R.gfa_on_device || !m.R.paths_split) throw std::runtime_error("export_path_tokens follows a finish with split path lines");
    if (n_ranks == 0 || n_ranks > AC_MAX_RANKS) throw std::runtime_error("export_path_tokens: bad rank count");
    PathTokenBody body{m.d_path.as<UStrand>(), m.d_pos2.as<uint32_t>(), (uint32_t*)dst, stride, n_ranks, {0}};
    for (uint32_t q = 0; q < n_ranks; ++q) { if (counts[q] > stride) throw std::runtime_error("export_path_tokens: a rank holds more occurrences than the stride"); body.first[q + 1] = body.first[q] + counts[q]; }
    if (body.first[n_ranks] != m.n_runs) throw std::runtime_error("export_path_tokens: the counts do not add up to the occurrences imported");
    ac_launch("path_tokens", &m.stream, body, m.n_runs);
}
void DevicePipeline::render_path_lines(const void* tokens, uint64_t n_tokens, const char** text, uint64_t* bytes) {
    Impl& m = *impl; m.make_current();
    m.require(Stage::RUNS, "runs_local must precede render_path_lines");
    if (n_tokens != m.n_own_runs) throw std::runtime_error("render_path_lines: one token per occurrence of this rank's sequences is expected");
    if (m.path_pre.size() != m.n_seqs) throw std::runtime_error("set_path_line_texts() must precede render_path_lines");
    const uint32_t lo = m.own_seq_lo, hi = m.own_seq_hi, n_own = hi - lo;
    uint64_t wrap_lo = 0, wrap_hi = 0;
    for (uint32_t i = 0; i < hi; ++i) { const uint64_t b = (uint64_t)m.path_pre[i] + m.path_suf[i]; wrap_hi += b; if (i < lo) wrap_lo += b; }
    uint64_t total_bytes = 0;
    if (n_own) {
        const uint64_t steps = n_tokens;
        m.d_own_off.ensure(((size_t)n_own + 1) * 8); m.d_own_last.ensure(steps + 8); m.d_own_size.ensure((steps + 1) * 4);
        ac_launch("path_off", &m.stream, PathOffBody{m.seqs.as<SeqInfo>() + lo, n_own, m.run_start.as<uint64_t>(), steps, m.d_own_off.as<uint64_t>()}, (uint64_t)n_own + 1);
        ac_memset(m.d_own_last.p, 0, steps + 8, &m.stream);
        ac_launch("path_last", &m.stream, PathLastBody{m.d_own_off.as<uint64_t>(), m.d_own_last.as<uint8_t>()}, n_own);
        ac_launch("path_size", &m.stream, PathSizeBody{(const UStrand*)tokens, nullptr, m.d_own_last.as<uint8_t>(), steps, m.d_own_size.as<uint32_t>()}, steps + 1);
        const uint64_t list_bytes = m.scan(&m.stream, m.d_own_size.as<uint32_t>(), m.d_own_size.as<uint32_t>(), steps + 1);
        total_bytes = list_bytes + (wrap_hi - wrap_lo);
        m.d_ptext.ensure(total_bytes + 64);
        const PathLineView pv{m.d_own_off.as<uint64_t>(), n_own, m.d_own_size.as<uint32_t>(), m.d_wrap_off.as<uint64_t>() + lo, m.d_pre_len.as<uint32_t>() + lo,
                              m.d_suf_len.as<uint32_t>() + lo, m.d_blob.as<char>(), m.d_blob_off.as<uint64_t>() + lo, wrap_lo};
        ac_launch("path_text", &m.stream, PathTextFullBody{(const UStrand*)tokens, nullptr, m.d_own_last.as<uint8_t>(), pv, m.d_ptext.as<char>()}, steps);
        ac_launch("path_wrap", &m.stream, PathWrapBody{pv, m.d_ptext.as<char>()}, 64ull * n_own);
        m.h_ptext.ensure(total_bytes + 64);
        ac_d2h(m.h_ptext.p, m.d_ptext.p, total_bytes, &m.stream);
    }
    ac_sync(&m.stream);
    *text = total_bytes ? m.h_ptext.as<char>() : nullptr; *bytes = total_bytes;
}

void DevicePipeline::build_local(uint32_t seq_lo, uint32_t seq_hi, bool multi) {
    Impl& m = *impl; m.make_current(); const int W = m.W;
    AC_DISPATCH_W(m.local_w, seq_lo, seq_hi, multi)
}
uint64_t DevicePipeline::count_entries() {
    Impl& m = *impl; m.make_current(); const int W = m.W;
    uint64_t count = 0;
    AC_DISPATCH_W(count = m.count_entries_w)
    return count;
}
void DevicePipeline::merge_entries(const void* dev_ptr, uint64_t n) {
    Impl& m = *impl; m.make_current(); const int W = m.W;
    AC_DISPATCH_W(m.merge_w, dev_ptr, n)
}
void DevicePipeline::runs_local() {
    Impl& m = *impl; m.make_current(); const int W = m.W;
    AC_DISPATCH_W(m.runs_local_w)
}
uint64_t DevicePipeline::local_runs() const { return impl->n_runs; }
void DevicePipeline::import_runs_padded(const void* dev_ptr, uint64_t stride, const uint64_t* counts, uint32_t n_ranks) {
    if (n_ranks == 0 || n_ranks > AC_MAX_RANKS) throw std::runtime_error("import_runs_padded: bad rank count");
    const void* ptrs[AC_MAX_RANKS];
    for (uint32_t q = 0; q < n_ranks; ++q) { if (counts[q] > stride) throw std::runtime_error("import_runs_padded: a rank holds more records than the stride"); ptrs[q] = (const char*)dev_ptr + (size_t)q * stride * sizeof(RunRec); }
    import_runs_from(ptrs, counts, n_ranks);
}
const void* DevicePipeline::export_entries_own(uint64_t* n) {
    const uint64_t count = count_entries();
    impl->own_entries.ensure((count + 1) * sizeof(SlotRec));
    export_entries(impl->own_entries.p, count);
    *n = count;
    return impl->own_entries.p;
}
const void* DevicePipeline::export_runs_own(uint64_t* n) {
    Impl& m = *impl; m.make_current();
    m.own_runs.ensure((m.n_runs + 1) * sizeof(RunRec));
    export_runs(m.own_runs.p, m.n_runs);
    *n = m.n_runs;
    return m.own_runs.p;
}
void DevicePipeline::enable_peer_access(const int* devices, int n) {
#ifndef AC_EMULATE
    for (int a = 0; a < n; ++a)
        for (int b = 0; b < n; ++b) {
            if (a == b) continue;
            int can = 0;
            AC_CUDA_CHECK(cudaDeviceCanAccessPeer(&can, devices[a], devices[b]));
            if (!can) throw std::runtime_error("device " + std::to_string(devices[a]) + " cannot map the memory of device " + std::to_string(devices[b]) + " (no peer access)");
            AC_CUDA_CHECK(cudaSetDevice(devices[a]));
            const cudaError_t e = cudaDeviceEnablePeerAccess(devices[b], 0);
            if (e != cudaSuccess && e != cudaErrorPeerAccessAlreadyEnabled) throw std::runtime_error(std::string("cudaDeviceEnablePeerAccess: ") + cudaGetErrorString(e));
            cudaGetLastError();
        }
#else
    (void)devices; (void)n;
#endif
}
void* DevicePipeline::strand_block(uint32_t seq_lo, uint32_t seq_hi, uint64_t* n_bytes) {
    Impl& m = *impl;
    if (seq_lo > seq_hi || seq_hi > m.n_seqs || m.total == 0) throw std::runtime_error("strand_block: bad range, or nothing uploaded");
    const SeqInfo* q = m.host_seqs.data();
    const uint64_t b0 = seq_lo < m.n_seqs ? q[seq_lo].start : m.total, b1 = seq_hi < m.n_seqs ? q[seq_hi].start : m.total;
    *n_bytes = b1 - b0;
    return m.ascii.as<uint8_t>() + b0;
}
void DevicePipeline::fetch_graph(PipelineResult& out, bool keep_positions) {
    Impl& m = *impl; m.make_current();
    if (m.stage < Stage::RUNS || !out.fused) throw std::runtime_error("fetch_graph follows a fused build");
    if (out.graph_fetched) return;
    m.pull_graph(out, keep_positions);
}

void DevicePipeline::build(PipelineResult& out, bool keep_positions, bool fused) {
    build_local(0, impl->n_seqs, false);
    runs_local();
    finish(out, keep_positions, fused);
}
```

Measured before the change: 5347.

## Remove host round-trips by sizing launches from device-resident counts

Adds a launch variant that reads the element count from device memory and bounds the grid by a host-side upper bound. This lets the candidate scan, table-overflow check, level computation and relocation bound run without stream synchronisations, and the remaining scalar readbacks are batched into a single sync. It also splits repeat emission into one base per thread by shrinking the minimum chunk. In exchange, buffers are sized to worst-case bounds, some grids are oversized, and a deferred table-overflow check moves error handling later in the fused build.

```diff
diff --git a/autocycler_b200/csrc/backend.h b/autocycler_b200/csrc/backend.h
--- a/autocycler_b200/csrc/backend.h
+++ b/autocycler_b200/csrc/backend.h
@@ -8,6 +8,7 @@
 #include <string>
 
 extern unsigned long long g_ac_kernel_launches;
+extern unsigned long long g_ac_host_waits;
 
 #ifdef AC_EMULATE
 #define AC_HD inline
@@ -35,7 +36,7 @@
 inline void ac_h2d(void* d, const void* h, size_t bytes, AcStream*) { memcpy(d, h, bytes); }
 inline void ac_d2h(void* h, const void* d, size_t bytes, AcStream*) { memcpy(h, d, bytes); }
 inline void ac_copy_dd(void* dst, const void* src, size_t bytes, AcStream*) { memcpy(dst, src, bytes); }
-inline void ac_sync(AcStream*) {}
+inline void ac_sync(AcStream*) { ++g_ac_host_waits; }
 inline void* ac_host_alloc(size_t bytes) { return malloc(bytes ? bytes : 1); }
 inline void ac_host_free(void* p) { free(p); }
 inline int ac_smem_optin() { return 227 * 1024; }
@@ -49,6 +50,12 @@
 template <class Body> inline void ac_launch(const char*, AcStream*, const Body& body, uint64_t n);
 template <int CTAS, class Body> inline void ac_launch_occ(const char* name, AcStream* st, const Body& body, uint64_t n) { ac_launch(name, st, body, n); }
 template <class Body> inline void ac_launch(const char*, AcStream*, const Body& body, uint64_t n) {
+    for (uint64_t i = 0; i < n; ++i) body(i);
+}
+template <class Body> inline void ac_launch_dev(const char* name, AcStream*, const Body& body, uint64_t n_bound, const uint32_t* n_dev, uint32_t lanes = 1) {
+    if (n_bound == 0) return;
+    const uint64_t n = (uint64_t)*n_dev * lanes;
+    if (n > n_bound * lanes) throw std::runtime_error(std::string("launch ") + name + ": device count above its bound");
     for (uint64_t i = 0; i < n; ++i) body(i);
 }
 struct AcGridSync { void operator()() const {} };
@@ -106,7 +113,7 @@
 inline void ac_h2d(void* d, const void* h, size_t bytes, AcStream* st) { AC_CUDA_CHECK(cudaMemcpyAsync(d, h, bytes, cudaMemcpyHostToDevice, st->s)); }
 inline void ac_d2h(void* h, const void* d, size_t bytes, AcStream* st) { AC_CUDA_CHECK(cudaMemcpyAsync(h, d, bytes, cudaMemcpyDeviceToHost, st->s)); }
 inline void ac_copy_dd(void* dst, const void* src, size_t bytes, AcStream* st) { AC_CUDA_CHECK(cudaMemcpyAsync(dst, src, bytes, cudaMemcpyDeviceToDevice, st->s)); }
-inline void ac_sync(AcStream* st) { AC_CUDA_CHECK(cudaStreamSynchronize(st->s)); }
+inline void ac_sync(AcStream* st) { ++g_ac_host_waits; AC_CUDA_CHECK(cudaStreamSynchronize(st->s)); }
 inline void ac_debug_sync(const char* name, AcStream* st) {
     static const bool on = getenv("AC_SYNC_LAUNCHES") != nullptr;
     if (!on) return;
@@ -226,6 +233,24 @@
     uint64_t want = (n + threads - 1) / threads;
     const uint64_t max_blocks = ac_sm_count() * 16;
     ac_launch_kernel(name, st, ac_body_kernel<Body>, (unsigned)(want < max_blocks ? want : max_blocks), threads, 0, body, n);
+}
+
+template <class Body> __global__ void __launch_bounds__(256) ac_body_kernel_dev(const Body body, const uint32_t* n_dev, uint32_t lanes) {
+    const uint64_t n = (uint64_t)*n_dev * lanes;
+    const uint64_t stride = (uint64_t)gridDim.x * blockDim.x;
+    const uint32_t lane = threadIdx.x & 31u;
+    for (uint64_t base = (uint64_t)blockIdx.x * blockDim.x + (threadIdx.x - lane); base < n; base += stride) {
+        const uint64_t i = base + lane;
+        if (i < n) body(i);
+        __syncwarp();
+    }
+}
+template <class Body> inline void ac_launch_dev(const char* name, AcStream* st, const Body& body, uint64_t n_bound, const uint32_t* n_dev, uint32_t lanes = 1) {
+    if (n_bound == 0) return;
+    const int threads = 256;
+    uint64_t want = (n_bound * lanes + threads - 1) / threads;
+    const uint64_t max_blocks = ac_sm_count() * 16;
+    ac_launch_kernel(name, st, ac_body_kernel_dev<Body>, (unsigned)(want < max_blocks ? want : max_blocks), threads, 0, body, n_dev, lanes);
 }
 #endif
 #endif
diff --git a/autocycler_b200/csrc/pipeline.cu b/autocycler_b200/csrc/pipeline.cu
--- a/autocycler_b200/csrc/pipeline.cu
+++ b/autocycler_b200/csrc/pipeline.cu
@@ -5,10 +5,11 @@
 #include <vector>
 
 unsigned long long g_ac_kernel_launches = 0;
+unsigned long long g_ac_host_waits = 0;
 
 #define AC_NONE32 0xFFFFFFFFu
 #define AC_CHUNK 32
-#define AC_MINCHUNK 128
+#define AC_MINCHUNK 32
 #define AC_MAX_RANKS 16
 #define AC_BOUND_STRIPES 64
 #ifndef AC_INSERT_CTAS
@@ -577,6 +578,10 @@
 };
 
 struct ClaimedCountBody { const uint32_t* bits; uint64_t n_words; uint32_t* cnt; AC_D void operator()(uint64_t w) const { cnt[w] = w < n_words ? ac_popc(bits[w]) : 0u; } };
+template <class Body> struct IfTableOk {
+    Body body; const unsigned long long* counters;
+    AC_D void operator()(uint64_t i) const { if (counters[2] | counters[3]) return; body(i); }
+};
 template <int W> struct ClaimedListBody {
     const uint32_t* bits; const uint32_t* off; const uint32_t* pos_slot; uint32_t* list;
     TableView t; KParams p; const uint8_t* interior; uint64_t* filter; uint64_t n_fwords;
@@ -894,16 +899,17 @@
 struct EmitSeqBody {
     const uint64_t* packed; uint32_t h; const DeviceUnitig* unitigs; uint32_t n_unitigs; const uint32_t* chunk_off;
     const uint32_t* rank; const uint64_t* seq_off; char* arena;
-    AC_D void operator()(uint64_t c) const {
+    AC_D void operator()(uint64_t i) const {
+        const uint64_t c = i / AC_MINCHUNK, t = i % AC_MINCHUNK;
         uint32_t lo = 0, hi = n_unitigs;
         while (hi - lo > 1) { uint32_t mid = (lo + hi) >> 1; if (chunk_off[mid] <= c) lo = mid; else hi = mid; }
         const DeviceUnitig u = unitigs[lo];
         const uint64_t first = (c - chunk_off[lo]) * AC_MINCHUNK;
-        const uint64_t n = (u.len - first < AC_MINCHUNK) ? u.len - first : AC_MINCHUNK;
+        if (first + t >= u.len) return;
         char* dst = arena + seq_off[rank[lo]];
-        const uint64_t g0 = u.start + h + first;
-        if (!u.flip) for (uint64_t t = 0; t < n; ++t) dst[first + t] = "ACGT"[packed_base(packed, g0 + t)];
-        else for (uint64_t t = 0; t < n; ++t) dst[u.len - 1 - (first + t)] = "TGCA"[packed_base(packed, g0 + t)];
+        const uint32_t b = packed_base(packed, u.start + h + first + t);
+        if (!u.flip) dst[first + t] = "ACGT"[b];
+        else dst[u.len - 1 - (first + t)] = "TGCA"[b];
     }
 };
 
@@ -1108,8 +1114,9 @@
     }
 };
 struct LevelsCoopBody {
-    const int32_t* pred; uint32_t* level; uint32_t* flags; uint64_t n;
+    const int32_t* pred; uint32_t* level; uint32_t* flags; const uint32_t* n_cands;
     template <class Sync> AC_D void operator()(uint64_t tid, uint64_t nt, Sync& sync) const {
+        const uint64_t n = *n_cands;
         for (uint32_t round = 0;; ++round) {
             uint32_t* changed = flags + round % 3;
             if (tid == 0) flags[(round + 1) % 3] = 0;
@@ -1597,7 +1604,7 @@
 enum class Stage { UPLOADED, TABLE, RUNS };
 
 struct DevicePipeline::Impl : DeviceContext {
-    uint64_t total = 0; uint32_t n_seqs = 0, k = 0, U = 0, n_chunks = 0; int W = 0;
+    uint64_t total = 0; uint32_t n_seqs = 0, k = 0, U = 0, chunk_bound = 0; int W = 0;
     DevBuf ascii, seqs, d_wrap_off, d_pre_len, d_suf_len, d_blob, d_blob_off, needles;
     ScratchSet scratch;
     ScratchBuf packed{scratch}, interior8{scratch}, slots{scratch}, pos_slot{scratch}, counters{scratch}, count_big{scratch}, claimed{scratch}, claimed_cnt{scratch}, occ_list{scratch},
@@ -1616,6 +1623,7 @@
     DeviceScan scan;
     PinBuf h_rec, h_depth, h_order, h_order2, h_arena, h_next_off, h_next, h_prev_off, h_prev, h_path, h_path_off, h_run_start, h_run_len;
     PinBuf h_cands, h_deps, h_spec, h_fixed, h_text, h_ptext;
+    PinBuf h_counts;
 #ifndef AC_EMULATE
     cudaEvent_t ev[N_MARKS];
     AcStream copy_stream;
@@ -1652,16 +1660,21 @@
     static uint32_t count_alarm() { static const uint32_t a = getenv("AC_COUNT_ALARM") ? (uint32_t)atoi(getenv("AC_COUNT_ALARM")) : AC_SLOT_COUNT_ALARM; return a; }
     template <int W> void local_w(uint32_t seq_lo, uint32_t seq_hi, bool multi);
     template <int W> void insert_w();
+    template <int W> void insert_attempt();
+    bool table_retry(const unsigned long long* hc);
+    bool defer_table_check = false;
+    unsigned long long waits_before = 0;
     uint64_t safe_cap = 0;
     int table_attempt = 0;
     std::vector<std::pair<const void*, uint64_t>> merged;
     template <int W> void merge_w(const void* dev_ptr, uint64_t n);
     template <int W> void runs_local_w();
     template <int W> void unitigs_w(PipelineResult& out);
-    void host_arrays(), paths(), work_list(), simplify(), renumber(), gfa(bool split_paths);
+    void host_arrays(), paths(), work_list(bool fused), simplify(), renumber(), gfa(bool split_paths);
     void results(PipelineResult& out, bool keep_positions, bool fused);
     struct Pending {
         uint64_t n_links = 0, n_cands = 0;
+        uint32_t levels = 0, levels_unsettled = 0; unsigned long long reloc_bound = 0;
         uint32_t* order_built = nullptr; uint32_t* final_order = nullptr; uint8_t* fix_start = nullptr;
         DevBuf* arena_src = nullptr; uint64_t arena_final = 0;
         bool any_moved = false, gfa_on_device = false, paths_split = false;
@@ -1671,7 +1684,7 @@
     std::vector<char> path_blob; std::vector<uint32_t> path_pre, path_suf; uint64_t path_wrap_total = 0;
     uint64_t uploaded_bytes = 0;
     uint64_t exp_n = 0, n_own_runs = 0; uint32_t own_seq_lo = 0, own_seq_hi = 0; bool exp_valid = false;
-    template <int W> uint64_t list_claimed(bool with_filter);
+    template <int W> uint64_t list_claimed(bool with_filter, bool want_count);
     template <int W> uint64_t count_entries_w();
 #ifdef AC_EMULATE
     static void fill(DevBuf* b) { static const bool on = getenv("AC_EMU_POISON") != nullptr; if (on && b->p) memset(b->p, 0xA5, b->cap); }
@@ -1783,6 +1796,7 @@
     if (seq_lo == seq_hi) { g_begin = g_end = 0; }
     else { g_begin = hs[seq_lo].start; g_end = hs[seq_hi - 1].start + hs[seq_hi - 1].len; }
     is_multi = multi; own_seq_lo = seq_lo; own_seq_hi = seq_hi; exp_valid = false;
+    waits_before = g_ac_host_waits;
     poison();
     n_windows = total - (uint64_t)n_seqs * (k - 1);
     cap = (n_windows + n_windows / 2 + 64 + 3) & ~3ull;
@@ -1798,6 +1812,7 @@
 
     const uint64_t safe_cap = cap;
     counters.ensure(AC_N_COUNTERS * sizeof(unsigned long long));
+    h_counts.ensure(32 + AC_BOUND_STRIPES * 8);
     unsigned long long hc[AC_N_COUNTERS] = {0, 0, 0, 0};
     big_counts = getenv("AC_BIG_COUNTS") != nullptr;
     const double load = getenv("AC_TABLE_LOAD") ? atof(getenv("AC_TABLE_LOAD")) : 0.5;
@@ -1825,54 +1840,62 @@
 }
 
 template <int W> void DevicePipeline::Impl::insert_w() {
+    pos_slot.ensure(total * sizeof(uint32_t));
+    for (;;) {
+        insert_attempt<W>();
+        if (defer_table_check) return;
+        unsigned long long* hc = h_counts.as<unsigned long long>();
+        ac_d2h(hc, counters.p, AC_N_COUNTERS * 8, &stream); ac_sync(&stream);
+        if (!table_retry(hc)) return;
+    }
+}
+template <int W> void DevicePipeline::Impl::insert_attempt() {
     const KParams p = make_kparams(k, W);
     const uint64_t n_words = (total + 31) / 32;
-    unsigned long long hc[AC_N_COUNTERS] = {0, 0, 0, 0};
-    pos_slot.ensure(total * sizeof(uint32_t));
-    for (;; ++table_attempt) {
-        if (table_attempt > 3) throw std::runtime_error("k-mer table build did not settle");
-        if (getenv("AC_HOST_PROFILE")) fprintf(stderr, "[device] k-mer table attempt %d: capacity %llu, side counts %d\n", table_attempt, (unsigned long long)cap, (int)big_counts);
-        poison_table();
-        slots.ensure(cap * sizeof(Slot));
-        ac_memset(slots.p, 0xFF, cap * sizeof(Slot), &stream);
-        if (big_counts) { count_big.ensure(cap * 4); ac_memset(count_big.p, 0, cap * 4, &stream); }
-        ac_memset(counters.p, 0, sizeof hc, &stream);
-        const TableView tv = table_view();
-        const uint64_t g_first = g_begin & ~63ull;
-        claimed.ensure((n_words + 8) * 4); ac_memset(claimed.p, 0, (n_words + 8) * 4, &stream);
-        const InsertBody<W> ins{tv, p, interior8.as<uint8_t>(), (uint32_t)g_first, (uint32_t)g_begin, (uint32_t)g_end, is_multi, pos_slot.as<uint32_t>(), counters.as<unsigned long long>(), false, claimed.as<uint32_t>()};
-        mark(INSERT_BEGIN);
-        ac_launch_occ<AC_INSERT_CTAS>("insert", &stream, ins, (g_end - g_first + 63) / 64 * 32);
-        mark(INSERT_END);
-        ac_d2h(hc, counters.p, sizeof hc, &stream); ac_sync(&stream);
-        if (hc[2] && cap != safe_cap) { cap = safe_cap; continue; }
-        if (hc[2]) throw std::runtime_error("k-mer table overflow");
-        if (hc[3] && !big_counts) { big_counts = true; continue; }
-        break;
-    }
+    if (table_attempt > 3) throw std::runtime_error("k-mer table build did not settle");
+    if (getenv("AC_HOST_PROFILE")) fprintf(stderr, "[device] k-mer table attempt %d: capacity %llu, side counts %d\n", table_attempt, (unsigned long long)cap, (int)big_counts);
+    poison_table();
+    slots.ensure(cap * sizeof(Slot));
+    ac_memset(slots.p, 0xFF, cap * sizeof(Slot), &stream);
+    if (big_counts) { count_big.ensure(cap * 4); ac_memset(count_big.p, 0, cap * 4, &stream); }
+    ac_memset(counters.p, 0, AC_N_COUNTERS * 8, &stream);
+    const TableView tv = table_view();
+    const uint64_t g_first = g_begin & ~63ull;
+    claimed.ensure((n_words + 8) * 4); ac_memset(claimed.p, 0, (n_words + 8) * 4, &stream);
+    const InsertBody<W> ins{tv, p, interior8.as<uint8_t>(), (uint32_t)g_first, (uint32_t)g_begin, (uint32_t)g_end, is_multi, pos_slot.as<uint32_t>(), counters.as<unsigned long long>(), false, claimed.as<uint32_t>()};
+    mark(INSERT_BEGIN);
+    ac_launch_occ<AC_INSERT_CTAS>("insert", &stream, ins, (g_end - g_first + 63) / 64 * 32);
+    mark(INSERT_END);
     ++table_attempt;
+}
+bool DevicePipeline::Impl::table_retry(const unsigned long long* hc) {
+    if (hc[2] && cap != safe_cap) { cap = safe_cap; return true; }
+    if (hc[2]) throw std::runtime_error("k-mer table overflow");
+    if (hc[3] && !big_counts) { big_counts = true; return true; }
     n_dotted = hc[1];
-}
-
-template <int W> uint64_t DevicePipeline::Impl::list_claimed(bool with_filter) {
+    return false;
+}
+
+template <int W> uint64_t DevicePipeline::Impl::list_claimed(bool with_filter, bool want_count) {
     const uint64_t n_words = (total + 31) / 32;
     claimed_cnt.ensure((n_words + 1) * 4);
     ac_launch("claimed_count", &stream, ClaimedCountBody{claimed.as<uint32_t>(), n_words, claimed_cnt.as<uint32_t>()}, n_words + 1);
-    const uint64_t n = scan(&stream, claimed_cnt.as<uint32_t>(), claimed_cnt.as<uint32_t>(), n_words + 1);
-    occ_list.ensure((n + 1) * 4);
+    const uint64_t n = scan(&stream, claimed_cnt.as<uint32_t>(), claimed_cnt.as<uint32_t>(), n_words + 1, want_count);
+    occ_list.ensure((cap + 1) * 4);
     if (with_filter) {
         static const uint64_t words_env = getenv("AC_EXT_FILTER_WORDS") ? strtoull(getenv("AC_EXT_FILTER_WORDS"), nullptr, 10) : 0;
-        n_fwords = words_env ? words_env : n / 2 + 64;
+        n_fwords = words_env ? words_env : cap / 4 + 64;
         ext_filter.ensure(n_fwords * 8);
         ac_memset(ext_filter.p, 0, n_fwords * 8, &stream);
     }
-    ac_launch("claimed_list", &stream, ClaimedListBody<W>{claimed.as<uint32_t>(), claimed_cnt.as<uint32_t>(), pos_slot.as<uint32_t>(), occ_list.as<uint32_t>(),
-                                                          table_view(), make_kparams(k, W), interior8.as<uint8_t>(), with_filter ? ext_filter.as<uint64_t>() : nullptr, n_fwords}, n_words * 32);
+    const ClaimedListBody<W> list{claimed.as<uint32_t>(), claimed_cnt.as<uint32_t>(), pos_slot.as<uint32_t>(), occ_list.as<uint32_t>(),
+                                  table_view(), make_kparams(k, W), interior8.as<uint8_t>(), with_filter ? ext_filter.as<uint64_t>() : nullptr, n_fwords};
+    ac_launch("claimed_list", &stream, IfTableOk<ClaimedListBody<W>>{list, counters.as<unsigned long long>()}, n_words * 32);
     return n;
 }
 template <int W> uint64_t DevicePipeline::Impl::count_entries_w() {
     require(Stage::TABLE, "build_local must precede the entry export");
-    exp_n = list_claimed<W>(false);
+    exp_n = list_claimed<W>(false, true);
     exp_valid = true;
     return exp_n;
 }
@@ -1909,24 +1932,37 @@
         if (hc[3] && !big_counts) throw std::runtime_error("a k-mer occurs more than 524287 times across the ranks: not supported by the multi-GPU exchange");
         n_dotted = hc[1];
     }
-    any_dotted = n_dotted != 0;
-    const TableView tv = table_view();
-
-    flags8.ensure(cap);
-    n_slots_used = list_claimed<W>(true);
-    const AdjacencyBody<W> adj{tv, p, any_dotted, occ_list.as<uint32_t>(), flags8.as<uint8_t>(), ext_filter.as<uint64_t>(), n_fwords};
-    if (is_multi && exp_valid && exp_n + 64 < n_slots_used) {
-        const uint64_t n_cw = (total + 31) / 32, n_adj = exp_n + 64;
-        if (getenv("AC_HOST_PROFILE")) fprintf(stderr, "[device] adjacency flags for this rank's own k-mers: at most %llu of %llu\n", (unsigned long long)n_adj, (unsigned long long)n_slots_used);
-        ac_launch("adjacency", &stream, AdjacencyOwnBody<W>{adj, claimed_cnt.as<uint32_t>(), g_begin >> 5, std::min<uint64_t>((g_end + 31) >> 5, n_cw)}, n_adj);
-    } else ac_launch("adjacency", &stream, adj, n_slots_used);
-    mark(ADJACENCY_END);
-
-    const uint64_t n_bwords = (total + 31) / 32;
-    bmask.ensure(n_bwords * sizeof(uint32_t)); bcount.ensure(n_bwords * sizeof(uint32_t)); boff.ensure(n_bwords * sizeof(uint32_t));
-    ac_launch("boundaries", &stream, BoundaryBody{packed.as<uint64_t>(), seqs.as<SeqInfo>(), n_seqs, p.h, g_begin, g_end, pos_slot.as<uint32_t>(),
-                                                  flags8.as<uint8_t>(), interior8.as<uint8_t>(), bmask.as<uint32_t>(), bcount.as<uint32_t>()}, n_bwords * 32);
-    n_runs = scan(&stream, bcount.as<uint32_t>(), boff.as<uint32_t>(), n_bwords);
+    const uint64_t n_words = (total + 31) / 32, n_bwords = n_words;
+    unsigned long long* hc = h_counts.as<unsigned long long>();
+    uint32_t* h32 = (uint32_t*)(hc + AC_N_COUNTERS);
+    for (;;) {
+        any_dotted = defer_table_check ? std::any_of(host_seqs.begin(), host_seqs.end(), [](const SeqInfo& q) { return q.lead || q.trail; }) : n_dotted != 0;
+        const TableView tv = table_view();
+        flags8.ensure(cap);
+        n_slots_used = list_claimed<W>(true, is_multi);
+        const AdjacencyBody<W> adj{tv, p, any_dotted, occ_list.as<uint32_t>(), flags8.as<uint8_t>(), ext_filter.as<uint64_t>(), n_fwords};
+        if (is_multi && exp_valid && exp_n + 64 < n_slots_used) {
+            const uint64_t n_cw = (total + 31) / 32, n_adj = exp_n + 64;
+            if (getenv("AC_HOST_PROFILE")) fprintf(stderr, "[device] adjacency flags for this rank's own k-mers: at most %llu of %llu\n", (unsigned long long)n_adj, (unsigned long long)n_slots_used);
+            ac_launch("adjacency", &stream, AdjacencyOwnBody<W>{adj, claimed_cnt.as<uint32_t>(), g_begin >> 5, std::min<uint64_t>((g_end + 31) >> 5, n_cw)}, n_adj);
+        } else ac_launch_dev("adjacency", &stream, IfTableOk<AdjacencyBody<W>>{adj, counters.as<unsigned long long>()}, cap, claimed_cnt.as<uint32_t>() + n_words);
+        mark(ADJACENCY_END);
+
+        bmask.ensure(n_bwords * sizeof(uint32_t)); bcount.ensure((n_bwords + 1) * sizeof(uint32_t)); boff.ensure((n_bwords + 1) * sizeof(uint32_t));
+        ac_memset(bcount.as<uint32_t>() + n_bwords, 0, 4, &stream);
+        ac_launch("boundaries", &stream, IfTableOk<BoundaryBody>{BoundaryBody{packed.as<uint64_t>(), seqs.as<SeqInfo>(), n_seqs, p.h, g_begin, g_end, pos_slot.as<uint32_t>(),
+                                                  flags8.as<uint8_t>(), interior8.as<uint8_t>(), bmask.as<uint32_t>(), bcount.as<uint32_t>()}, counters.as<unsigned long long>()}, n_bwords * 32);
+        scan(&stream, bcount.as<uint32_t>(), boff.as<uint32_t>(), n_bwords + 1, false);
+        ac_d2h(hc, counters.p, AC_N_COUNTERS * 8, &stream);
+        ac_d2h(h32, claimed_cnt.as<uint32_t>() + n_words, 4, &stream);
+        ac_d2h(h32 + 1, boff.as<uint32_t>() + n_bwords, 4, &stream);
+        ac_sync(&stream);
+        if (!defer_table_check || !table_retry(hc)) break;
+        insert_w<W>();
+        mark(TABLE_END); mark(RUNS_BEGIN);
+    }
+    if (any_dotted != (n_dotted != 0)) throw std::runtime_error("dotted k-mers and the sequences' dots disagree");
+    n_slots_used = h32[0]; n_runs = h32[1];
     mark(BOUNDARIES_END);
     run_start.ensure(n_runs * sizeof(uint64_t)); run_len.ensure(n_runs * 4); run_hs.ensure(n_runs * 4); run_ts.ensure(n_runs * 4);
     ac_launch("run_scatter", &stream, RunScatterBody{bmask.as<uint32_t>(), boff.as<uint32_t>(), run_start.as<uint64_t>()}, n_bwords);
@@ -1972,7 +2008,7 @@
     AC_DISPATCH_W(m.unitigs_w, out)
     m.host_arrays();
     m.paths();
-    m.work_list();
+    m.work_list(fused);
     if (fused && m.R.n_cands > 0) m.simplify();
     m.mark(SIMPLIFY_END);
     if (fused) {
@@ -2008,10 +2044,11 @@
     nchunks.ensure(((size_t)U + 1) * 4); chunk_off.ensure(((size_t)U + 1) * 4);
     ac_launch("chunk_count", &stream, ChunkCountBody{unitigs.as<DeviceUnitig>(), nchunks.as<uint32_t>()}, U);
     ac_memset(nchunks.as<uint32_t>() + U, 0, 4, &stream);
-    n_chunks = scan(&stream, nchunks.as<uint32_t>(), chunk_off.as<uint32_t>(), (uint64_t)U + 1);
-    partial.ensure((size_t)n_chunks * sizeof(MinPartial<W>));
-    ac_launch("chunk_min", &stream, ChunkMinBody<W>{packed.as<uint64_t>(), seqs.as<SeqInfo>(), n_seqs, p, unitigs.as<DeviceUnitig>(), U,
-                                                    chunk_off.as<uint32_t>(), partial.as<MinPartial<W>>()}, n_chunks);
+    scan(&stream, nchunks.as<uint32_t>(), chunk_off.as<uint32_t>(), (uint64_t)U + 1, false);
+    chunk_bound = (uint32_t)(n_windows / AC_MINCHUNK + U);
+    partial.ensure((size_t)chunk_bound * sizeof(MinPartial<W>));
+    ac_launch_dev("chunk_min", &stream, ChunkMinBody<W>{packed.as<uint64_t>(), seqs.as<SeqInfo>(), n_seqs, p, unitigs.as<DeviceUnitig>(), U,
+                                                        chunk_off.as<uint32_t>(), partial.as<MinPartial<W>>()}, chunk_bound, chunk_off.as<uint32_t>() + U);
     ac_launch("unitig_min", &stream, UnitigMinBody<W>{chunk_off.as<uint32_t>(), partial.as<MinPartial<W>>(), unitigs.as<DeviceUnitig>()}, U);
     mark(SEEDS_END);
 
@@ -2030,20 +2067,22 @@
     d_seq_off.ensure((size_t)U * 8); d_min_fpos.ensure((size_t)U * 4); d_min_rpos.ensure((size_t)U * 4);
     ac_launch("seed_gather", &stream, SeedGatherBody{perm, unitigs.as<DeviceUnitig>(), U, rank.as<uint32_t>(), d_len.as<uint32_t>(), d_depth.as<uint32_t>(),
                                                      need.as<uint32_t>(), d_min_fpos.as<uint32_t>(), d_min_rpos.as<uint32_t>()}, (uint64_t)U + 1);
-    if (n_windows + (uint64_t)U * 2 * AC_SEQ_SLACK >= 0xFFFFFFF0ull) throw std::runtime_error("unitig sequence arena would exceed 4 GB");
-    const uint64_t arena_bytes = scan(&stream, need.as<uint32_t>(), need.as<uint32_t>(), (uint64_t)U + 1);
+    const uint64_t arena_bound = n_windows + (uint64_t)U * 2 * AC_SEQ_SLACK;
+    if (arena_bound >= 0xFFFFFFF0ull) throw std::runtime_error("unitig sequence arena would exceed 4 GB");
+    scan(&stream, need.as<uint32_t>(), need.as<uint32_t>(), (uint64_t)U + 1, false);
     ac_launch("seq_off", &stream, SeqOffBody{need.as<uint32_t>(), d_seq_off.as<uint64_t>()}, U);
-    d_arena.ensure(arena_bytes);
-    ac_launch("emit_seq", &stream, EmitSeqBody{packed.as<uint64_t>(), make_kparams(k, W).h, unitigs.as<DeviceUnitig>(), U, chunk_off.as<uint32_t>(), rank.as<uint32_t>(),
-                                               d_seq_off.as<uint64_t>(), d_arena.as<char>()}, n_chunks);
-    R.arena_final = arena_bytes; R.arena_src = &d_arena;
+    d_arena.ensure(arena_bound);
+    ac_launch_dev("emit_seq", &stream, EmitSeqBody{packed.as<uint64_t>(), make_kparams(k, W).h, unitigs.as<DeviceUnitig>(), U, chunk_off.as<uint32_t>(), rank.as<uint32_t>(),
+                                                   d_seq_off.as<uint64_t>(), d_arena.as<char>()}, chunk_bound, chunk_off.as<uint32_t>() + U, AC_MINCHUNK);
+    R.arena_src = &d_arena;
     const uint32_t n_strands = 2 * U;
     strand_cnt.ensure(((size_t)n_strands + 1) * 4); d_next_off.ensure(((size_t)n_strands + 1) * 4);
     prev_cnt.ensure(((size_t)n_strands + 1) * 4); d_prev_off.ensure(((size_t)n_strands + 1) * 4);
     ac_launch("link_count", &stream, LinkCountBody{link_count.as<uint32_t>(), rank.as<uint32_t>(), unitigs.as<DeviceUnitig>(), n_strands, strand_cnt.as<uint32_t>()},
               (uint64_t)n_strands + 1);
-    const uint64_t n_links = R.n_links = scan(&stream, strand_cnt.as<uint32_t>(), d_next_off.as<uint32_t>(), (uint64_t)n_strands + 1);
-    d_next.ensure(n_links * 4); d_prev.ensure(n_links * 4);
+    scan(&stream, strand_cnt.as<uint32_t>(), d_next_off.as<uint32_t>(), (uint64_t)n_strands + 1, false);
+    const uint64_t link_bound = (uint64_t)n_strands * AC_MAX_LINKS;
+    d_next.ensure(link_bound * 4); d_prev.ensure(link_bound * 4);
     ac_memset(prev_cnt.p, 0, ((size_t)n_strands + 1) * 4, &stream);
     d_small.ensure(64); ac_memset(d_small.p, 0, 64, &stream);
     ac_launch("link_order", &stream, LinkOrderBody{link_count.as<uint32_t>(), links.as<uint32_t>(), rank.as<uint32_t>(), unitigs.as<DeviceUnitig>(),
@@ -2067,7 +2106,7 @@
     R.order_built = sort_indices(&stream, number_less, U, sort_a.as<uint32_t>(), sort_b.as<uint32_t>(), sort_ra.as<SortRec>(), sort_rb.as<SortRec>());
 }
 
-void DevicePipeline::Impl::work_list() {
+void DevicePipeline::Impl::work_list(bool fused) {
     d_fixed.ensure((size_t)U * 4); ac_memset(d_fixed.p, 0, (size_t)U * 4, &stream);
     uint8_t* seed_start = d_fixed.as<uint8_t>(); uint8_t* seed_end = seed_start + U; uint8_t* fix_start = R.fix_start = seed_end + U; uint8_t* fix_end = fix_start + U;
     ac_launch("fixed_seed", &stream, FixedSeedBody{d_path_off.as<uint64_t>(), d_path.as<UStrand>(), seed_start, seed_end}, n_seqs);
@@ -2077,31 +2116,50 @@
     const CandidateView cview{R.order_built, d_next_off.as<uint32_t>(), d_next.as<UStrand>(), d_prev_off.as<uint32_t>(), d_prev.as<UStrand>(), fix_start, fix_end};
     cand_flag.ensure((2 * (size_t)U + 1) * 4); cand_index.ensure((2 * (size_t)U + 1) * 4);
     ac_launch("candidate_flag", &stream, CandidateFlagBody{cview, U, cand_flag.as<uint32_t>()}, 2ull * U + 1);
-    const uint64_t n_cands = R.n_cands = scan(&stream, cand_flag.as<uint32_t>(), cand_index.as<uint32_t>(), 2ull * U + 1);
-    d_cands.ensure((n_cands + 1) * sizeof(ExpandCandidate)); d_cand_at.ensure(2 * (size_t)U * 4 + 4); d_deps.ensure((size_t)U * sizeof(ExpandDeps) + 4); d_spec.ensure((n_cands + 1) * 4);
+    scan(&stream, cand_flag.as<uint32_t>(), cand_index.as<uint32_t>(), 2ull * U + 1, false);
+    const uint64_t cand_bound = 2ull * U;
+    const uint32_t* n_cands_dev = cand_index.as<uint32_t>() + cand_bound;
+    d_cands.ensure((cand_bound + 1) * sizeof(ExpandCandidate)); d_cand_at.ensure(2 * (size_t)U * 4 + 4); d_deps.ensure((size_t)U * sizeof(ExpandDeps) + 4); d_spec.ensure((cand_bound + 1) * 4);
     ac_launch("candidate_fill", &stream, CandidateFillBody{cview, cand_flag.as<uint32_t>(), cand_index.as<uint32_t>(), d_cands.as<ExpandCandidate>(), d_cand_at.as<int32_t>()}, 2ull * U);
     ac_launch("dependents", &stream, DependentsBody{d_next_off.as<uint32_t>(), d_next.as<UStrand>(), d_prev_off.as<uint32_t>(), d_prev.as<UStrand>(), d_cand_at.as<int32_t>(),
                                                     d_deps.as<ExpandDeps>()}, U);
-    ac_launch("common_length", &stream, CommonLengthBody{d_cands.as<ExpandCandidate>(), d_rec.as<UnitigRec>(), d_arena.as<char>(), d_spec.as<uint32_t>()}, n_cands);
+    ac_launch_dev("common_length", &stream, CommonLengthBody{d_cands.as<ExpandCandidate>(), d_rec.as<UnitigRec>(), d_arena.as<char>(), d_spec.as<uint32_t>()}, cand_bound, n_cands_dev);
+    if (fused) {
+        d_pred.ensure(cand_bound * 7 * 4 + 4); d_level.ensure(cand_bound * 4 + 4); d_flagmax.ensure(32); d_counters64.ensure((AC_PASS_WORDS + 8) * 8);
+        unsigned long long* c64 = d_counters64.as<unsigned long long>();
+        ac_launch_dev("level_pred", &stream, LevelPredBody{d_cands.as<ExpandCandidate>(), d_deps.as<ExpandDeps>(), d_pred.as<int32_t>()}, cand_bound, n_cands_dev);
+        ac_memset(d_level.p, 0, cand_bound * 4, &stream); ac_memset(d_flagmax.p, 0, 32, &stream);
+        if (cand_bound) ac_launch_coop("levels", &stream, LevelsCoopBody{d_pred.as<int32_t>(), d_level.as<uint32_t>(), d_flagmax.as<uint32_t>(), n_cands_dev}, cand_bound, 1024);
+        ac_memset(d_counters64.p, 0, (AC_PASS_WORDS + 8) * 8, &stream);
+        ac_launch_dev("reloc_bound", &stream, RelocBoundBody{d_cands.as<ExpandCandidate>(), d_rec.as<UnitigRec>(), d_cand_at.as<int32_t>(), c64 + AC_PASS_SET(1) + 1}, cand_bound, n_cands_dev);
+    }
+    uint32_t* h32 = h_counts.as<uint32_t>();
+    unsigned long long* h64 = h_counts.as<unsigned long long>() + 4;
+    ac_d2h(h32 + 0, need.as<uint32_t>() + U, 4, &stream);
+    ac_d2h(h32 + 1, d_next_off.as<uint32_t>() + 2ull * U, 4, &stream);
+    ac_d2h(h32 + 2, n_cands_dev, 4, &stream);
+    if (fused) {
+        ac_d2h(h32 + 3, d_flagmax.as<uint32_t>() + 3, 8, &stream);
+        ac_d2h(h64, d_counters64.as<unsigned long long>() + AC_PASS_SET(1) + 1, AC_BOUND_STRIPES * 8, &stream);
+    }
+    ac_sync(&stream);
+    R.arena_final = h32[0]; R.n_links = h32[1]; R.n_cands = h32[2];
+    if (fused) {
+        R.levels = h32[3]; R.levels_unsettled = h32[4];
+        R.reloc_bound = 0; for (int x = 0; x < AC_BOUND_STRIPES; ++x) R.reloc_bound += h64[x];
+    }
     mark(WORK_LIST_END);
 }
 
 void DevicePipeline::Impl::simplify() {
     const uint64_t n_cands = R.n_cands, arena_bytes = R.arena_final;
-    d_pred.ensure(n_cands * 7 * 4); d_level.ensure(n_cands * 4); d_flagmax.ensure(32); d_counters64.ensure((AC_PASS_WORDS + 8) * 8);
     d_dirty.ensure(((n_cands + 63) / 64) * 8 + 8); d_exhausted.ensure(n_cands + 8);
     unsigned long long* c64 = d_counters64.as<unsigned long long>();
     unsigned long long* res = c64 + AC_PASS_WORDS;
-    ac_launch("level_pred", &stream, LevelPredBody{d_cands.as<ExpandCandidate>(), d_deps.as<ExpandDeps>(), d_pred.as<int32_t>()}, n_cands);
-    ac_memset(d_level.p, 0, n_cands * 4, &stream); ac_memset(d_flagmax.p, 0, 32, &stream);
-    ac_launch_coop("levels", &stream, LevelsCoopBody{d_pred.as<int32_t>(), d_level.as<uint32_t>(), d_flagmax.as<uint32_t>(), n_cands}, n_cands, 1024);
-    ac_memset(d_counters64.p, 0, (AC_PASS_WORDS + 8) * 8, &stream);
     const RelocBoundBody bound_body{d_cands.as<ExpandCandidate>(), d_rec.as<UnitigRec>(), d_cand_at.as<int32_t>(), c64 + AC_PASS_SET(1) + 1};
-    ac_launch("reloc_bound", &stream, bound_body, n_cands);
-    uint32_t fm[8]; unsigned long long h64[AC_PASS_WORDS + 8];
-    ac_d2h(fm, d_flagmax.p, 32, &stream); ac_d2h(h64, c64, sizeof h64, &stream); ac_sync(&stream);
-    if (fm[4]) throw std::runtime_error("candidate levels did not settle");
-    unsigned long long bound = 0; for (int x = 0; x < AC_BOUND_STRIPES; ++x) bound += h64[AC_PASS_SET(1) + 1 + x];
+    unsigned long long h64[AC_PASS_WORDS + 8];
+    if (R.levels_unsettled) throw std::runtime_error("candidate levels did not settle");
+    unsigned long long bound = R.reloc_bound;
     if (arena_bytes + bound >= 0xFFFFFFF0ull) throw std::runtime_error("unitig sequence arena would exceed 4 GB");
     d_arena2.ensure(arena_bytes + 2 * bound + 64);
     ac_copy_dd(d_arena2.p, d_arena.p, arena_bytes, &stream);
@@ -2111,7 +2169,7 @@
     ac_memset(d_dirty.p, 0, ((n_cands + 63) / 64) * 8 + 8, &stream); ac_memset(d_exhausted.p, 0, n_cands + 8, &stream);
     static const bool always_grow = getenv("AC_DEVICE_TIGHT_ARENA") != nullptr;
     uint32_t next_set = 0, next_due = 0; uint64_t passes = 0;
-    const uint32_t due_stride = fm[3] + 2;
+    const uint32_t due_stride = R.levels + 2;
     d_due.ensure((size_t)3 * due_stride * 4); ac_memset(d_due.p, 0, (size_t)3 * due_stride * 4, &stream);
     for (bool first = true;; first = false) {
         const ApplyLevelBody apply{d_cands.as<ExpandCandidate>(), d_deps.as<ExpandDeps>(), d_level.as<uint32_t>(), 0, d_spec.as<uint32_t>(),
@@ -2124,7 +2182,7 @@
         R.arena_final = h64[0]; R.bases_removed = h64[AC_PASS_REMOVED]; R.any_moved = r[1] != 0;
         passes += r[2]; next_set = (uint32_t)r[5]; next_due = (uint32_t)r[7];
         if (getenv("AC_HOST_PROFILE")) fprintf(stderr, "[device] expand_repeats launch: %llu passes (%llu so far), %u levels, %llu candidates, %llu left on the work list, last pass moved %llu bases\n",
-                                               r[2], (unsigned long long)passes, fm[3], (unsigned long long)n_cands, r[4], r[0]);
+                                               r[2], (unsigned long long)passes, R.levels, (unsigned long long)n_cands, r[4], r[0]);
         if (r[0] == 0) break;
         if (passes > 1000000) throw std::runtime_error("repeat expansion did not settle");
         bound = r[3];
@@ -2203,6 +2261,7 @@
     }
     uint32_t small[16];
     ac_d2h(small, d_small.p, 64, &stream); ac_sync(&stream); d2h += 64;
+    if (getenv("AC_HOST_PROFILE")) fprintf(stderr, "[device] host waits: %llu\n", g_ac_host_waits - waits_before);
     out.links_single = (R.n_links - small[0]) / 2 + small[0];
     out.length_before = n_slots_used;
     out.length_after = n_slots_used - R.bases_removed;
@@ -2380,6 +2439,7 @@
 }
 
 void DevicePipeline::build(PipelineResult& out, bool keep_positions, bool fused) {
+    struct Deferred { bool& on; explicit Deferred(bool& on) : on(on) { on = true; } ~Deferred() { on = false; } } deferred(impl->defer_table_check);
     build_local(0, impl->n_seqs, false);
     runs_local();
     finish(out, keep_positions, fused);
```

Result: no change. 5416 (median of 6 runs) (+1.3%).
